# dobrosketchkun/dither_pie

Hardware: AMD Instinct MI355X
Metric: Mpixel/s dither+quantize @4K 256-color (Bayer 8x8 + nearest-palette, uint8 RGB in/out) (higher is better)
Workload: dtype u8; 1 GPU; C2: Bayer 8x8 + 256-colour nearest palette palr(256,7), 3840x2160 RGB, 24 distinct frames rnd(2160,3840,1234+i) per GPU resident in HBM, frames sharded per rank; frames_per_gpu=24, h=2160, w=3840, colors=256, matrix=8x8, parallelism=frames x1

## Files before the change

dither_pie_amd/csrc/accel.hip:

```cpp
#include <algorithm>
#include <cstdio>
#include <cstdlib>
#include <string>
#include <vector>

#include "dp_internal.h"
#include "ordered_fine.h"
#include "tree_query.hip.h"

namespace dp {
namespace {

__device__ __forceinline__ int med3i(const int a, const int b, const int c)
{
    return max(min(a, b), min(max(a, b), c));
}

constexpr int kExcCap = 1 << 16;

template <int MW, int CAP>
__global__ __launch_bounds__(256) void accel_scan_kernel(const PalDev pal, uint32_t *__restrict__ masks,
                                                         uint32_t *__restrict__ nmasks, uint32_t *__restrict__ nsub, uint32_t *__restrict__ code1,
                                                         uint32_t *__restrict__ code2, uint4 *__restrict__ exc,
                                                         uint32_t *__restrict__ exc_count)
// ... 196 lines not shown
{
    const int cell = blockIdx.x;
    const int rc = cell >> 8, gc = (cell >> 4) & 15, bc = cell & 15;
    const int K = pal.K;
    constexpr int kBig = 0x7fffffff;
    constexpr int IM = (1 << kIdxBits) - 1;
    for (int t = 0; t < 16; ++t) {
        const int id = threadIdx.x + 256 * t;
        const uint32_t r = rc * 16 + (id >> 8), g = gc * 16 + ((id >> 4) & 15), b = bc * 16 + (id & 15);
        const uint32_t x4 = r | (g << 8) | (b << 16);
        int m0 = kBig, m1 = kBig, m2 = kBig, m3 = kBig;
        for (int j = 0; j < K; ++j) {
            const int dot = (int)__builtin_amdgcn_udot4(x4, pal.p4[j], 0u, false);
            const int key = pal.nkey[j] - (dot << (kIdxBits + 1));
            const int n3 = med3i(m2, m3, key);
            const int n2 = med3i(m1, m2, key);
            const int n1 = med3i(m0, m1, key);
            m0 = min(m0, key);
            m1 = n1;
            m2 = n2;
            m3 = n3;
        }
        const int d1 = m1 >> kIdxBits, d2 = m2 >> kIdxBits, d3 = m3 >> kIdxBits;
        const uint32_t ur = lut[r], ug = lut[256 + g], ub = lut[512 + b];
        const uint32_t wcell = ((ur >> 4) << 8) | ((ug >> 4) << 4) | (ub >> 4);
        const uint32_t sub = 1u + ((((ur >> 3) & 1u) << 2) | (((ug >> 3) & 1u) << 1) | ((ub >> 3) & 1u));
        uint32_t *whole = masks + (size_t)wcell * 9 * MW, *part = whole + (size_t)sub * MW;
        auto mark = [&](int j) {
            const uint32_t bit = 1u << (j & 31);
            if (!(whole[j >> 5] & bit)) atomicOr(&whole[j >> 5], bit);
            if (!(part[j >> 5] & bit)) atomicOr(&part[j >> 5], bit);
        };
        mark(m0 & IM);
        if (K > 1) mark(m1 & IM);
        if (K > 2 && d2 == d1) mark(m2 & IM);
        if (K > 3 && d3 == d1)
            for (int j = 0; j < K; ++j) {
                const int dot = (int)__builtin_amdgcn_udot4(x4, pal.p4[j], 0u, false);
                const int dj = (pal.nkey[j] - (dot << (kIdxBits + 1))) >> kIdxBits;
                if (dj <= d1) mark(j);
            }
    }
}


constexpr double kFloatListMargin = 1.0 + 6.103515625e-5;

__device__ __forceinline__ void float_members(const double *s_pts, const int K, const double r, const double g,
                                              const double b, uint32_t *mask_a, uint32_t *mask_b)
{
    const double inf = __longlong_as_double(0x7ff0000000000000LL);
    double b0 = inf, b1 = inf;
    for (int j = 0; j < K; ++j) {
        const double d = sq_dist3(s_pts + 3 * j, r, g, b);
        if (d < b1) {
            if (d < b0) {
                b1 = b0;
                b0 = d;
            } else {
                b1 = d;
            }
        }
    }
    const double bound = __dmul_rn(b1, kFloatListMargin);
    for (int j = 0; j < K; ++j) {
        const double d = sq_dist3(s_pts + 3 * j, r, g, b);
        if (d <= bound) {
            atomicOr(&mask_a[j >> 5], 1u << (j & 31));
            if (mask_b) atomicOr(&mask_b[j >> 5], 1u << (j & 31));
        }
    }
}

__global__ __launch_bounds__(256) void accel_scan_float_kernel(const PalDev pal, const uint8_t *__restrict__ reach,
                                                               uint32_t *__restrict__ masks)
{
    __shared__ uint32_t s_mask[9][8];
    __shared__ double s_pts[256 * 3];
    if (threadIdx.x < 72) (&s_mask[0][0])[threadIdx.x] = 0;
    for (int i = threadIdx.x; i < pal.K * 3; i += 256) s_pts[i] = pal.pts[i];
    __syncthreads();
    const int cell = blockIdx.x;
    const int rc = cell >> 8, gc = (cell >> 4) & 15, bc = cell & 15;
    for (int t = 0; t < 16; ++t) {
        const int id = threadIdx.x + 256 * t;
        const int r = rc * 16 + (id >> 8), g = gc * 16 + ((id >> 4) & 15), b = bc * 16 + (id & 15);
        if (!(reach[r] && reach[g] && reach[b])) continue;
        const int sub = 1 + (((((id >> 8) >> 3) & 1) << 2) | (((((id >> 4) & 15) >> 3) & 1) << 1) | (((id & 15) >> 3) & 1));
        float_members(s_pts, pal.K, (double)r, (double)g, (double)b, s_mask[0], s_mask[sub]);
    }
    __syncthreads();
    if (threadIdx.x < 72) masks[cell * 72 + threadIdx.x] = (&s_mask[0][0])[threadIdx.x];
}

__global__ __launch_bounds__(64) void accel_box_float_kernel(const PalDev pal, const uint8_t *__restrict__ reach,
                                                             const Box *__restrict__ boxes, uint32_t *__restrict__ masks)
{
    __shared__ uint32_t s_mask[8];
    __shared__ double s_pts[256 * 3];
    if (threadIdx.x < 8) s_mask[threadIdx.x] = 0;
    for (int i = threadIdx.x; i < pal.K * 3; i += 64) s_pts[i] = pal.pts[i];
    __syncthreads();
    const Box bx = boxes[blockIdx.x];
    const int n = bx.size * bx.size * bx.size;
    for (int id = threadIdx.x; id < n; id += 64) {
        const int r = bx.r0 + id / (bx.size * bx.size), g = bx.g0 + (id / bx.size) % bx.size, b = bx.b0 + id % bx.size;
        if (!(reach[r] && reach[g] && reach[b])) continue;
        float_members(s_pts, pal.K, (double)r, (double)g, (double)b, s_mask, nullptr);
    }
    __syncthreads();
    if (threadIdx.x < 8) masks[blockIdx.x * 8 + threadIdx.x] = s_mask[threadIdx.x];
}

}

namespace {


template <class B, class Launch>
int run_box_kernel(const std::vector<B> &boxes, std::vector<uint32_t> &bm, Launch launch)
{
    B *d_boxes = nullptr;
    uint32_t *d_bm = nullptr;
    hipError_t e = hipMalloc((void **)&d_boxes, sizeof(B) * boxes.size());
    if (e == hipSuccess) e = hipMalloc((void **)&d_bm, sizeof(uint32_t) * bm.size());
    if (e == hipSuccess) e = hipMemcpy(d_boxes, boxes.data(), sizeof(B) * boxes.size(), hipMemcpyHostToDevice);
    if (e == hipSuccess) {
        launch(d_boxes, d_bm, (unsigned)boxes.size());
        e = hipGetLastError();
    }
    if (e == hipSuccess) e = hipMemcpy(bm.data(), d_bm, sizeof(uint32_t) * bm.size(), hipMemcpyDeviceToHost);
    if (d_boxes) (void)hipFree(d_boxes);
    if (d_bm) (void)hipFree(d_bm);
    if (e != hipSuccess) return hip_fail(e, "accelerator refinement");
    return DP_OK;
}

}

int build_accel(PalDev &dev, const std::vector<uint32_t> &p4_host, void **blob_out, size_t *blob_bytes, std::vector<uint32_t> *fine_masks,
                uint32_t **fine_dev)
{
    *blob_out = nullptr;
    *blob_bytes = 0;
    fine_masks->clear();
    *fine_dev = nullptr;
    const int K = dev.K;
    constexpr size_t kCodeWords = (size_t)1 << 20;
    uint32_t *d_masks = nullptr;
    uint8_t *blob = nullptr;
    const int mw = K <= 256 ? 8 : 32;
    const bool big_q = dev.n_inner > kQueueSmall;
    const size_t bytes = sizeof(uint32_t) * (3 * kCodeWords + 2 * kTabMaxWords + kTabCapWords) + sizeof(uint4) * kExcCap + 16 + 768 +
                         sizeof(uint32_t) * (2 * kCells + 2 * kWideCap * kWideList + kCompactMaxWords) + kLeanTabBytes;
    DP_HIP(hipMalloc((void **)&blob, bytes));
    struct DevFree {
        void *p = nullptr;
        ~DevFree()
        {
            if (p) (void)hipFree(p);
        }
    } masks_guard;
    hipError_t e = hipMalloc((void **)&d_masks, sizeof(uint32_t) * kCells * 18 * mw);
    masks_guard.p = d_masks;
    uint32_t *d_nmasks = d_masks + (size_t)kCells * 9 * mw, *d_nsub = d_nmasks + (size_t)kCells * mw;
    if (e == hipSuccess) e = hipMemset(blob, 0, sizeof(uint32_t) * 3 * kCodeWords);
    if (e != hipSuccess) {
        (void)hipFree(blob);
        return hip_fail(e, "accelerator allocation");
    }
    uint32_t *code1 = reinterpret_cast<uint32_t *>(blob);
    uint32_t *code2 = code1 + kCodeWords;
    uint32_t *d_tab = code2 + 2 * kCodeWords;
    uint4 *d_exc = reinterpret_cast<uint4 *>(d_tab + kTabMaxWords);
    uint32_t *d_exc_count = reinterpret_cast<uint32_t *>(d_exc + kExcCap);
    e = hipMemset(d_exc_count, 0, sizeof(uint32_t));
    if (e != hipSuccess) {
        (void)hipFree(blob);
        return hip_fail(e, "accelerator allocation");
    }
#define DP_SCAN(MW, C) hipLaunchKernelGGL((accel_scan_kernel<MW, C>), dim3(kCells), dim3(256), 0, 0, dev, d_masks, d_nmasks, d_nsub, code1, code2, d_exc, d_exc_count)
    if (mw == 8) {
        if (big_q) DP_SCAN(8, kQueueLarge); else DP_SCAN(8, kQueueSmall);
    } else {
        if (big_q) DP_SCAN(32, kQueueLarge); else DP_SCAN(32, kQueueSmall);
    }
#undef DP_SCAN
    std::vector<uint32_t> masks((size_t)kCells * 9 * mw), nmasks((size_t)kCells * 9 * mw);
    e = hipGetLastError();
    if (e == hipSuccess) e = hipMemcpy(masks.data(), d_masks, sizeof(uint32_t) * masks.size(), hipMemcpyDeviceToHost);
    if (e == hipSuccess) e = hipMemcpy(nmasks.data(), d_nmasks, sizeof(uint32_t) * nmasks.size(), hipMemcpyDeviceToHost);
    if (e != hipSuccess) {
        (void)hipFree(blob);
        return hip_fail(e, "accelerator scan");
    }

    std::vector<uint32_t> tab;
    TableStats st;
    auto box_masks = [&](const std::vector<Box> &boxes, std::vector<uint32_t> &bm) {
        return run_box_kernel(boxes, bm, [&](const Box *db, uint32_t *dm, unsigned n) {
            if (mw == 8) hipLaunchKernelGGL(accel_box_kernel<8>, dim3(n), dim3(64), 0, 0, dev, db, dm);
            else hipLaunchKernelGGL(accel_box_kernel<32>, dim3(n), dim3(64), 0, 0, dev, db, dm);
        });
    };
    std::vector<uint32_t> tab4, perm4, perm8, wide4, wide8;
    TableStats st4;
    bool use4 = false;
    if (K <= 64) {
        const int rc4 = assemble_table(masks, mw, 4, kTabCapWords, K, p4_host, p4_host, box_masks, tab4, st4, nmasks.data(), 4, &perm4, &wide4);
        if (rc4 != DP_OK) {
            (void)hipFree(blob);
            return rc4;
        }
        use4 = !st4.too_big && st4.n_split_cells <= kCells * 4 / 100;
        if (exp_env("DP_DEBUG_ACCEL"))
            fprintf(stderr, "accel K=%d: 4-entry table: %d split cells, %d split nodes, %d slow, %zu words, too_big=%d -> use=%d\n", K,
                    st4.n_split_cells, st4.n_split, st4.n_slow, tab4.size(), (int)st4.too_big, (int)use4);
    }
    const bool have8 = K >= 8;
    if (have8) {
        const int rc = assemble_table(masks, mw, 8, kTabMaxWords, K, p4_host, p4_host, box_masks, tab, st, nmasks.data(), kNearSlots, &perm8, &wide8);
        if (rc != DP_OK) {
            (void)hipFree(blob);
            return rc;
        }
        if (exp_env("DP_DEBUG_ACCEL"))
            fprintf(stderr, "accel K=%d: 8-entry table: %d split cells, %d split nodes, %d slow, %zu words (%s), longest list %d, too_big=%d\n",
                    K, st.n_split_cells, st.n_split, st.n_slow, tab.size(), tab.size() <= (size_t)kTabCapWords ? "all in LDS" : "deep nodes in global memory",
                    st.max_cnt, (int)st.too_big);
    }
    if ((!have8 || st.too_big) && !use4) {
        (void)hipFree(blob);
        return DP_OK;
    }
    const std::vector<uint32_t> mass = mass_points(p4_host);
    const int n_mass = (int)mass.size();
    const bool ok8 = have8 && !st.too_big;
    const bool u8_spilled = ok8 && tab.size() > (size_t)kTabCapWords;
    const int m4 = use4 ? entries_in_split_cells(tab4, 4, mass) : n_mass;
    const int m8 = ok8 ? entries_in_split_cells(tab, 8, mass) : n_mass;
    if (use4 && ok8 && m4 * 20 > n_mass && m8 * 2 <= m4) use4 = false;
    const char *force_env = exp_env("DP_FORCE_TABLE");
    const std::string force = force_env ? force_env : "";
    if (force == "u4") use4 = K <= 64 && !st4.too_big;
    else if (!force.empty() && ok8) use4 = false;
    const int u_mass = use4 ? m4 : m8;
    const int u_cells = use4 ? st4.n_split_cells : st.n_split_cells;
    const bool u_spilled = !use4 && u8_spilled;
    const bool u_crowded = u_spilled || u_cells > kCells * 3 / 100 || u_mass * 4 >= n_mass;
    const bool try_warp = (u_crowded && !(use4 && m4 * 50 <= n_mass)) || u_mass * 50 > n_mass;
    std::vector<uint32_t> wtab;
    TableStats wst;
    WarpMaps wm;
    int wbw = 0, w_mass = 0;
    bool w_spilled = false;
    uint32_t *d_wtab = d_exc_count + 4 + kTabCapWords;
    uint8_t *d_lut = reinterpret_cast<uint8_t *>(d_wtab + kTabMaxWords);
    if (K >= 8 && (try_warp || force[0] == 'w') && force[0] != 'u' && !exp_env("DP_NO_WARP")) {
        make_warp(p4_host, wm);
        auto warped = [&](const uint32_t c) {
            return (uint32_t)wm.lut[0][c & 255] | ((uint32_t)wm.lut[1][(c >> 8) & 255] << 8) | ((uint32_t)wm.lut[2][(c >> 16) & 255] << 16);
        };
        std::vector<uint32_t> coordw(K), massw(mass.size());
        for (int j = 0; j < K; ++j) coordw[j] = warped(p4_host[j]);
        for (size_t j = 0; j < mass.size(); ++j) massw[j] = warped(mass[j]);
        e = hipMemcpy(d_lut, &wm.lut[0][0], 768, hipMemcpyHostToDevice);
        if (e == hipSuccess) e = hipMemset(d_masks, 0, sizeof(uint32_t) * kCells * 9 * mw);
        if (e == hipSuccess) {
            if (mw == 8) hipLaunchKernelGGL(accel_scan_warp_kernel<8>, dim3(kCells), dim3(256), 0, 0, dev, d_lut, d_masks);
            else hipLaunchKernelGGL(accel_scan_warp_kernel<32>, dim3(kCells), dim3(256), 0, 0, dev, d_lut, d_masks);
            e = hipGetLastError();
        }
        std::vector<uint32_t> wmasks((size_t)kCells * 9 * mw);
        if (e == hipSuccess) e = hipMemcpy(wmasks.data(), d_masks, sizeof(uint32_t) * wmasks.size(), hipMemcpyDeviceToHost);
        if (e != hipSuccess) {
            (void)hipFree(blob);
            return hip_fail(e, "accelerator scan (warped cells)");
        }
        auto box_masks_w = [&](const std::vector<Box> &boxes, std::vector<uint32_t> &bm) {
            std::vector<Range> ranges(boxes.size());
            for (size_t q = 0; q < boxes.size(); ++q) {
                const Box &b = boxes[q];
                ranges[q] = Range{wm.lo[0][b.r0], wm.lo[0][b.r0 + b.size], wm.lo[1][b.g0], wm.lo[1][b.g0 + b.size],
                                  wm.lo[2][b.b0], wm.lo[2][b.b0 + b.size]};
            }
            return run_box_kernel(ranges, bm, [&](const Range *db, uint32_t *dm, unsigned n) {
                if (mw == 8) hipLaunchKernelGGL(accel_range_kernel<8>, dim3(n), dim3(256), 0, 0, dev, db, dm);
                else hipLaunchKernelGGL(accel_range_kernel<32>, dim3(n), dim3(256), 0, 0, dev, db, dm);
            });
        };
        int w4_mass = -1;
        if (K <= 64 && force != "w8") {
            TableStats s4;
            std::vector<uint32_t> t4;
            const int rc4 = assemble_table(wmasks, mw, 4, kTabCapWords - 192, K, coordw, p4_host, box_masks_w, t4, s4);
            if (rc4 != DP_OK) {
                (void)hipFree(blob);
                return rc4;
            }
            w4_mass = s4.too_big ? n_mass : entries_in_split_cells(t4, 4, massw);
            if (!s4.too_big && ((s4.n_split_cells <= kCells / 100 && s4.n_slow == 0 && w4_mass * 50 <= n_mass) || force == "w4")) {
                wtab.swap(t4);
                wst = s4;
                wbw = 4;
                w_mass = w4_mass;
            }
        }
        if (wbw == 0) {
            const int rc8 = assemble_table(wmasks, mw, 8, kTabMaxWords, K, coordw, p4_host, box_masks_w, wtab, wst);
            if (rc8 != DP_OK) {
                (void)hipFree(blob);
                return rc8;
            }
            if (!wst.too_big) {
                wbw = 8;
                w_spilled = wtab.size() > (size_t)(kTabCapWords - 192);
                w_mass = entries_in_split_cells(wtab, 8, massw);
                if (w_spilled) crowded_nodes_first(wtab, wst, 8, coordw);
            }
        }
        if (exp_env("DP_DEBUG_ACCEL"))
            fprintf(stderr, "accel K=%d: mass in split cells: plain 4-entry %d, plain 8-entry %d of %d (in use: %d-entry, %d cells%s); warped 4-entry %d, "
                    "warped %d-entry table: %d, %d split cells, %d nodes, %d slow, %zu words%s\n",
                    K, m4, m8, n_mass, use4 ? 4 : 8, u_cells, u_spilled ? ", spilled" : "", w4_mass, wbw, w_mass, wst.n_split_cells, wst.n_split,
                    wst.n_slow, wtab.size(), w_spilled ? " (deep nodes in global memory)" : "");
        if (wbw != 0 && (w_mass * 2 > u_mass || (u_mass - w_mass) * 50 < n_mass) && !(u_spilled && !w_spilled) && force.empty()) wbw = 0;
    } else if (exp_env("DP_DEBUG_ACCEL")) {
        fprintf(stderr, "accel K=%d: mass in split cells: plain 4-entry %d, plain 8-entry %d of %d (in use: %d-entry, %d cells)\n", K, m4, m8, n_mass,
                use4 ? 4 : 8, u_cells);
    }
    dev.warp_tab = nullptr;
    dev.warp_lut = nullptr;
    dev.warp_words = dev.warp_total = dev.warp_bw = dev.warp_adapt = 0;
    dev.adapt = (!use4 && u_crowded) ? 1 : 0;
    if (wbw != 0) {
        e = hipMemcpy(d_wtab, wtab.data(), sizeof(uint32_t) * wtab.size(), hipMemcpyHostToDevice);
        if (e != hipSuccess) {
            (void)hipFree(blob);
            return hip_fail(e, "accelerator upload (warped cells)");
        }
        dev.warp_tab = d_wtab;
        dev.warp_lut = d_lut;
        dev.warp_bw = wbw;
        dev.warp_total = (int)wtab.size();
        dev.warp_words = w_spilled ? std::min((int)wtab.size(), kTabStageWords - 3 * 64) : (int)wtab.size();
        dev.warp_adapt = (wbw == 8 && (w_spilled || wst.n_split_cells > kCells * 3 / 100 || w_mass * 4 >= n_mass)) ? 1 : 0;
    }
    dev.cell_perm = dev.cell_perm4 = nullptr;
    dev.near_slots = 0;
    const bool fast8 = have8 && !st.too_big && !st.wide_overflow && !use4 && wbw == 0 && !dev.adapt && tab.size() <= (size_t)kTabCapWords &&
                       wide8.size() <= (size_t)kWideCap * kWideList && !exp_env("DP_NO_FAST");
    if (exp_env("DP_DEBUG_ACCEL") && have8)
        fprintf(stderr, "accel K=%d: fast kernel on the 8-entry table: %s (%d cells with a nearest set above %d entries, %zu flat lists)\n", K,
                fast8 ? "yes" : "no", st.n_near_overflow, kNearSlots, wide8.size() / kWideList);
    if (!fast8) perm8.clear();
    uint32_t *d_perm8 = reinterpret_cast<uint32_t *>(d_lut + 768), *d_perm4 = d_perm8 + kCells;
    uint32_t *d_wide8 = d_perm4 + kCells, *d_wide4 = d_wide8 + kWideCap * kWideList;
    dev.cell_wide = dev.cell_wide4 = nullptr;
    dev.n_wide = dev.n_wide4 = 0;
    if (!perm8.empty()) {
        e = hipMemcpy(d_perm8, perm8.data(), sizeof(uint32_t) * kCells, hipMemcpyHostToDevice);
        if (e == hipSuccess && !wide8.empty()) e = hipMemcpy(d_wide8, wide8.data(), sizeof(uint32_t) * wide8.size(), hipMemcpyHostToDevice);
        dev.cell_wide = d_wide8;
        dev.n_wide = (int)(wide8.size() / kWideList);
        if (e != hipSuccess) {
            (void)hipFree(blob);
            return hip_fail(e, "accelerator upload (staging order)");
        }
        dev.cell_perm = d_perm8;
        dev.near_slots = kNearSlots;
    }
    if (use4 && wbw == 0 && !perm4.empty() && !st4.wide_overflow && wide4.size() <= (size_t)kWideCap * kWideList && !exp_env("DP_NO_FAST")) {
        e = hipMemcpy(d_perm4, perm4.data(), sizeof(uint32_t) * kCells, hipMemcpyHostToDevice);
        if (e == hipSuccess && !wide4.empty()) e = hipMemcpy(d_wide4, wide4.data(), sizeof(uint32_t) * wide4.size(), hipMemcpyHostToDevice);
        dev.cell_wide4 = d_wide4;
        dev.n_wide4 = (int)(wide4.size() / kWideList);
        if (e != hipSuccess) {
            (void)hipFree(blob);
            return hip_fail(e, "accelerator upload (staging order)");
        }
        dev.cell_perm4 = d_perm4;
    }
    dev.cell_tab = nullptr;
    dev.tab_words = 0;
    dev.tab_total = 0;
    if (have8 && !st.too_big && tab.size() > (size_t)kTabCapWords) crowded_nodes_first(tab, st, 8, p4_host);
    dev.comp_tab = nullptr;
    dev.comp_words = dev.comp_warp = 0;
    {
        const bool from_warp = wbw == 8 && (dev.warp_adapt != 0 || exp_env("DP_FORCE_COMPACT"));
        const bool from_plain = wbw == 0 && (dev.adapt != 0 || exp_env("DP_FORCE_COMPACT")) && have8 && !st.too_big;
        const std::vector<uint32_t> &src = from_warp ? wtab : tab;
        if (K <= 256 && (from_warp || from_plain) && src.size() / 4 <= (size_t)kCompactMaxWords && !exp_env("DP_NO_COMPACT")) {
            const std::vector<uint32_t> ct = compact_table(src, p4_host);
            uint32_t *d_comp = d_wide4 + kWideCap * kWideList;
            e = hipMemcpy(d_comp, ct.data(), sizeof(uint32_t) * ct.size(), hipMemcpyHostToDevice);
            if (e != hipSuccess) {
                (void)hipFree(blob);
                return hip_fail(e, "accelerator upload (compact table)");
            }
            dev.comp_tab = d_comp;
            dev.comp_words = (int)ct.size();
            dev.comp_warp = from_warp ? 1 : 0;
            if (exp_env("DP_DEBUG_ACCEL"))
                fprintf(stderr, "accel K=%d: compact table over %s cells: %zu bytes\n", K, from_warp ? "warped" : "plain", ct.size() * 4);
        }
    }
    dev.fine_tab = nullptr;
    dev.fine_words = dev.fine_win = dev.fine_wide = 0;
    if (have8 && !st.too_big && !use4 && wbw == 0 && !dev.adapt && mw == 8 && K >= kWideList && !exp_env("DP_NO_FINE")) {
        fine_masks->resize((size_t)2 * kFineCells * mw);
        uint32_t *ftm = fine_masks->data(), *fnm = ftm + (size_t)kFineCells * mw;
        for (int cell = 0; cell < kCells; ++cell)
            for (int sub = 0; sub < 8; ++sub) {
                const int rc = cell >> 8, gc = (cell >> 4) & 15, bc = cell & 15;
                const size_t fc = (size_t)fine_cell(rc * 16 + ((sub >> 2) & 1) * 8, gc * 16 + ((sub >> 1) & 1) * 8, bc * 16 + (sub & 1) * 8);
                std::copy_n(&masks[((size_t)cell * 9 + 1 + sub) * mw], mw, &ftm[fc * mw]);
                std::copy_n(&nmasks[((size_t)kCells + (size_t)cell * 8 + sub) * mw], mw, &fnm[fc * mw]);
            }
        *fine_dev = d_wide4 + kWideCap * kWideList + kCompactMaxWords;
    }
    if (have8 && !st.too_big) {
        e = hipMemcpy(d_tab, tab.data(), sizeof(uint32_t) * tab.size(), hipMemcpyHostToDevice);
        if (e != hipSuccess) {
            (void)hipFree(blob);
            return hip_fail(e, "accelerator upload");
        }
        dev.cell_tab = d_tab;
        dev.tab_total = (int)tab.size();
        dev.tab_words = tab.size() <= (size_t)kTabCapWords ? (int)tab.size() : std::min((int)tab.size(), kTabStageWords);
    } else {
        st = st4;
    }
    dev.cell_tab4 = nullptr;
    dev.tab4_words = 0;
    if (use4) {
        uint32_t *d_tab4 = d_exc_count + 4;
        e = hipMemcpy(d_tab4, tab4.data(), sizeof(uint32_t) * tab4.size(), hipMemcpyHostToDevice);
        if (e != hipSuccess) {
            dev.cell_tab = nullptr;
            (void)hipFree(blob);
            return hip_fail(e, "accelerator upload");
        }
        dev.cell_tab4 = d_tab4;
        dev.tab4_words = (int)tab4.size();
    }
    dev.n_split = st.n_split;
    dev.n_slow_blocks = st.n_slow;
    dev.n_split_cells = st.n_split_cells;
    dev.max_cell = st.max_cnt;
    dev.code1 = code1;
    dev.code2 = code2;
    {
        uint32_t n_exc = 0;
        e = hipMemcpy(&n_exc, d_exc_count, sizeof(uint32_t), hipMemcpyDeviceToHost);
        if (e == hipSuccess && n_exc > 0 && n_exc <= (uint32_t)kExcCap) {
            std::vector<uint4> ex(n_exc);
            e = hipMemcpy(ex.data(), d_exc, sizeof(uint4) * n_exc, hipMemcpyDeviceToHost);
            std::sort(ex.begin(), ex.end(), [](const uint4 &a, const uint4 &b) { return a.x < b.x; });
            if (e == hipSuccess) e = hipMemcpy(d_exc, ex.data(), sizeof(uint4) * n_exc, hipMemcpyHostToDevice);
        }
        if (e != hipSuccess) {
            dev.cell_tab = nullptr;
            (void)hipFree(blob);
            return hip_fail(e, "accelerator exception list");
        }
        dev.exc = d_exc;
        dev.n_exc = n_exc <= (uint32_t)kExcCap ? (int)n_exc : -1;
    }
    *blob_out = blob;
    *blob_bytes = bytes;
    return DP_OK;
}

int build_fine(PalDev &dev, const std::vector<uint32_t> &p4_host, const std::vector<uint32_t> &fine_masks, uint32_t *fine_dev)
{
    constexpr int mw = 8;
    FineTable ft;
    fine_pack(fine_masks.data(), fine_masks.data() + (size_t)kFineCells * mw, mw, dev.K, p4_host, fine_table_fits, ft);
    if (exp_env("DP_DEBUG_ACCEL"))
        fprintf(stderr, "accel K=%d: fine table: %s, %d windows, %d wide cells, %lld bytes\n", dev.K, ft.ok ? "yes" : "no", ft.n_win, ft.n_wide,
                (long long)fine_table_bytes(ft.n_win, ft.n_wide));
    if (!ft.ok) return DP_OK;
    const std::vector<uint32_t> im = ft.lds_image();
    const hipError_t e = hipMemcpy(fine_dev, im.data(), sizeof(uint32_t) * im.size(), hipMemcpyHostToDevice);
    if (e != hipSuccess) return hip_fail(e, "accelerator upload (fine table)");
    dev.fine_tab = fine_dev;
    dev.fine_words = (int)im.size();
    dev.fine_win = ft.n_win;
    dev.fine_wide = ft.n_wide;
    return DP_OK;
}

int build_accel_float(PalDev &dev, const float *pal_f32, const uint8_t *lut_host, void **blob_out, size_t *blob_bytes)
{
    *blob_out = nullptr;
    *blob_bytes = 0;
    const int K = dev.K;
    std::vector<uint8_t> reach(256, lut_host ? 0 : 1);
    if (lut_host)
        for (int v = 0; v < 256; ++v) reach[lut_host[v]] = 1;
    std::vector<uint32_t> coord4(K), word(K);
    for (int j = 0; j < K; ++j) {
        uint32_t c[3];
        for (int k = 0; k < 3; ++k) {
            const float v = pal_f32[3 * j + k];
            c[k] = (uint32_t)std::min(255.0f, std::max(0.0f, std::nearbyint(v)));
        }
        coord4[j] = c[0] | (c[1] << 8) | (c[2] << 16);
        word[j] = (uint32_t)j * 16u;
    }
    const size_t bytes = sizeof(uint32_t) * kTabMaxWords + 256 + sizeof(uint32_t) * kCompactMaxWords;
    uint8_t *blob = nullptr;
    uint32_t *d_masks = nullptr;
    DP_HIP(hipMalloc((void **)&blob, bytes));
    uint32_t *d_tab = reinterpret_cast<uint32_t *>(blob);
    uint8_t *d_reach = blob + sizeof(uint32_t) * kTabMaxWords;
    hipError_t e = hipMalloc((void **)&d_masks, sizeof(uint32_t) * kCells * 72);
    if (e == hipSuccess) e = hipMemcpy(d_reach, reach.data(), 256, hipMemcpyHostToDevice);
    if (e != hipSuccess) {
        (void)hipFree(blob);
        if (d_masks) (void)hipFree(d_masks);
        return hip_fail(e, "float accelerator allocation");
    }
    hipLaunchKernelGGL(accel_scan_float_kernel, dim3(kCells), dim3(256), 0, 0, dev, d_reach, d_masks);
    std::vector<uint32_t> masks((size_t)kCells * 72);
    e = hipGetLastError();
    if (e == hipSuccess) e = hipMemcpy(masks.data(), d_masks, sizeof(uint32_t) * masks.size(), hipMemcpyDeviceToHost);
    (void)hipFree(d_masks);
    if (e != hipSuccess) {
        (void)hipFree(blob);
        return hip_fail(e, "float accelerator scan");
    }
    std::vector<uint32_t> tab;
    TableStats st;
    const int rc = assemble_table(
        masks, 8, 8, kTabMaxWords, K, coord4, word,
        [&](const std::vector<Box> &boxes, std::vector<uint32_t> &bm) {
            return run_box_kernel(boxes, bm, [&](const Box *db, uint32_t *dm, unsigned n) {
                hipLaunchKernelGGL(accel_box_float_kernel, dim3(n), dim3(64), 0, 0, dev, d_reach, db, dm);
            });
        },
        tab, st);
    if (rc != DP_OK || st.too_big) {
        (void)hipFree(blob);
        return rc;
    }
    if ((int)tab.size() > (160 * 1024 - K * 16 - 256) / 4) crowded_nodes_first(tab, st, 8, coord4);
    e = hipMemcpy(d_tab, tab.data(), sizeof(uint32_t) * tab.size(), hipMemcpyHostToDevice);
    if (e != hipSuccess) {
        (void)hipFree(blob);
        return hip_fail(e, "float accelerator upload");
    }
    dev.ftab = d_tab;
    dev.ftab_total = (int)tab.size();
    const int stage_cap = (160 * 1024 - K * 16 - 256) / 4;
    dev.ftab_words = (int)tab.size() <= stage_cap ? (int)tab.size() : 4096 * 8 + ((stage_cap - 4096 * 8) / 64) * 64;
    dev.n_split = st.n_split;
    dev.n_slow_blocks = st.n_slow;
    dev.max_cell = st.max_cnt;
    dev.comp_tab = nullptr;
    dev.comp_words = dev.comp_warp = 0;
    if (K <= 256 && tab.size() / 4 <= (size_t)kCompactMaxWords && !exp_env("DP_NO_COMPACT")) {
        const std::vector<uint32_t> ct = compact_table(tab, word);
        uint32_t *d_comp = reinterpret_cast<uint32_t *>(d_reach + 256);
        e = hipMemcpy(d_comp, ct.data(), sizeof(uint32_t) * ct.size(), hipMemcpyHostToDevice);
        if (e != hipSuccess) {
            (void)hipFree(blob);
            dev.ftab = nullptr;
            return hip_fail(e, "float accelerator upload (compact table)");
        }
        dev.comp_tab = d_comp;
        dev.comp_words = (int)ct.size();
    }
    *blob_out = blob;
    *blob_bytes = bytes;
    return DP_OK;
}

}
```

dither_pie_amd/csrc/dp_internal.h:

```cpp
#pragma once
#include <hip/hip_runtime.h>

#include <atomic>
#include <cstdarg>
#include <cstdint>
#include <cstdio>
#include <cstdlib>
#include <mutex>
#include <vector>

#include "../../include/ditherpie_hip.h"
#include "host_logic.h"

namespace dp {

constexpr int kQueueTiles = 65536;
constexpr int kIdxBits = 10;
constexpr int kLocalBits = 8;

void set_error(const char *fmt, ...);

inline const char *exp_env(const char *name)
{
#ifdef DP_EXPERIMENTS
    return std::getenv(name);
#else
    (void)name;
    return nullptr;
#endif
}
int hip_fail(hipError_t e, const char *what);

inline void trace_diffusion(const char *kernel, const char *schedule, int G, long long grid, int waves, size_t lds, int K, int n_inner,
                            int model, int numba, int serpentine)
{
#ifdef DP_EXPERIMENTS
    if (std::getenv("DP_ED_TRACE"))
        fprintf(stderr, "dp_diffusion: kernel=%s schedule=%s G=%d grid=%lld waves=%d lds=%zu K=%d n_inner=%d model=%d numba=%d serpentine=%d repair=%d\n",
                kernel, schedule, G, grid, waves, lds, K, n_inner, model, numba, serpentine ? 1 : 0, G > 1 ? 1 : 0);
#else
    (void)kernel; (void)schedule; (void)G; (void)grid; (void)waves; (void)lds; (void)K; (void)n_inner; (void)model; (void)numba; (void)serpentine;
#endif
}

#define DP_HIP(call)                                   \
    do {                                               \
        hipError_t e__ = (call);                       \
        if (e__ != hipSuccess) return dp::hip_fail(e__, #call); \
    } while (0)

struct PalDev {
    int K;
    int n_nodes;
    int n_inner;
    int is_integer;
    const uint32_t *p4;
    const int32_t *nkey;
    const double *pts;
    const float *pts_f32;
    const uint32_t *out_rgb;
    const uint8_t *lut_in;
    const int32_t *indices;
    const int32_t *split_dim;
    const double *split;
    const int32_t *start, *end, *less, *greater;
    double mins[3], maxes[3];
    const uint32_t *cell_tab;
    int tab_words;
    int tab_total;
    const uint32_t *cell_tab4;
    int tab4_words;
    const uint32_t *cell_perm;
    const uint32_t *cell_perm4;
    int near_slots;
    const uint32_t *cell_wide, *cell_wide4;
    int n_wide, n_wide4;
    int adapt;
    const uint32_t *warp_tab;
    const uint8_t *warp_lut;
    int warp_words, warp_total;
    int warp_bw;
    int warp_adapt;
    const uint32_t *comp_tab;
    int comp_words;
    int comp_warp;
    const uint32_t *fine_tab;
    int fine_words;
    int fine_win, fine_wide;
    int n_split;
    int n_slow_blocks;
    int n_split_cells;
    int max_cell;
    const uint32_t *code1;
    const uint32_t *code2;
    const uint32_t *ftab;
    int ftab_words;
    int ftab_total;
    const float4 *fcand;
    const uint4 *ed_cells;
    const uint4 *ed_nodes;
    const uint32_t *ed_coarse;
    const uint32_t *ed_coarse_ext;
    const uint4 *ed_ext16;
    const uint4 *ed_ext_nodes;
    const uint4 *ed_lists16;
    const uint32_t *ed_h4;
    int ed_h4_words;
    int ed_h4_shallow;
    int ed_h4_global;
    int ed_h4_lds_words;
    const uint4 *exc;
    int n_exc;
};

struct ThrDev {
    int th_h, th_w;
    const float *f32;
    const uint32_t *m;
    int sh;
    const float *fpad;
    const uint32_t *mpad;
    uint32_t cls_nib[32];
    int has_cls;
    int tw_pad;
    int pow2;
    double inv_h, inv_w;
};

inline ThrDev no_thresholds()
{
    ThrDev t{};
    t.th_h = t.th_w = 1;
    t.pow2 = 1;
    t.inv_h = t.inv_w = 1.0;
    return t;
}

struct PatDev {
    const uint8_t *tab;
    const uint32_t *c_rank;
    const uint32_t *out_rank;
    int K;
    int brick;
};

struct MetDev {
    const uint16_t *tab;
    const int4 *lab;
    const uint32_t *out_rgb;
    const uint16_t *cbrt;
    int K;
};

}

struct dp_palette {
    dp::PalDev dev;
    void *blob;
    size_t blob_bytes;
    void *accel_blob;
    void *ed_blob;
    void *ext_blob;
    size_t accel_bytes;
    bool accel_tried, same_out;
    std::vector<uint32_t> p4_host;
    std::vector<float> pal_host;
    std::vector<uint8_t> lut_host;
    bool float_accel;
    int device;
    std::vector<double> pts_host;
    bool ed_tried;
    bool ext_tried;
    std::mutex build_mu, dev_mu;
    dp::PatDev pat;
    void *pat_blob;
    std::vector<uint32_t> fine_masks;
    uint32_t *fine_dev;
    std::atomic<bool> fine_pending;
    int metric;
    dp::MetDev met;
    void *met_blob;
};

struct dp_thresholds {
    dp::ThrDev dev;
    void *blob;
    void *blob_pad;
    int device;
};

namespace dp {
struct ProfMark {
    hipEvent_t ev[3];
    int n;
};
bool prof_on();
ProfMark *prof_begin(hipStream_t s);
void prof_mid(ProfMark *m, hipStream_t s);
void prof_end(ProfMark *m, hipStream_t s);
}

namespace dp {
int build_accel(PalDev &dev, const std::vector<uint32_t> &p4_host, void **blob_out, size_t *blob_bytes, std::vector<uint32_t> *fine_masks,
                uint32_t **fine_dev);
int build_fine(PalDev &dev, const std::vector<uint32_t> &p4_host, const std::vector<uint32_t> &fine_masks, uint32_t *fine_dev);
int build_accel_float(PalDev &dev, const float *pal_f32, const uint8_t *lut_host, void **blob_out, size_t *blob_bytes);
int build_ed_cells(PalDev &dev, const double *pts_host, void **blob_out);
int build_ed_ext(PalDev &dev, const double *pts_host, void **blob_out);
int launch_ordered(const uint8_t *in, uint8_t *out, int64_t n_frames, int h, int w, int y0, int x0,
                   const PalDev &pal, int mode, const ThrDev *thr, float ign_scale, int ign_seed, void *ws,
                   size_t ws_bytes, hipStream_t s);
int launch_ign_thresholds(float *out, int h, int w, int y0, int x0, float scale, int seed, hipStream_t s);
int launch_blue_noise(int size, uint32_t seed, float *out_dev, void *scratch_dev, hipStream_t s);
size_t blue_noise_scratch_bytes(int size);
int launch_error_diffusion(const uint8_t *in, uint8_t *out, int64_t n_frames, int h, int w, const PalDev &pal,
                           const int32_t *dx, const int32_t *dy, const float *wq, int ntaps, int serpentine,
                           void *ws, size_t ws_bytes, hipStream_t s, const double *wq64 = nullptr, const double *hybrid = nullptr);
size_t error_diffusion_ws_bytes(int64_t n_frames, int h, int w);
int launch_kmeans_step(const uint8_t *px, int64_t n, const double *centers, const double *mean, int K, int64_t *sums, int64_t *counts,
                       int64_t *sumsq, hipStream_t s);
size_t distinct_first_ws_bytes(int64_t n);
int launch_distinct_first(const uint8_t *px, int64_t n, uint8_t *out, long long *n_distinct, void *ws, hipStream_t s);
size_t distinct_stream_state_bytes();
size_t distinct_stream_ws_bytes(int64_t n);
int launch_distinct_stream_reset(void *state, long long *n_distinct, hipStream_t s);
int launch_distinct_stream_add(const uint8_t *px, int64_t n, void *state, uint8_t *list, long long *n_distinct, void *ws, hipStream_t s);
size_t hist_sample_ws_bytes();
int launch_hist_sample(const void *hist, const long long *ranks, int n_ranks, uint8_t *out, unsigned long long *n_bad, void *ws, hipStream_t s);
size_t kmeans_hist_bytes();
size_t kmeans_hist_ws_bytes(int64_t n);
int launch_kmeans_hist_build(const uint8_t *px, int64_t n, void *hist, int accumulate, void *ws, hipStream_t s);
int launch_kmeans_hist_step(const void *hist, const double *centers, const double *mean, int K, int64_t *sums, int64_t *counts,
                            int64_t *sumsq, hipStream_t s);
int launch_kmeans_hist_iterate(const void *hist, double *centers, const double *mean, int K, int64_t *totals, int64_t *prev,
                               double *status, uint32_t *ticket, double tol, int max_iter, int first, hipStream_t s);
int launch_kmeans_pp(const uint8_t *sample, int n, int K, int first, const double *uniforms, int n_trials, int *out_ids,
                     double *out_centers, hipStream_t s);
int launch_kmeans_update(const int64_t *totals, double *centers, int64_t *prev, double *status, int K, double tol, int max_iter,
                         hipStream_t s);
int launch_variance_gate(const uint8_t *in, uint8_t *gate, int64_t n_frames, int h, int w, const PalDev &pal, float thr,
                         int radius, void *ws, hipStream_t s);
size_t variance_gate_ws_bytes(int64_t n_frames, int h, int w);
int launch_variable_diffusion(const uint8_t *in, uint8_t *out, int64_t n_frames, int h, int w, const PalDev &pal, int model,
                              float p0, float p1, int serpentine, const uint8_t *gate, const float *coef, void *ws,
                              hipStream_t s);
int launch_riemersma(const uint8_t *in, uint8_t *out, int64_t n_frames, int h, int w, const PalDev &pal, hipStream_t s);
size_t halftone_ws_bytes(int64_t n_frames, int h, int w, const dp_halftone_params &P);
int launch_halftone(const uint8_t *in, uint8_t *out, int64_t n_frames, int h, int w, const PalDev &pal,
                    const dp_halftone_params &P, void *ws, size_t ws_bytes, hipStream_t s);
int launch_halftone_pow_flags(int h, int w, const dp_halftone_params &P, int32_t *idx, int64_t cap,
                              unsigned long long *count, hipStream_t s);
int wavelet_filter_len(int wid);
int64_t wavelet_uniforms_needed(int h, int w, int wid);
size_t wavelet_ws_bytes(int64_t n_frames, int h, int w, int wid);
int launch_wavelet(const uint8_t *in, uint8_t *out, int64_t n_frames, int h, int w, const PalDev &pal,
                   const dp_wavelet_params &P, void *ws, size_t ws_bytes, hipStream_t s);
int pattern_check_palette(const char *fn, const dp_palette *p);
int pattern_ensure_table(const dp_palette *pal, hipStream_t s);
PatDev pattern_snapshot(const dp_palette *pal);
bool metric_refused(const char *fn, const dp_palette *pal);
int palette_create_impl(const char *fn, const float *pal_f32, const uint8_t *out_colors, int K, const uint8_t *lut_in, int metric,
                        dp_palette **out);
int metric_ensure_table_locked(dp_palette *p, hipStream_t s);
int launch_metric_rank_table(const MetDev &md, const uint32_t *rank_of, uint8_t *tab, hipStream_t s);
int launch_void_cluster(uint16_t *ranks_dev, int n_matrices, const uint32_t *seeds_host, int h, int w, int sigma256, hipStream_t s);
int launch_resize_nearest(const uint8_t *in, uint8_t *out, int64_t n_frames, int h, int w, int oh, int ow,
                          hipStream_t s);
}
```

dither_pie_amd/csrc/host.cpp:

```cpp
#include <algorithm>
#include <cmath>
#include <cstring>
#include <limits>
#include <numeric>

#include "dp_internal.h"
#include "../../include/ditherpie_hip_dotdiff.h"
#include "../../include/ditherpie_hip_cells.h"
#include "../../include/ditherpie_hip_voidcluster.h"

namespace dp {

static thread_local char g_err[512] = "";

void set_error(const char *fmt, ...)
{
    va_list ap;
    va_start(ap, fmt);
    vsnprintf(g_err, sizeof(g_err), fmt, ap);
    va_end(ap);
}

int hip_fail(hipError_t e, const char *what)
{
    set_error("HIP error %d (%s) in %s", (int)e, hipGetErrorString(e), what);
    return e == hipErrorOutOfMemory ? DP_ENOMEM : DP_EHIP;
}


static thread_local bool g_prof = false;
static thread_local std::vector<ProfMark> *g_marks = nullptr;

bool prof_on() { return g_prof; }

ProfMark *prof_begin(hipStream_t s)
{
    if (!g_prof) return nullptr;
    if (!g_marks) g_marks = new std::vector<ProfMark>();
    if (g_marks->capacity() < 65536) g_marks->reserve(65536);
    if (g_marks->size() >= 65536) return nullptr;
    ProfMark m;
    m.n = 0;
    for (auto &e : m.ev) {
        if (hipEventCreate(&e) != hipSuccess) return nullptr;
    }
    g_marks->push_back(m);
    ProfMark *p = &g_marks->back();
    (void)hipEventRecord(p->ev[0], s);
    p->n = 1;
    return p;
}

void prof_mid(ProfMark *m, hipStream_t s)
{
    if (!m) return;
    (void)hipEventRecord(m->ev[1], s);
    m->n = 2;
}

void prof_end(ProfMark *m, hipStream_t s)
{
    if (!m) return;
    if (m->n == 1) prof_mid(m, s);
    (void)hipEventRecord(m->ev[2], s);
    m->n = 3;
}

}

using namespace dp;

extern "C" {

int dp_version(void) { return DP_ABI_VERSION; }

const char *dp_last_error(void) { return g_err; }

int dp_device_info(int *n_devices, char *arch_buf, size_t arch_buf_len)
{
    int n = 0;
    hipError_t e = hipGetDeviceCount(&n);
    if (e != hipSuccess) {
        n = 0;
        (void)hipGetLastError();
    }
    if (n_devices) *n_devices = n;
    if (arch_buf && arch_buf_len) {
        arch_buf[0] = 0;
        if (n > 0) {
            int dev = 0;
            DP_HIP(hipGetDevice(&dev));
            hipDeviceProp_t prop;
            DP_HIP(hipGetDeviceProperties(&prop, dev));
            snprintf(arch_buf, arch_buf_len, "%s", prop.gcnArchName);
        }
    }
    return DP_OK;
}

int dp_kdtree_build_host(const double *pts, int K, int32_t *indices, int32_t *split_dim, double *split,
                         int32_t *start, int32_t *end, int32_t *less, int32_t *greater, int *n_nodes)
{
    if (!pts || K < 1 || !indices || !split_dim || !split || !start || !end || !less || !greater || !n_nodes) {
        set_error("dp_kdtree_build_host: bad argument");
        return DP_EINVAL;
    }
    HostTree t;
    build_tree(pts, K, t);
    const size_t n = t.split_dim.size();
    std::memcpy(indices, t.indices.data(), sizeof(int32_t) * (size_t)K);
    std::memcpy(split_dim, t.split_dim.data(), sizeof(int32_t) * n);
    std::memcpy(split, t.split.data(), sizeof(double) * n);
    std::memcpy(start, t.start.data(), sizeof(int32_t) * n);
    std::memcpy(end, t.end.data(), sizeof(int32_t) * n);
    std::memcpy(less, t.less.data(), sizeof(int32_t) * n);
    std::memcpy(greater, t.greater.data(), sizeof(int32_t) * n);
    *n_nodes = (int)n;
    return DP_OK;
}

int dp_palette_create(const float *pal_f32, const uint8_t *out_colors, int K, const uint8_t *lut_in,
                      dp_palette **out)
{
    return dp::palette_create_impl("dp_palette_create", pal_f32, out_colors, K, lut_in, 0, out);
}

}

int dp::palette_create_impl(const char *fn, const float *pal_f32, const uint8_t *out_colors, int K, const uint8_t *lut_in, int metric,
                            dp_palette **out)
{
    if (!pal_f32 || !out_colors || !out || K < 1) {
        set_error("%s: bad argument", fn);
        return DP_EINVAL;
    }
    if (K > DP_MAX_COLORS) {
        set_error("%s: %d colours requested, this backend supports at most %d", fn, K,
                  DP_MAX_COLORS);
        return DP_EUNSUPPORTED;
    }
    std::vector<double> pts((size_t)K * 3);
    bool integer = (lut_in == nullptr);
    for (int i = 0; i < K * 3; ++i) {
        const float v = pal_f32[i];
        if (!std::isfinite(v)) {
            set_error("%s: non-finite palette value", fn);
            return DP_EINVAL;
        }
        pts[i] = (double)v;
        if (!(v >= 0.0f && v <= 255.0f && v == std::floor(v))) integer = false;
    }
    HostTree t;
    build_tree(pts.data(), K, t);
    const int nn = (int)t.split_dim.size();
    int inner = 0;
    for (int i = 0; i < nn; ++i) inner += t.split_dim[i] >= 0;
    if (inner > kQueueLarge) {
        set_error("%s: KD-tree with %d inner nodes exceeds the device traversal queue (%d)", fn, inner,
                  kQueueLarge);
        return DP_EUNSUPPORTED;
    }

    std::vector<uint8_t> blob;
    auto put = [&](const void *src, size_t bytes) {
        size_t off = (blob.size() + 15) & ~size_t(15);
        blob.resize(off + bytes);
        if (bytes) std::memcpy(blob.data() + off, src, bytes);
        return off;
    };
    std::vector<uint32_t> p4(K), orgb(K);
    std::vector<int32_t> nkey(K);
    for (int j = 0; j < K; ++j) {
        orgb[j] = (uint32_t)out_colors[3 * j] | ((uint32_t)out_colors[3 * j + 1] << 8) |
                  ((uint32_t)out_colors[3 * j + 2] << 16);
        if (integer) {
            const uint32_t r = (uint32_t)pal_f32[3 * j], g = (uint32_t)pal_f32[3 * j + 1],
                           b = (uint32_t)pal_f32[3 * j + 2];
            p4[j] = r | (g << 8) | (b << 16);
            nkey[j] = (int32_t)(((r * r + g * g + b * b) << kIdxBits) | (uint32_t)j);
        } else {
            p4[j] = 0;
            nkey[j] = 0;
        }
    }
    const size_t o_p4 = put(p4.data(), sizeof(uint32_t) * K);
    const size_t o_nk = put(nkey.data(), sizeof(int32_t) * K);
    const size_t o_pts = put(pts.data(), sizeof(double) * 3 * K);
    const size_t o_pf = put(pal_f32, sizeof(float) * 3 * K);
    const size_t o_org = put(orgb.data(), sizeof(uint32_t) * K);
    const size_t o_lut = lut_in ? put(lut_in, 256) : 0;
    std::vector<float> fcand((size_t)K * 4);
    for (int j = 0; j < K; ++j) {
        fcand[4 * j] = pal_f32[3 * j];
        fcand[4 * j + 1] = pal_f32[3 * j + 1];
        fcand[4 * j + 2] = pal_f32[3 * j + 2];
        std::memcpy(&fcand[4 * j + 3], &orgb[j], sizeof(float));
    }
    const size_t o_fc = put(fcand.data(), sizeof(float) * 4 * K);
    const size_t o_idx = put(t.indices.data(), sizeof(int32_t) * K);
    const size_t o_sd = put(t.split_dim.data(), sizeof(int32_t) * nn);
    const size_t o_sp = put(t.split.data(), sizeof(double) * nn);
    const size_t o_st = put(t.start.data(), sizeof(int32_t) * nn);
    const size_t o_en = put(t.end.data(), sizeof(int32_t) * nn);
    const size_t o_le = put(t.less.data(), sizeof(int32_t) * nn);
    const size_t o_gr = put(t.greater.data(), sizeof(int32_t) * nn);

    dp_palette *p = new (std::nothrow) dp_palette();
    if (!p) return DP_ENOMEM;
    p->blob = nullptr;
    p->blob_bytes = blob.size();
    hipError_t e = hipGetDevice(&p->device);
    if (e == hipSuccess) e = hipMalloc(&p->blob, blob.size());
    if (e == hipSuccess) e = hipMemcpy(p->blob, blob.data(), blob.size(), hipMemcpyHostToDevice);
    if (e != hipSuccess) {
        if (p->blob) (void)hipFree(p->blob);
        delete p;
        return hip_fail(e, "dp_palette_create upload");
    }
    const uint8_t *base = (const uint8_t *)p->blob;
    PalDev &d = p->dev;
    d = PalDev{};
    d.K = K;
    d.n_nodes = nn;
    d.n_inner = inner;
    d.is_integer = integer ? 1 : 0;
    d.p4 = (const uint32_t *)(base + o_p4);
    d.nkey = (const int32_t *)(base + o_nk);
    d.pts = (const double *)(base + o_pts);
    d.pts_f32 = (const float *)(base + o_pf);
    d.out_rgb = (const uint32_t *)(base + o_org);
    d.lut_in = lut_in ? (base + o_lut) : nullptr;
    d.fcand = (const float4 *)(base + o_fc);
    d.indices = (const int32_t *)(base + o_idx);
    d.split_dim = (const int32_t *)(base + o_sd);
    d.split = (const double *)(base + o_sp);
    d.start = (const int32_t *)(base + o_st);
    d.end = (const int32_t *)(base + o_en);
    d.less = (const int32_t *)(base + o_le);
    d.greater = (const int32_t *)(base + o_gr);
    for (int c = 0; c < 3; ++c) {
        d.mins[c] = t.mins[c];
        d.maxes[c] = t.maxes[c];
    }
    p->ed_blob = nullptr;
    p->ext_blob = nullptr;
    p->accel_blob = nullptr;
    p->accel_bytes = 0;
    p->accel_tried = false;
    p->p4_host = p4;
    p->same_out = integer && K >= 4 && K <= DP_MAX_COLORS;
    for (int j = 0; j < K && p->same_out; ++j) p->same_out = (orgb[j] == p4[j]);
    p->float_accel = !integer && K >= 8 && K <= 256;
    for (int i = 0; i < 3 * K && p->float_accel; ++i) p->float_accel = pal_f32[i] >= 0.0f && pal_f32[i] <= 255.0f;
    if (p->float_accel) {
        p->pal_host.assign(pal_f32, pal_f32 + 3 * K);
        if (lut_in) p->lut_host.assign(lut_in, lut_in + 256);
    }
    p->pts_host = pts;
    p->ed_tried = false;
    p->ext_tried = false;
    p->pat = dp::PatDev{nullptr, nullptr, nullptr, 0, 0};
    p->pat_blob = nullptr;
    p->fine_dev = nullptr;
    p->fine_pending = false;
    p->metric = metric;
    p->met = dp::MetDev{nullptr, nullptr, nullptr, nullptr, 0};
    p->met_blob = nullptr;
    *out = p;
    return DP_OK;
}

extern "C" {

static dp::PalDev snapshot(const dp_palette *pal_c)
{
    dp_palette *p = const_cast<dp_palette *>(pal_c);
    std::lock_guard<std::mutex> lock(p->dev_mu);
    return p->dev;
}

static void publish(dp_palette *p, const dp::PalDev &d)
{
    std::lock_guard<std::mutex> lock(p->dev_mu);
    p->dev = d;
}

static int ensure_ed_tables(const dp_palette *pal_c)
{
    dp_palette *p = const_cast<dp_palette *>(pal_c);
    std::lock_guard<std::mutex> lock(p->build_mu);
    if (p->ed_tried) return DP_OK;
    p->ed_tried = true;
    if (p->dev.K > 8 && p->dev.K <= DP_MAX_COLORS) {
        dp::PalDev d = snapshot(p);
        const int rc = build_ed_cells(d, p->pts_host.data(), &p->ed_blob);
        if (rc != DP_OK) return rc;
        publish(p, d);
    }
    return DP_OK;
}

static int ensure_ed_ext(const dp_palette *pal_c)
{
    dp_palette *p = const_cast<dp_palette *>(pal_c);
    std::lock_guard<std::mutex> lock(p->build_mu);
    if (p->ext_tried) return DP_OK;
    p->ext_tried = true;
    if (p->dev.K > 16) {
        dp::PalDev d = snapshot(p);
        const int rc = build_ed_ext(d, p->pts_host.data(), &p->ext_blob);
        if (rc != DP_OK) return rc;
        publish(p, d);
    }
    return DP_OK;
}

static int ensure_fine_table(const dp_palette *pal_c, hipStream_t s)
{
    dp_palette *p = const_cast<dp_palette *>(pal_c);
    std::lock_guard<std::mutex> lock(p->build_mu);
    if (!p->fine_pending.load()) return DP_OK;
    hipStreamCaptureStatus capturing = hipStreamCaptureStatusNone;
    if (hipStreamIsCapturing(s, &capturing) != hipSuccess || capturing != hipStreamCaptureStatusNone) return DP_OK;
    p->fine_pending = false;
    dp::PalDev d = snapshot(p);
    const int rc = build_fine(d, p->p4_host, p->fine_masks, p->fine_dev);
    std::vector<uint32_t>().swap(p->fine_masks);
    if (rc != DP_OK) return rc;
    publish(p, d);
    return DP_OK;
}

void dp_palette_destroy(dp_palette *p)
{
    if (!p) return;
    if (p->ed_blob) (void)hipFree(p->ed_blob);
    if (p->ext_blob) (void)hipFree(p->ext_blob);
    if (p->blob) (void)hipFree(p->blob);
    if (p->accel_blob) (void)hipFree(p->accel_blob);
    if (p->pat_blob) (void)hipFree(p->pat_blob);
    if (p->met_blob) (void)hipFree(p->met_blob);
    delete p;
}

int dp_palette_info(const dp_palette *p, int *K, int *is_integer, int *n_nodes)
{
    if (!p) {
        set_error("dp_palette_info: NULL palette");
        return DP_EINVAL;
    }
    if (K) *K = p->dev.K;
    if (is_integer) *is_integer = p->dev.is_integer;
    if (n_nodes) *n_nodes = p->dev.n_nodes;
    return DP_OK;
}

int dp_palette_build_accel(dp_palette *p)
{
    if (!p) {
        set_error("dp_palette_build_accel: NULL palette");
        return DP_EINVAL;
    }
    if (p->metric != 0) return DP_OK;
    std::lock_guard<std::mutex> lock(p->build_mu);
    if (p->accel_tried || !(p->same_out || p->float_accel)) return DP_OK;
    p->accel_tried = true;
    dp::PalDev d = snapshot(p);
    int rc;
    if (p->float_accel)
        rc = build_accel_float(d, p->pal_host.data(), p->lut_host.empty() ? nullptr : p->lut_host.data(), &p->accel_blob,
                               &p->accel_bytes);
    else
        rc = build_accel(d, p->p4_host, &p->accel_blob, &p->accel_bytes, &p->fine_masks, &p->fine_dev);
    if (rc == DP_OK) publish(p, d);
    if (rc == DP_OK && !p->fine_masks.empty()) p->fine_pending = true;
    return rc;
}

int dp_palette_accel_info(const dp_palette *p, int *pool_entries, int *max_cell)
{
    if (!p) {
        set_error("dp_palette_accel_info: NULL palette");
        return DP_EINVAL;
    }
    const dp::PalDev d = snapshot(p);
    if (pool_entries) *pool_entries = d.cell_tab ? d.tab_words : (d.cell_tab4 ? d.tab4_words : (d.ftab ? d.ftab_words : 0));
    if (max_cell) *max_cell = (d.cell_tab || d.cell_tab4 || d.ftab) ? d.max_cell : 0;
    return DP_OK;
}

static hipError_t thresholds_upload(void *dst, const void *src, size_t bytes, bool on_stream, hipStream_t s)
{
    if (!on_stream) return hipMemcpy(dst, src, bytes, hipMemcpyHostToDevice);
    const hipError_t e = hipMemcpyAsync(dst, src, bytes, hipMemcpyHostToDevice, s);
    return e == hipSuccess ? hipStreamSynchronize(s) : e;
}

static int thresholds_from_device_f32(float *dev_f32, int th_h, int th_w, const float *host_copy,
                                      dp_thresholds **out, bool on_stream = false, hipStream_t stream = nullptr)
{
    const int n = th_h * th_w;
    int sh = -1;
    std::vector<uint32_t> m;
    for (int s = 0; s <= 13 && sh < 0; ++s) {
        bool ok = true;
        for (int i = 0; i < n && ok; ++i) {
            const double v = (double)host_copy[i] * (double)(1u << s);
            ok = host_copy[i] >= 0.0f && host_copy[i] <= 1.0f && v == std::floor(v);
        }
        if (ok) sh = s;
    }
    dp_thresholds *t = new (std::nothrow) dp_thresholds();
    if (!t) return DP_ENOMEM;
    t->blob = dev_f32;
    (void)hipGetDevice(&t->device);
    t->dev = dp::no_thresholds();
    t->dev.th_h = th_h;
    t->dev.th_w = th_w;
    t->dev.f32 = dev_f32;
    t->blob_pad = nullptr;
    if (sh >= 0) {
        m.resize(n);
        for (int i = 0; i < n; ++i) m[i] = (uint32_t)((double)host_copy[i] * (double)(1u << sh));
        uint32_t *dm = (uint32_t *)(dev_f32 + n);
        hipError_t e = thresholds_upload(dm, m.data(), sizeof(uint32_t) * n, on_stream, stream);
        if (e != hipSuccess) {
            delete t;
            return hip_fail(e, "thresholds integer upload");
        }
        t->dev.m = dm;
        t->dev.sh = sh;
    }
    t->dev.pow2 = ((th_h & (th_h - 1)) == 0 && (th_w & (th_w - 1)) == 0) ? 1 : 0;
    t->dev.inv_h = 1.0 / (double)th_h;
    t->dev.inv_w = 1.0 / (double)th_w;
    if ((int64_t)th_h * (th_w + 3) <= (1 << 18)) {
        const int twp = th_w + 3;
        const size_t np = (size_t)th_h * twp;
        std::vector<uint32_t> pad(2 * np);
        for (int y = 0; y < th_h; ++y)
            for (int x = 0; x < twp; ++x) {
                const size_t src = (size_t)y * th_w + (x % th_w);
                std::memcpy(&pad[(size_t)y * twp + x], &host_copy[src], sizeof(float));
                pad[np + (size_t)y * twp + x] = sh >= 0 ? m[src] : 0u;
            }
        if (n <= 256 && t->dev.pow2) {
            bool any = false;
            for (int r = 0; r < th_h; ++r)
                for (int p0 = 0; p0 < th_w; ++p0) {
                    uint32_t bits = 0;
                    for (int q = 0; q < 4; ++q) {
                        bool all = true;
                        for (int l = 0; l < 64 && all; ++l) all = host_copy[(size_t)r * th_w + (size_t)((p0 + 4 * l + q) % th_w)] >= 0.5f;
                        bits |= all ? (1u << q) : 0u;
                    }
                    const int idx = r * th_w + p0;
                    t->dev.cls_nib[idx >> 3] |= bits << ((idx & 7) * 4);
                    any |= bits != 0;
                }
            t->dev.has_cls = any ? 1 : 0;
        }
        void *dp = nullptr;
        hipError_t e = hipMalloc(&dp, sizeof(uint32_t) * pad.size());
        if (e == hipSuccess) e = thresholds_upload(dp, pad.data(), sizeof(uint32_t) * pad.size(), on_stream, stream);
        if (e != hipSuccess) {
            if (dp) (void)hipFree(dp);
            delete t;
            return hip_fail(e, "thresholds padded upload");
        }
        t->blob_pad = dp;
        t->dev.fpad = (const float *)dp;
        t->dev.mpad = sh >= 0 ? (const uint32_t *)dp + np : nullptr;
        t->dev.tw_pad = twp;
    }
    *out = t;
    return DP_OK;
}

int dp_thresholds_create(const float *thr_host, int th_h, int th_w, dp_thresholds **out)
{
    if (!thr_host || !out || th_h < 1 || th_w < 1 || (int64_t)th_h * th_w > (1 << 20)) {
        set_error("dp_thresholds_create: bad argument");
        return DP_EINVAL;
    }
    const int n = th_h * th_w;
    for (int i = 0; i < n; ++i)
        if (std::isnan(thr_host[i])) {
            set_error("dp_thresholds_create: NaN threshold");
            return DP_EINVAL;
        }
    float *d = nullptr;
    DP_HIP(hipMalloc((void **)&d, sizeof(float) * 2 * (size_t)n));
    hipError_t e = hipMemcpy(d, thr_host, sizeof(float) * n, hipMemcpyHostToDevice);
    if (e != hipSuccess) {
        (void)hipFree(d);
        return hip_fail(e, "dp_thresholds_create upload");
    }
    int rc = thresholds_from_device_f32(d, th_h, th_w, thr_host, out);
    if (rc != DP_OK) (void)hipFree(d);
    return rc;
}

int dp_thresholds_blue_noise(int size, uint32_t seed, void *stream, dp_thresholds **out)
{
    if (!out || size < 2 || size > 256) {
        set_error("dp_thresholds_blue_noise: size must be in [2,256]");
        return DP_EINVAL;
    }
    const int n = size * size;
    float *d = nullptr;
    void *scratch = nullptr;
    DP_HIP(hipMalloc((void **)&d, sizeof(float) * 2 * (size_t)n));
    hipStream_t s = (hipStream_t)stream;
    hipError_t e = hipMallocAsync(&scratch, blue_noise_scratch_bytes(size), s);
    if (e != hipSuccess) {
        (void)hipFree(d);
        return hip_fail(e, "blue-noise scratch");
    }
    int rc = launch_blue_noise(size, seed, d, scratch, s);
    std::vector<float> host(n);
    if (rc == DP_OK) {
        e = hipMemcpyAsync(host.data(), d, sizeof(float) * n, hipMemcpyDeviceToHost, s);
        if (e == hipSuccess) e = hipStreamSynchronize(s);
        if (e != hipSuccess) rc = hip_fail(e, "blue-noise download");
    }
    (void)hipFreeAsync(scratch, s);
    if (rc == DP_OK) rc = thresholds_from_device_f32(d, size, size, host.data(), out, true, s);
    if (rc != DP_OK) (void)hipFree(d);
    return rc;
}

int dp_thresholds_shape(const dp_thresholds *t, int *th_h, int *th_w, int *is_integer_form)
{
    if (!t) {
        set_error("dp_thresholds_shape: NULL");
        return DP_EINVAL;
    }
    if (th_h) *th_h = t->dev.th_h;
    if (th_w) *th_w = t->dev.th_w;
    if (is_integer_form) *is_integer_form = t->dev.m != nullptr;
    return DP_OK;
}

int dp_thresholds_download(const dp_thresholds *t, float *thr_host)
{
    if (!t || !thr_host) {
        set_error("dp_thresholds_download: NULL");
        return DP_EINVAL;
    }
    DP_HIP(hipMemcpy(thr_host, t->dev.f32, sizeof(float) * (size_t)t->dev.th_h * t->dev.th_w,
                     hipMemcpyDeviceToHost));
    return DP_OK;
}

void dp_thresholds_destroy(dp_thresholds *t)
{
    if (!t) return;
    if (t->blob) (void)hipFree(t->blob);
    if (t->blob_pad) (void)hipFree(t->blob_pad);
    delete t;
}

int dp_ign_thresholds(float *out_dev, int h, int w, int y0, int x0, float scale, int seed, void *stream)
{
    if (!out_dev || h < 1 || w < 1) {
        set_error("dp_ign_thresholds: bad argument");
        return DP_EINVAL;
    }
    return launch_ign_thresholds(out_dev, h, w, y0, x0, scale, seed, (hipStream_t)stream);
}

size_t dp_ordered_workspace_bytes(int64_t n_frames, int h, int w)
{
    if (n_frames < 0 || h < 0 || w < 0) return 0;
    const int64_t npx = n_frames * (int64_t)h * w;
    const int64_t tiles = (npx + 255) / 256;
    return (size_t)(tiles * 32 + 1024 + 4 * ((size_t)dp::kQueueTiles + 8));
}

int dp_ordered_u8(const uint8_t *in_dev, uint8_t *out_dev, int64_t n_frames, int h, int w, int y0, int x0,
                  const dp_palette *pal, int mode, const dp_thresholds *thr, float ign_scale, int ign_seed,
                  void *workspace_dev, size_t workspace_bytes, void *stream)
{
    if (metric_refused("dp_ordered_u8", pal)) return DP_EUNSUPPORTED;
    if (n_frames == 0 && pal && h >= 1 && w >= 1) return DP_OK;
    if (!in_dev || !out_dev || !pal || n_frames < 0 || h < 1 || w < 1 || y0 < 0 || x0 < 0) {
        set_error("dp_ordered_u8: bad argument");
        return DP_EINVAL;
    }
    if (mode != DP_MODE_NEAREST && mode != DP_MODE_MATRIX && mode != DP_MODE_IGN) {
        set_error("dp_ordered_u8: unknown mode %d", mode);
        return DP_EINVAL;
    }
    if (mode == DP_MODE_MATRIX && !thr) {
        set_error("dp_ordered_u8: DP_MODE_MATRIX needs a threshold matrix");
        return DP_EINVAL;
    }
    if ((int64_t)h * w > (int64_t)1 << 30 || (int64_t)y0 + h > (int64_t)1 << 30 || (int64_t)x0 + w > (int64_t)1 << 30) {
        set_error("dp_ordered_u8: frame too large");
        return DP_EINVAL;
    }
    if (n_frames == 0) return DP_OK;
    if (!workspace_dev || workspace_bytes < dp_ordered_workspace_bytes(n_frames, h, w) ||
        ((uintptr_t)workspace_dev & 15)) {
        set_error("dp_ordered_u8: workspace too small or misaligned (need %zu bytes, 16-byte aligned)",
                  dp_ordered_workspace_bytes(n_frames, h, w));
        return DP_EWORKSPACE;
    }
    if (mode == DP_MODE_MATRIX && thr->dev.mpad && pal->fine_pending.load(std::memory_order_relaxed)) {
        const int rc = ensure_fine_table(pal, (hipStream_t)stream);
        if (rc != DP_OK) return rc;
    }
    return launch_ordered(in_dev, out_dev, n_frames, h, w, y0, x0, snapshot(pal), mode, thr ? &thr->dev : nullptr,
                          ign_scale, ign_seed, workspace_dev, workspace_bytes, (hipStream_t)stream);
}

size_t dp_error_diffusion_workspace_bytes(int64_t n_frames, int h, int w)
{
    if (n_frames < 0 || h < 0 || w < 0) return 0;
    return error_diffusion_ws_bytes(n_frames, h, w);
}

static int error_diffusion_common(const uint8_t *in_dev, uint8_t *out_dev, int64_t n_frames, int h, int w,
                                  const dp_palette *pal, const int32_t *dx, const int32_t *dy, const float *wq,
                                  const double *wq64, int ntaps, int serpentine, void *workspace_dev, size_t workspace_bytes,
                                  void *stream, const char *fn, const double *hybrid = nullptr);

int dp_error_diffusion_u8(const uint8_t *in_dev, uint8_t *out_dev, int64_t n_frames, int h, int w,
                          const dp_palette *pal, const int32_t *dx, const int32_t *dy, const float *wq,
                          int ntaps, int serpentine, void *workspace_dev, size_t workspace_bytes,
                          void *stream)
{
    return error_diffusion_common(in_dev, out_dev, n_frames, h, w, pal, dx, dy, wq, nullptr, ntaps, serpentine, workspace_dev,
                                  workspace_bytes, stream, "dp_error_diffusion_u8");
}

int dp_error_diffusion_numba_u8(const uint8_t *in_dev, uint8_t *out_dev, int64_t n_frames, int h, int w,
                                const dp_palette *pal, const int32_t *dx, const int32_t *dy, const float *weights,
                                double divisor, int ntaps, int serpentine, void *workspace_dev, size_t workspace_bytes,
                                void *stream)
{
    if (ntaps < 0 || ntaps > 16 || (ntaps && !weights) || !(divisor > 0.0)) {
        set_error("dp_error_diffusion_numba_u8: bad argument");
        return DP_EINVAL;
    }
    float wq[16];
    double wq64[16];
    for (int k = 0; k < ntaps; ++k) {
        wq64[k] = (double)weights[k] / divisor;
        wq[k] = (float)wq64[k];
    }
    return error_diffusion_common(in_dev, out_dev, n_frames, h, w, pal, dx, dy, wq, wq64, ntaps, serpentine, workspace_dev,
                                  workspace_bytes, stream, "dp_error_diffusion_numba_u8");
}

int dp_hybrid_numba_u8(const uint8_t *in_dev, uint8_t *out_dev, int64_t n_frames, int h, int w, const dp_palette *pal,
                       double lum_factor, double col_factor, void *workspace_dev, size_t workspace_bytes, void *stream)
{
    static const int32_t dx[4] = {1, -1, 0, 1}, dy[4] = {0, 1, 1, 1};
    static const double wq64[4] = {7.0 / 16.0, 3.0 / 16.0, 5.0 / 16.0, 1.0 / 16.0};
    static const float wq[4] = {7.0f / 16.0f, 3.0f / 16.0f, 5.0f / 16.0f, 1.0f / 16.0f};
    const double hybrid[2] = {lum_factor, col_factor};
    return error_diffusion_common(in_dev, out_dev, n_frames, h, w, pal, dx, dy, wq, wq64, 4, 0, workspace_dev, workspace_bytes, stream,
                                  "dp_hybrid_numba_u8", hybrid);
}

static int error_diffusion_common(const uint8_t *in_dev, uint8_t *out_dev, int64_t n_frames, int h, int w,
                                  const dp_palette *pal, const int32_t *dx, const int32_t *dy, const float *wq,
                                  const double *wq64, int ntaps, int serpentine, void *workspace_dev, size_t workspace_bytes,
                                  void *stream, const char *fn, const double *hybrid)
{
    if (metric_refused(fn, pal)) return DP_EUNSUPPORTED;
    if (n_frames == 0 && pal && h >= 1 && w >= 1) return DP_OK;
    if (!in_dev || !out_dev || !pal || n_frames < 0 || h < 1 || w < 1 || ntaps < 0 || ntaps > 16 ||
        (ntaps && (!dx || !dy || !wq))) {
        set_error("%s: bad argument", fn);
        return DP_EINVAL;
    }
    for (int k = 0; k < ntaps; ++k) {
        const bool forward = dy[k] > 0 || (dy[k] == 0 && dx[k] > 0);
        if (!forward || dy[k] > 2 || dx[k] < -2 || dx[k] > 2) {
            set_error("%s: tap %d (dx=%d, dy=%d) is outside the supported causal window", fn, k, dx[k], dy[k]);
            return DP_EUNSUPPORTED;
        }
    }
    if (n_frames == 0) return DP_OK;
    if (!workspace_dev || workspace_bytes < dp_error_diffusion_workspace_bytes(n_frames, h, w)) {
        set_error("%s: workspace too small (need %zu bytes)", fn, dp_error_diffusion_workspace_bytes(n_frames, h, w));
        return DP_EWORKSPACE;
    }
    const int rc_tab = ensure_ed_tables(pal);
    if (rc_tab != DP_OK) return rc_tab;
    return launch_error_diffusion(in_dev, out_dev, n_frames, h, w, snapshot(pal), dx, dy, wq, ntaps, serpentine,
                                  workspace_dev, workspace_bytes, (hipStream_t)stream, wq64, hybrid);
}

int dp_variable_diffusion_u8(const uint8_t *in_dev, uint8_t *out_dev, int64_t n_frames, int h, int w,
                             const dp_palette *pal, int model, float p0, float p1, int serpentine,
                             const uint8_t *gate_dev, const float *coef_dev, void *workspace_dev,
                             size_t workspace_bytes, void *stream)
{
    if (metric_refused("dp_variable_diffusion_u8", pal)) return DP_EUNSUPPORTED;
    if (n_frames == 0 && pal && h >= 1 && w >= 1) return DP_OK;
    if (!in_dev || !out_dev || !pal || n_frames < 0 || h < 1 || w < 1 || model < 1 || model > 4 ||
        (model == DP_DIFFUSER_ADAPTIVE_VARIANCE && !gate_dev) || (model == DP_DIFFUSER_OSTROMOUKHOV && !coef_dev)) {
        set_error("dp_variable_diffusion_u8: bad argument");
        return DP_EINVAL;
    }
    if (!workspace_dev || workspace_bytes < dp_error_diffusion_workspace_bytes(n_frames, h, w)) {
        set_error("dp_variable_diffusion_u8: workspace too small (need %zu bytes)",
                  dp_error_diffusion_workspace_bytes(n_frames, h, w));
        return DP_EWORKSPACE;
    }
    const int rc_tab = ensure_ed_tables(pal);
    if (rc_tab != DP_OK) return rc_tab;
    if (model != DP_DIFFUSER_OSTROMOUKHOV) {
        const int rc_ext = ensure_ed_ext(pal);
        if (rc_ext != DP_OK) return rc_ext;
    }
    return launch_variable_diffusion(in_dev, out_dev, n_frames, h, w, snapshot(pal), model, p0, p1, serpentine ? 1 : 0,
                                     gate_dev, coef_dev, workspace_dev, (hipStream_t)stream);
}

int dp_riemersma_u8(const uint8_t *in_dev, uint8_t *out_dev, int64_t n_frames, int h, int w, const dp_palette *pal, void *stream)
{
    if (metric_refused("dp_riemersma_u8", pal)) return DP_EUNSUPPORTED;
    if (!pal || n_frames < 0 || h < 0 || w < 0) {
        set_error("dp_riemersma_u8: bad argument (NULL palette or negative size)");
        return DP_EINVAL;
    }
    if (n_frames == 0 || h == 0 || w == 0) return DP_OK;
    if (!in_dev || !out_dev) {
        set_error("dp_riemersma_u8: bad argument (NULL frame buffer)");
        return DP_EINVAL;
    }
    try {
        return launch_riemersma(in_dev, out_dev, n_frames, h, w, snapshot(pal), (hipStream_t)stream);
    } catch (const std::exception &e) {
        set_error("dp_riemersma_u8: %s", e.what());
        return DP_ENOMEM;
    }
}

static bool halftone_params_ok(const char *fn, const dp_halftone_params *P, int K)
{
    if (!P) {
        set_error("%s: bad argument (NULL params)", fn);
        return false;
    }
    if (!(std::isfinite(P->cell_size) && P->cell_size > 0.0)) {
        set_error("%s: bad argument (cell_size must be finite and > 0)", fn);
        return false;
    }
    if (!(std::isfinite(P->cos_a) && std::isfinite(P->sin_a) && std::isfinite(P->exponent) && std::isfinite(P->min_dot) &&
          std::isfinite(P->max_dot) && std::isfinite(P->sharpness))) {
        set_error("%s: bad argument (non-finite parameter)", fn);
        return false;
    }
    if (P->exp_class < DP_HT_EXP_IDENTITY || P->exp_class > DP_HT_EXP_POW || P->shape < DP_HT_SHAPE_CIRCLE ||
        P->shape > DP_HT_SHAPE_DIAMOND) {
        set_error("%s: bad argument (unknown exponent class or shape)", fn);
        return false;
    }
// ... 391 lines not shown
```

dither_pie_amd/csrc/host_logic.h:

```cpp
#pragma once
#include <algorithm>
#include <cmath>
#include <cstdint>
#include <cstring>
#include <initializer_list>
#include <limits>
#include <numeric>
#include <thread>
#include <utility>
#include <exception>
#include <vector>

#include "../../include/ditherpie_hip.h"

namespace dp {

constexpr int kLeafSize = 10;
constexpr int kWideList = 16;
constexpr int kQueueSmall = 64;
constexpr int kQueueLarge = 256;

struct HostTree {
    int K = 0;
    std::vector<double> pts;
// ... 260 lines not shown
        }
        if (st.too_big || kids.empty()) break;
        std::vector<Box> boxes(kids.size());
        for (size_t q = 0; q < kids.size(); ++q) boxes[q] = kids[q].box;
        std::vector<uint32_t> bm(kids.size() * (size_t)mw);
        const int rc = box_masks(boxes, bm);
        if (rc != DP_OK) return rc;
        for (size_t q = 0; q < kids.size(); ++q) {
            const Box &c = kids[q].box;
            uint32_t blk[8];
            if (make_block(&bm[q * (size_t)mw], c.r0 + c.size / 2, c.g0 + c.size / 2, c.b0 + c.size / 2, blk))
                std::copy(blk, blk + bw, tab.begin() + kids[q].pos);
            else
                pending.push_back(kids[q]);
        }
    }
    return DP_OK;
}

inline void crowded_nodes_first(std::vector<uint32_t> &tab, const TableStats &st, const int bw, const std::vector<uint32_t> &coord4)
{
    const size_t n = st.node_box.size();
    if (n < 2) return;
    std::vector<int> score(n, 0);
    for (size_t k = 0; k < n; ++k) {
        const Box &b = st.node_box[k];
        for (const uint32_t c : coord4) {
            const int r = c & 255, g = (c >> 8) & 255, bl = (c >> 16) & 255;
            score[k] += (r >= b.r0 && r < b.r0 + b.size && g >= b.g0 && g < b.g0 + b.size && bl >= b.b0 && bl < b.b0 + b.size);
        }
    }
    std::vector<uint32_t> order(n), where(n);
    for (size_t k = 0; k < n; ++k) order[k] = (uint32_t)k;
    std::stable_sort(order.begin(), order.end(), [&](uint32_t a, uint32_t b) { return score[a] > score[b]; });
    for (size_t k = 0; k < n; ++k) where[order[k]] = (uint32_t)k;
    const size_t base = (size_t)kCells * bw, node_words = 8 * (size_t)bw;
    std::vector<uint32_t> moved(tab.size());
    std::copy(tab.begin(), tab.begin() + base, moved.begin());
    for (size_t k = 0; k < n; ++k)
        std::copy(tab.begin() + base + k * node_words, tab.begin() + base + (k + 1) * node_words,
                  moved.begin() + base + where[k] * node_words);
    for (uint32_t &w : moved)
        if ((w >> 30) == 2u) w = 0x80000000u | where[w & 0xffffffu];
    tab.swap(moved);
}

struct WarpMaps {
    uint8_t lut[3][256];
    int lo[3][257];
};

inline void make_warp(const std::vector<uint32_t> &coord4, WarpMaps &wm)
{
    const size_t K = coord4.size();
    for (int c = 0; c < 3; ++c) {
        std::vector<int> v(K);
        for (size_t j = 0; j < K; ++j) v[j] = (coord4[j] >> (8 * c)) & 255;
        std::sort(v.begin(), v.end());
        int a[17];
        a[0] = 0;
        a[16] = 256;
        for (int i = 1; i < 16; ++i) {
            int q = v[K * (size_t)i / 16];
            q = std::max(q, a[i - 1] + 1);
            q = std::min(q, 256 - (16 - i));
            a[i] = q;
        }
        for (int i = 0; i < 16; ++i) {
            const int w = a[i + 1] - a[i];
            for (int x = a[i]; x < a[i + 1]; ++x) wm.lut[c][x] = (uint8_t)(16 * i + ((x - a[i]) * 16) / w);
        }
        int x = 0;
        for (int u = 0; u <= 256; ++u) {
            while (x < 256 && (int)wm.lut[c][x] < u) ++x;
            wm.lo[c][u] = x;
        }
    }
}

inline std::vector<uint32_t> mass_points(const std::vector<uint32_t> &coord4)
{
    std::vector<uint32_t> out(coord4);
    const size_t K = coord4.size();
    constexpr int kNear = 4;
    for (size_t j = 0; j < K && K > (size_t)kNear; ++j) {
        const int r = coord4[j] & 255, g = (coord4[j] >> 8) & 255, b = (coord4[j] >> 16) & 255;
        uint64_t best[kNear];
        for (uint64_t &v : best) v = ~0ull;
        for (size_t k = 0; k < K; ++k) {
            if (k == j) continue;
            const int dr = (int)(coord4[k] & 255) - r, dg = (int)((coord4[k] >> 8) & 255) - g, db = (int)((coord4[k] >> 16) & 255) - b;
            uint64_t key = ((uint64_t)(dr * dr + dg * dg + db * db) << 32) | k;
            for (uint64_t &v : best)
                if (key < v) std::swap(key, v);
        }
        for (const uint64_t key : best) {
            const uint32_t c = coord4[key & 0xffffffffu];
            const int cr = c & 255, cg = (c >> 8) & 255, cb = (c >> 16) & 255;
            for (const int q : {1, 2})
                out.push_back((uint32_t)(r + (cr - r) * q / 4) | ((uint32_t)(g + (cg - g) * q / 4) << 8) | ((uint32_t)(b + (cb - b) * q / 4) << 16));
        }
    }
    return out;
}

constexpr int kCompactMaxWords = 36 * 1024;
inline std::vector<uint32_t> compact_table(const std::vector<uint32_t> &tab, const std::vector<uint32_t> &coord4)
{
    std::vector<std::pair<uint32_t, uint32_t>> by_colour(coord4.size());
    for (size_t j = 0; j < coord4.size(); ++j) by_colour[j] = {coord4[j], (uint32_t)j};
    std::sort(by_colour.begin(), by_colour.end());
    std::vector<uint32_t> out(tab.size() / 4);
    for (size_t b = 0; b + 8 <= tab.size(); b += 8) {
        if (tab[b] >> 31) {
            const bool split = (tab[b] >> 30) == 2u;
            out[b / 4] = split ? (0x80000000u | (uint32_t)((4096u + (tab[b] & 0xffffffu) * 8u) * 8u)) : 0xC0000000u;
            out[b / 4 + 1] = 0xffffffffu;
            continue;
        }
        uint32_t w[2] = {0u, 0u};
        for (int i = 0; i < 8; ++i) {
            int nth = 0;
            for (int k = 0; k < i; ++k) nth += tab[b + k] == tab[b + i];
            auto it = std::lower_bound(by_colour.begin(), by_colour.end(), std::make_pair(tab[b + i], 0u));
            uint32_t idx = 0u;
            if (it != by_colour.end() && it->first == tab[b + i]) {
                if ((size_t)(it - by_colour.begin()) + nth < by_colour.size() && (it + nth)->first == tab[b + i]) it += nth;
                idx = it->second;
            }
            w[i >> 2] |= idx << (8 * (i & 3));
        }
        out[b / 4] = w[0];
        out[b / 4 + 1] = w[1];
    }
    return out;
}

inline int entries_in_split_cells(const std::vector<uint32_t> &tab, const int bw, const std::vector<uint32_t> &coord4)
{
    int n = 0;
    for (const uint32_t c : coord4) {
        const size_t slot = (size_t)cell_slot((c & 255) >> 4, ((c >> 8) & 255) >> 4, ((c >> 16) & 255) >> 4);
        n += (int)(tab[slot * bw] >> 31);
    }
    return n;
}


constexpr int kFineCells = 32 * 32 * 32;
constexpr int kFineQuad = 4, kFineWindow = 6;
constexpr int kFineIds = kWideCap;

inline int fine_cell(const int r, const int g, const int b) { return (r >> 3) | ((g >> 3) << 5) | ((b >> 3) << 10); }

struct FineTable {
    bool ok = false;
    int n_win = 0, n_wide = 0;
    std::vector<uint16_t> off;
    std::vector<uint32_t> quad;
    std::vector<uint32_t> pair;
    std::vector<uint16_t> win_idx;
    std::vector<uint16_t> wide_cell;
    std::vector<uint32_t> wide;
    std::vector<uint16_t> wide_idx;
    std::vector<uint32_t> lds_image() const
    {
        std::vector<uint32_t> im;
        im.reserve(quad.size() + wide.size() + pair.size() + kFineCells / 2 + kFineIds / 2);
        im.insert(im.end(), quad.begin(), quad.end());
        im.insert(im.end(), wide.begin(), wide.end());
        im.insert(im.end(), pair.begin(), pair.end());
        for (int c = 0; c < kFineCells; c += 2) im.push_back((uint32_t)off[c] | ((uint32_t)off[c + 1] << 16));
        for (int i = 0; i < kFineIds; i += 2) {
            const uint32_t lo = i < n_wide ? wide_cell[i] : 0xffffu, hi = i + 1 < n_wide ? wide_cell[i + 1] : 0xffffu;
            im.push_back(lo | (hi << 16));
        }
        return im;
    }
};

template <class Fits>
void fine_pack(const uint32_t *tmask, const uint32_t *nmask, const int mw, const int K, const std::vector<uint32_t> &coord4, Fits fits,
               FineTable &ft)
{
    ft = FineTable{};
    if (K < kWideList || K > 256 || K > 32 * mw) return;
    struct Mask {
        uint64_t w[4];
        int count() const
        {
            int n = 0;
            for (int i = 0; i < 4; ++i)
                for (uint64_t bits = w[i]; bits; bits &= bits - 1ull) ++n;
            return n;
        }
        bool any() const { return (w[0] | w[1] | w[2] | w[3]) != 0; }
        bool operator==(const Mask &o) const { return w[0] == o.w[0] && w[1] == o.w[1] && w[2] == o.w[2] && w[3] == o.w[3]; }
        Mask without(const Mask &o) const { return Mask{{w[0] & ~o.w[0], w[1] & ~o.w[1], w[2] & ~o.w[2], w[3] & ~o.w[3]}}; }
        Mask with(const Mask &o) const { return Mask{{w[0] | o.w[0], w[1] | o.w[1], w[2] | o.w[2], w[3] | o.w[3]}}; }
        void set(const int j) { w[j >> 6] |= 1ull << (j & 63); }
    };
    auto load = [&](const uint32_t *m) {
        Mask r{{0, 0, 0, 0}};
        for (int wi = 0; wi < mw && wi < 8; ++wi) r.w[wi >> 1] |= (uint64_t)m[wi] << (32 * (wi & 1));
        for (int j = K; j < 256; ++j) r.w[j >> 6] &= ~(1ull << (j & 63));
        return r;
    };
    auto each = [](const Mask &m, auto f) {
        for (int wi = 0; wi < 4; ++wi)
            for (uint64_t bits = m.w[wi]; bits; bits &= bits - 1ull) f(64 * wi + __builtin_ctzll(bits));
    };
    ft.off.assign(kFineCells, 0);
    std::vector<Mask> tms(kFineCells), nms(kFineCells);
    constexpr int kClasses = (kFineWindow + 1) * (kFineQuad + 1);
    int class_count[kClasses + 1] = {0};
    std::vector<uint8_t> cls(kFineCells, 0xff);
    for (int cell = 0; cell < kFineCells; ++cell) {
        const Mask tm = tms[cell] = load(tmask + (size_t)cell * mw), nm = nms[cell] = load(nmask + (size_t)cell * mw);
        const int nt = tm.count(), nn = nm.count();
        if (nt > kWideList) return;
        if (nn > kFineQuad || nt > kFineWindow) {
            if (ft.n_wide == kFineIds || !fits(1, ft.n_wide + 1)) return;
            ++ft.n_wide;
            ft.wide_cell.push_back((uint16_t)cell);
            Mask list = tm;
            for (int j = 0, n = nt; n < kWideList; ++j)
                if (!(tm.w[j >> 6] >> (j & 63) & 1ull)) {
                    list.set(j);
                    ++n;
                }
            each(list, [&](const int j) {
                ft.wide_idx.push_back((uint16_t)j);
                ft.wide.push_back(coord4[j]);
            });
            continue;
        }
        cls[cell] = (uint8_t)((kFineWindow - nt) * (kFineQuad + 1) + (kFineQuad - nn));
        ++class_count[cls[cell] + 1];
    }
    for (int c = 0; c < kClasses; ++c) class_count[c + 1] += class_count[c];
    std::vector<int> order(class_count[kClasses]);
    for (int cell = 0; cell < kFineCells; ++cell)
        if (cls[cell] != 0xff) order[class_count[cls[cell]]++] = cell;
    struct Win {
        Mask a, ab;
        int na, nb;
    };
    std::vector<Win> wins(1, Win{Mask{{0, 0, 0, 0}}, Mask{{0, 0, 0, 0}}, kFineQuad, kFineWindow - kFineQuad});
    std::vector<std::vector<int>> holds(K);
    constexpr int kSlots = 1 << 16;
    std::vector<int> seen(kSlots, 0);
    for (const int cell : order) {
        const Mask &nm = nms[cell], &tm = tms[cell];
        uint64_t h = 0x9e3779b97f4a7c15ull;
        for (int wi = 0; wi < 4; ++wi) h = (h ^ nm.w[wi]) * 0xff51afd7ed558ccdull, h = (h ^ (h >> 29) ^ tm.w[wi]) * 0xc4ceb9fe1a85ec53ull;
        int slot = (int)((h >> 40) & (kSlots - 1));
        bool met = false;
        for (; seen[slot] != 0; slot = (slot + 1) & (kSlots - 1))
            if (nms[seen[slot] - 1] == nm && tms[seen[slot] - 1] == tm) {
                ft.off[cell] = ft.off[seen[slot] - 1];
                met = true;
                break;
            }
        if (met) continue;
        seen[slot] = cell + 1;
        const Mask rest = tm.without(nm);
        int best = -1, best_cost = kFineWindow + 1;
        int rarest = -1;
        each(nm, [&](const int j) {
            if (rarest < 0 || holds[j].size() < holds[rarest].size()) rarest = j;
        });
        {
            for (const int wi : holds[rarest]) {
                const Win &w = wins[wi];
                const Mask need_a = nm.without(w.a), need_r = rest.without(w.ab);
                int c = 0;
                if (need_a.any() || need_r.any()) {
                    if (w.na + w.nb == kFineWindow || need_a.without(w.ab).w[0] != need_a.w[0] || need_a.without(w.ab).w[1] != need_a.w[1] ||
                        need_a.without(w.ab).w[2] != need_a.w[2] || need_a.without(w.ab).w[3] != need_a.w[3])
                        continue;
                    const int add_a = need_a.count();
                    if (w.na + add_a > kFineQuad) continue;
                    const int add_r = need_r.count();
                    if (add_r > (kFineQuad - w.na - add_a) + (kFineWindow - kFineQuad - w.nb)) continue;
                    c = add_a + add_r;
                }
                if (c < best_cost || (c == best_cost && wi < best)) {
                    best = wi;
                    best_cost = c;
                }
            }
        }
        if (best < 0) {
            if (wins.size() == 0xffffu || !fits((int)wins.size() + 1, ft.n_wide)) return;
            best = (int)wins.size();
            wins.push_back(Win{Mask{{0, 0, 0, 0}}, Mask{{0, 0, 0, 0}}, 0, 0});
        }
        Win &w = wins[best];
        each(nm.without(w.a), [&](const int j) {
            w.a.set(j);
            w.ab.set(j);
            ++w.na;
            holds[j].push_back(best);
        });
        each(rest.without(w.ab), [&](const int j) {
            w.ab.set(j);
            if (w.nb < kFineWindow - kFineQuad) {
                ++w.nb;
            } else {
                w.a.set(j);
                ++w.na;
                holds[j].push_back(best);
            }
        });
        ft.off[cell] = (uint16_t)best;
    }
    ft.n_win = (int)wins.size();
    ft.win_idx.assign((size_t)ft.n_win * kFineWindow, 0);
    for (int wi = 1; wi < ft.n_win; ++wi) {
        Win &w = wins[wi];
        for (int j = 0; w.na + w.nb < kFineWindow; ++j)
            if (!(w.ab.w[j >> 6] >> (j & 63) & 1ull)) {
                w.ab.set(j);
                if (w.na < kFineQuad) w.a.set(j), ++w.na;
                else ++w.nb;
            }
        uint16_t *e = &ft.win_idx[(size_t)wi * kFineWindow];
        int pa = 0, pb = kFineQuad;
        each(w.a, [&](const int j) { e[pa++] = (uint16_t)j; });
        each(w.ab.without(w.a), [&](const int j) { e[pb++] = (uint16_t)j; });
    }
    ft.quad.resize((size_t)ft.n_win * kFineQuad);
    ft.pair.resize((size_t)ft.n_win * (kFineWindow - kFineQuad));
    for (int wi = 0; wi < ft.n_win; ++wi)
        for (int p = 0; p < kFineWindow; ++p) {
            const uint32_t c = coord4[ft.win_idx[(size_t)wi * kFineWindow + p]];
            if (p < kFineQuad) ft.quad[(size_t)wi * kFineQuad + p] = c;
            else ft.pair[(size_t)wi * (kFineWindow - kFineQuad) + p - kFineQuad] = c;
        }
    ft.ok = true;
}


struct U4 {
    uint32_t x, y, z, w;
};
inline U4 make_u4(uint32_t x, uint32_t y, uint32_t z, uint32_t w) { return U4{x, y, z, w}; }

constexpr int kEdCells = 32 * 32 * 32;

template <class F>
inline void parallel_cells(const int n, F &&body, const int serial_below = 1024)
{
    unsigned nt = std::thread::hardware_concurrency();
    nt = nt < 1 ? 1 : (nt > 8 ? 8 : nt);
    if (n < serial_below || nt == 1) {
        body(0, n);
        return;
    }
    std::vector<std::thread> th;
    const int chunk = (n + (int)nt - 1) / (int)nt;
    for (unsigned t = 1; t < nt; ++t) {
        const int lo = (int)t * chunk, hi = std::min(n, lo + chunk);
        if (lo < hi) th.emplace_back([&body, lo, hi]() { body(lo, hi); });
    }
    body(0, std::min(n, chunk));
    for (auto &t : th) t.join();
}

struct EdTables {
    std::vector<U4> nodes;
    bool give_up = false;
    std::vector<U4> l16;
    std::vector<uint32_t> coarse;
    std::vector<uint32_t> ext;
    std::vector<U4> ext16;
    std::vector<U4> ext_nodes;
    std::vector<uint32_t> h4;
    size_t h4_wanted = 0;
    double h4_none = 0.0;
    double h4_depth = 0.0;
};
constexpr size_t kEdH4LdsWords = 27648;
constexpr size_t kEdH4MaxWords = 65536;
constexpr uint32_t kEdH4NoAnswer = 0xffff00ffu;

constexpr size_t kEdExtMaxNodes = 2048;
inline int ed_list_cap(const int K) { return K > 256 ? 12 : 15; }
inline int ed_list_get(const uint32_t (&w)[4], const int pos , const bool wide)
{
    if (!wide) return (int)((w[(pos + 1) >> 2] >> (8 * ((pos + 1) & 3))) & 255u);
    const int off = 8 + 10 * pos, wi = off >> 5, sh = off & 31;
    uint32_t v = w[wi] >> sh;
    if (sh > 22 && wi < 3) v |= w[wi + 1] << (32 - sh);
    return (int)(v & 1023u);
}
inline void ed_list_put(uint32_t (&w)[4], const int pos , const int j, const bool wide)
{
    if (!wide) {
        w[(pos + 1) >> 2] |= (uint32_t)j << (8 * ((pos + 1) & 3));
        return;
    }
    const int off = 8 + 10 * pos, wi = off >> 5, sh = off & 31;
    w[wi] |= (uint32_t)j << sh;
    if (sh > 22 && wi < 3) w[wi + 1] |= (uint32_t)j >> (32 - sh);
}

inline void ed_tables_refine(const double *pts, const int K, std::vector<U4> &host, EdTables &out, const int what = 1)
{
    const bool wide = K > 256;
    const int cap = ed_list_cap(K);
    std::vector<U4> &nodes = out.nodes;
    nodes.clear();
    auto box_list = [&](const std::vector<int> &from, const double lo[3], const double size, std::vector<int> &list) {
        double bound = std::numeric_limits<double>::infinity();
        for (int j : from) {
            double far2 = 0.0;
            for (int k = 0; k < 3; ++k) {
                const double c = pts[3 * j + k];
                const double m = std::max(std::fabs(c - lo[k]), std::fabs(c - (lo[k] + size)));
                far2 += m * m;
            }
            bound = std::min(bound, far2);
        }
        bound = bound * (1.0 + 1e-12) + 1e-9;
        list.clear();
        for (int j : from) {
            double near2 = 0.0;
            for (int k = 0; k < 3; ++k) {
                const double c = pts[3 * j + k];
                const double m = std::max(std::max(lo[k] - c, c - (lo[k] + size)), 0.0);
                near2 += m * m;
            }
            if (near2 <= bound) list.push_back(j);
        }
    };
    auto prune_list = [&](const double lo[3], const double size, std::vector<int> &list) {
        std::vector<int> keep;
        for (int j : list) {
            bool dominated = false;
            for (int k : list) {
                if (k == j) continue;
                double mx = 0.0;
                for (int d = 0; d < 3; ++d) {
                    const double a = 2.0 * (pts[3 * j + d] - pts[3 * k + d]);
                    mx += std::max(a * lo[d], a * (lo[d] + size));
                    mx += pts[3 * k + d] * pts[3 * k + d] - pts[3 * j + d] * pts[3 * j + d];
                }
                if (mx < -1e-9 * (1.0 + std::fabs(mx))) {
                    dominated = true;
                    break;
                }
            }
            if (!dominated) keep.push_back(j);
        }
        list.swap(keep);
    };
    int corner_entry[8];
    for (int c = 0; c < 8; ++c) {
        double best = std::numeric_limits<double>::infinity();
        corner_entry[c] = 0;
        for (int j = 0; j < K; ++j) {
            double d2 = 0.0;
            for (int d = 0; d < 3; ++d) {
                const double m = pts[3 * j + d] - ((c >> d) & 1 ? 255.0 : 0.0);
                d2 += m * m;
            }
            if (d2 < best) {
                best = d2;
                corner_entry[c] = j;
            }
        }
    }
    auto pack = [&](const std::vector<int> &list, const double *lo = nullptr, const double size = 0.0) {
        uint32_t w[4] = {(uint32_t)list.size(), 0u, 0u, 0u};
        for (size_t n = 1; n <= list.size(); ++n) ed_list_put(w, (int)n - 1, list[n - 1], wide);
        if (lo && !list.empty() && list.size() <= 12 && (int)list.size() < K) {
            const int oct = (lo[0] + 0.5 * size < 128.0 ? 1 : 0) | (lo[1] + 0.5 * size < 128.0 ? 2 : 0) | (lo[2] + 0.5 * size < 128.0 ? 4 : 0);
            int filler = corner_entry[oct];
            if (std::find(list.begin(), list.end(), filler) != list.end()) {
                filler = -1;
                double far_d = -1.0;
                for (int j = 0; j < K; ++j) {
                    if (std::find(list.begin(), list.end(), j) != list.end()) continue;
                    double d2 = 0.0;
                    for (int d = 0; d < 3; ++d) {
                        const double m = pts[3 * j + d] - (lo[d] + 0.5 * size);
                        d2 += m * m;
                    }
                    if (d2 > far_d) {
                        far_d = d2;
                        filler = j;
                    }
// ... 2130 lines not shown
```

dither_pie_amd/csrc/host_sanitize.cpp:

```cpp
#include <cstdio>
#include <cstdlib>
#include <cstring>
#include <string>

#include "host_logic.h"
#include "ordered_plan.h"
#include "ordered_fine.h"

using namespace dp;

static std::vector<double> read_pts(const char *path, int K)
{
    std::vector<double> p((size_t)K * 3);
    FILE *f = fopen(path, "rb");
    if (!f || fread(p.data(), sizeof(double), p.size(), f) != p.size()) {
        fprintf(stderr, "cannot read %d points from %s\n", K, path);
        exit(2);
    }
    fclose(f);
    return p;
}

static uint32_t lcg(uint32_t &s)
{
// ... 500 lines not shown
            return 2;
        }
        const size_t n = (size_t)head[0], stride = (size_t)head[1], pre_rows = head[6] ? n : 1;
        std::vector<int64_t> sizes(n), offsets(n + 1, -1);
        std::vector<uint8_t> streams(n * stride), pre(pre_rows * (size_t)head[5]), post((size_t)head[7]);
        std::vector<uint8_t> out(n * (size_t)png_file_bound(head[1], head[5], head[7]));
        if (fread(sizes.data(), sizeof(int64_t), n, f) != n || fread(streams.data(), 1, streams.size(), f) != streams.size() ||
            fread(pre.data(), 1, pre.size(), f) != pre.size() || fread(post.data(), 1, post.size(), f) != post.size()) {
            fprintf(stderr, "short record %d in %s\n", c, path);
            return 2;
        }
        const int64_t total = png_file_assemble(streams.data(), head[1], sizes.data(), head[0], head[2], (uint32_t)head[3], (uint32_t)head[4], pre.data(),
                                                head[6] ? head[5] : 0, head[5], post.data(), head[7], out.data(), offsets.data());
        if (total < 0 || (size_t)total > out.size() || offsets[n] != total) {
            printf("case %d: %lld bytes against a bound of %zu\n", c, (long long)total, out.size());
            return 1;
        }
        printf("file %d %lld ", c, (long long)total);
        for (int64_t i = 0; i < total; ++i) printf("%02x", out[(size_t)i]);
        printf("\n");
        uint32_t joined = crc32_bytes(nullptr, 0);
        for (size_t r = 0; r < n; ++r) {
            const size_t len = (size_t)png_file_clamp(sizes[r], head[1]);
            const uint32_t one = crc32_bytes(streams.data() + r * stride, len);
            joined = crc32_combine(joined, one, len);
            printf("crc %d %zu %08x %08x\n", c, r, one, joined);
        }
    }
    fclose(f);
    return 0;
}

static int run_orderedplan(const char *path, const int n_cases)
{
    FILE *f = fopen(path, "rb");
    if (!f) {
        fprintf(stderr, "cannot open %s\n", path);
        return 2;
    }
    for (int c = 0; c < n_cases; ++c) {
        OrderedFacts facts;
        OrderedSwitches sw;
        if (fread(&facts, sizeof(facts), 1, f) != 1 || fread(&sw, sizeof(sw), 1, f) != 1 || facts.hw < 1 || facts.w < 1 || facts.n_cus < 1) {
            fprintf(stderr, "bad record %d in %s\n", c, path);
            return 2;
        }
        const OrderedPlan p = plan_ordered(facts, sw);
        static const char *const tables[] = {"plain8", "plain4", "warped"};
        printf("plan %d %s %d %d %d %d %d %s %u %u %u %u %u %u %u %d %d %u\n", c, family_name(p.family), p.mode, p.bw, (int)p.adapt, (int)p.warp,
               (int)p.half, tables[p.table], p.grid, p.block, p.n_tiles, p.n_words, p.adv_y, p.adv_x, p.lds_bytes, p.fix_mode,
               (int)p.fix_big_queue, p.fix_grid);
    }
    fclose(f);
    return 0;
}

static void fine_masks(const std::vector<uint8_t> &pal, const int K, const int mw, std::vector<uint32_t> &tm, std::vector<uint32_t> &nm)
{
    tm.assign((size_t)kFineCells * mw, 0u);
    nm.assign((size_t)kFineCells * mw, 0u);
    parallel_cells(kFineCells, [&](const int lo, const int hi) {
        std::vector<int> cand, d;
        for (int cell = lo; cell < hi; ++cell) {
            const int c0[3] = {(cell & 31) * 8, ((cell >> 5) & 31) * 8, (cell >> 10) * 8};
            int u0 = 1 << 30, u1 = 1 << 30;
            std::vector<int> dmin(K);
            for (int j = 0; j < K; ++j) {
                int lo2 = 0, hi2 = 0;
                for (int k = 0; k < 3; ++k) {
                    const int p = pal[3 * j + k], a = c0[k], b = c0[k] + 7;
                    const int near = p < a ? a - p : (p > b ? p - b : 0), far = std::max(std::abs(p - a), std::abs(p - b));
                    lo2 += near * near;
                    hi2 += far * far;
                }
                dmin[j] = lo2;
                if (hi2 < u0) {
                    u1 = u0;
                    u0 = hi2;
                } else if (hi2 < u1) {
                    u1 = hi2;
                }
            }
            cand.clear();
            for (int j = 0; j < K; ++j)
                if (dmin[j] <= u1) cand.push_back(j);
            d.resize(cand.size());
            uint32_t *t = &tm[(size_t)cell * mw], *n = &nm[(size_t)cell * mw];
            for (int i = 0; i < 512; ++i) {
                const int r = c0[0] + (i & 7), g = c0[1] + ((i >> 3) & 7), b = c0[2] + (i >> 6);
                int d0 = 1 << 30, d1 = 1 << 30;
                for (size_t q = 0; q < cand.size(); ++q) {
                    const uint8_t *p = &pal[3 * (size_t)cand[q]];
                    d[q] = (r - p[0]) * (r - p[0]) + (g - p[1]) * (g - p[1]) + (b - p[2]) * (b - p[2]);
                    if (d[q] < d0) {
                        d1 = d0;
                        d0 = d[q];
                    } else if (d[q] < d1) {
                        d1 = d[q];
                    }
                }
                for (size_t q = 0; q < cand.size(); ++q) {
                    const int j = cand[q];
                    if (d[q] <= d1) t[j >> 5] |= 1u << (j & 31);
                    if (d[q] == d0) n[j >> 5] |= 1u << (j & 31);
                }
            }
        }
    });
}

static int run_finepack(const char *path, const int K, const char *out_path)
{
    if (K < 2 || K > 256) {
        fprintf(stderr, "finepack: 2 <= K <= 256\n");
        return 2;
    }
    std::vector<uint8_t> pal((size_t)K * 3);
    FILE *f = fopen(path, "rb");
    if (!f || fread(pal.data(), 1, pal.size(), f) != pal.size()) {
        fprintf(stderr, "cannot read %d colours from %s\n", K, path);
        return 2;
    }
    fclose(f);
    const int mw = 8;
    std::vector<uint32_t> coord4(K), tm, nm;
    for (int j = 0; j < K; ++j) coord4[j] = (uint32_t)pal[3 * j] | ((uint32_t)pal[3 * j + 1] << 8) | ((uint32_t)pal[3 * j + 2] << 16);
    fine_masks(pal, K, mw, tm, nm);
    FineTable ft, again;
    fine_pack(tm.data(), nm.data(), mw, K, coord4, fine_table_fits, ft);
    fine_pack(tm.data(), nm.data(), mw, K, coord4, fine_table_fits, again);
    const std::vector<uint32_t> im = ft.ok ? ft.lds_image() : std::vector<uint32_t>();
    int bad = ft.ok != again.ok || ft.off != again.off || ft.win_idx != again.win_idx || ft.wide_idx != again.wide_idx;
    if (ft.ok) bad += (int64_t)im.size() * 4 != fine_table_bytes(ft.n_win, ft.n_wide) || !fine_table_fits(ft.n_win, ft.n_wide);
    f = fopen(out_path, "wb");
    if (!f) return 2;
    const int32_t head[4] = {ft.ok ? 1 : 0, ft.n_win, ft.n_wide, (int32_t)im.size()};
    fwrite(head, sizeof(int32_t), 4, f);
    if (ft.ok) {
        fwrite(ft.off.data(), 2, ft.off.size(), f);
        fwrite(ft.win_idx.data(), 2, ft.win_idx.size(), f);
        fwrite(ft.wide_cell.data(), 2, ft.wide_cell.size(), f);
        fwrite(ft.wide_idx.data(), 2, ft.wide_idx.size(), f);
        fwrite(ft.quad.data(), 4, ft.quad.size(), f);
        fwrite(ft.pair.data(), 4, ft.pair.size(), f);
        fwrite(ft.wide.data(), 4, ft.wide.size(), f);
        fwrite(im.data(), 4, im.size(), f);
    }
    fclose(f);
    printf("finepack K=%d ok=%d windows=%d wide=%d bytes=%lld bad=%d\n", K, (int)ft.ok, ft.n_win, ft.n_wide,
           (long long)(ft.ok ? fine_table_bytes(ft.n_win, ft.n_wide) : 0), bad);
    return bad ? 1 : 0;
}

static int run_fineplan(const char *path, const int n_cases)
{
    FILE *f = fopen(path, "rb");
    if (!f) {
        fprintf(stderr, "cannot open %s\n", path);
        return 2;
    }
    for (int c = 0; c < n_cases; ++c) {
        OrderedFacts facts;
        OrderedSwitches sw;
        FineFacts ff;
        if (fread(&facts, sizeof(facts), 1, f) != 1 || fread(&sw, sizeof(sw), 1, f) != 1 || fread(&ff, sizeof(ff), 1, f) != 1 || facts.hw < 1 ||
            facts.w < 1 || facts.n_cus < 1) {
            fprintf(stderr, "bad record %d in %s\n", c, path);
            return 2;
        }
        const OrderedPlan p = plan_ordered(facts, sw);
        printf("fine %d %s %d\n", c, family_name(p.family), (int)fine_replaces(p, ff));
    }
    fclose(f);
    return 0;
}

static int run_finekeys(const char *path, const int n_cases)
{
    FILE *f = fopen(path, "rb");
    if (!f) {
        fprintf(stderr, "cannot open %s\n", path);
        return 2;
    }
    for (int c = 0; c < n_cases; ++c) {
        FineFacts ff;
        if (fread(&ff, sizeof(ff), 1, f) != 1 || ff.n_win < 0 || ff.thr_bytes < 0) {
            fprintf(stderr, "bad record %d in %s\n", c, path);
            fclose(f);
            return 2;
        }
        printf("keys %d %d\n", c, fine_keys_level(ff));
    }
    fclose(f);
    return 0;
}

static int run_voidcluster(const char *path, const int n_cases)
{
    FILE *f = fopen(path, "rb");
    if (!f) {
        fprintf(stderr, "cannot open %s\n", path);
        return 2;
    }
    for (int c = 0; c < n_cases; ++c) {
        int32_t head[4];
        if (fread(head, sizeof(int32_t), 4, f) != 4 || !vac_args_ok(head[0], head[1], head[3])) {
            fprintf(stderr, "bad record %d in %s\n", c, path);
            return 2;
        }
        const int n = head[0] * head[1];
        std::vector<uint16_t> ranks((size_t)n);
        std::vector<float> thr((size_t)n);
        int rounds = 0;
        vac_generate(head[0], head[1], (uint32_t)head[2], head[3], ranks.data(), &rounds);
        vac_thresholds(ranks.data(), n, thr.data());
        printf("ranks %d %d", c, rounds);
        for (int i = 0; i < n; ++i) printf(" %u", (unsigned)ranks[(size_t)i]);
        printf("\nthr %d", c);
        for (int i = 0; i < n; ++i) {
            uint32_t bits;
            std::memcpy(&bits, &thr[(size_t)i], sizeof(bits));
            printf(" %08x", bits);
        }
        printf("\n");
    }
    fclose(f);
    return 0;
}

static int run_metric(const char *path, const int n_cases)
{
    FILE *f = fopen(path, "rb");
    if (!f) {
        fprintf(stderr, "cannot open %s\n", path);
        return 2;
    }
    for (int c = 0; c < n_cases; ++c) {
        int32_t head[2];
        if (fread(head, sizeof(int32_t), 2, f) != 2 || head[0] < 1 || head[0] > 256 || head[1] < 0 || head[1] > (1 << 20)) {
            fprintf(stderr, "bad record %d in %s\n", c, path);
            return 2;
        }
        const int K = head[0], n = head[1];
        std::vector<float> pal((size_t)3 * K), thr((size_t)n);
        std::vector<uint8_t> rgb((size_t)3 * n);
        if (fread(pal.data(), sizeof(float), pal.size(), f) != pal.size() || fread(thr.data(), sizeof(float), thr.size(), f) != thr.size() ||
            fread(rgb.data(), 1, rgb.size(), f) != rgb.size() || !metric_palette_ok(pal.data(), K)) {
            fprintf(stderr, "bad record %d in %s\n", c, path);
            return 2;
        }
        std::vector<int32_t> lab((size_t)3 * n), coords((size_t)3 * K), d0((size_t)n), d1((size_t)n);
        std::vector<uint8_t> i0((size_t)n), i1((size_t)n);
        for (int i = 0; i < n; ++i) metric_lab(rgb[3 * (size_t)i], rgb[3 * (size_t)i + 1], rgb[3 * (size_t)i + 2], i & 1 ? metric_cbrt_table() : nullptr, &lab[3 * (size_t)i]);
        metric_palette_coords(pal.data(), K, 1, coords.data());
        metric_top2(rgb.data(), n, coords.data(), K, 1, i0.data(), i1.data(), d0.data(), d1.data());
        printf("lab %d", c);
        for (int i = 0; i < 3 * n; ++i) printf(" %d", lab[(size_t)i]);
        printf("\ntop %d", c);
        for (int i = 0; i < n; ++i) printf(" %u %u %d", (unsigned)i0[(size_t)i], (unsigned)i1[(size_t)i], (int)metric_takes_nearest(d0[(size_t)i], d1[(size_t)i], thr[(size_t)i]));
        printf("\n");
    }
    fclose(f);
    return 0;
}

static int run_idiffplan(const char *path, const int n_cases)
{
    FILE *f = fopen(path, "rb");
    if (!f) {
        fprintf(stderr, "cannot open %s\n", path);
        return 2;
    }
    for (int c = 0; c < n_cases; ++c) {
        int32_t head[3];
        if (fread(head, sizeof(int32_t), 3, f) != 3 || head[0] > 64) {
            fprintf(stderr, "bad record %d in %s\n", c, path);
            return 2;
        }
        const size_t n = head[0] > 0 ? (size_t)head[0] : 0;
        std::vector<int32_t> dx(n), dy(n), wt(n);
        if (fread(dx.data(), sizeof(int32_t), n, f) != n || fread(dy.data(), sizeof(int32_t), n, f) != n || fread(wt.data(), sizeof(int32_t), n, f) != n) {
            fprintf(stderr, "bad record %d in %s\n", c, path);
            return 2;
        }
        IdiffPlan p;
        const int rc = idiff_plan(dx.data(), dy.data(), wt.data(), head[0], head[1], head[2], p);
        printf("idiff %d %d %d %d", c, rc, p.n, p.skew);
        for (int k = 0; k < p.n; ++k) printf(" %u", (unsigned)p.q[k]);
        printf("\n");
    }
    fclose(f);
    return 0;
}

static int run_okfit(const char *path, const int n_cases)
{
    FILE *f = fopen(path, "rb");
    if (!f) {
        fprintf(stderr, "cannot open %s\n", path);
        return 2;
    }
    for (int c = 0; c < n_cases; ++c) {
        int32_t head[3];
        if (fread(head, sizeof(int32_t), 3, f) != 3 || head[0] < 0 || head[0] > (1 << 24)) {
            fprintf(stderr, "bad record %d in %s\n", c, path);
            return 2;
        }
        const size_t n = (size_t)head[0];
        std::vector<uint32_t> codes(n), counts(n);
        if (fread(codes.data(), sizeof(uint32_t), n, f) != n || fread(counts.data(), sizeof(uint32_t), n, f) != n) {
            fprintf(stderr, "bad record %d in %s\n", c, path);
            return 2;
        }
        const int K = head[1], rule = okfit_check(codes.data(), counts.data(), (int64_t)n, K, head[2]);
        printf("okfit %d %d", c, rule);
        if (!rule) {
            std::vector<uint8_t> pal((size_t)3 * K);
            std::vector<int32_t> centres((size_t)3 * K);
            int n_iter = 0;
            uint64_t distortion = 0;
            okfit_host(codes.data(), counts.data(), (int64_t)n, K, head[2], pal.data(), centres.data(), &n_iter, &distortion);
            printf(" %d %llu", n_iter, (unsigned long long)distortion);
            for (int i = 0; i < 3 * K; ++i) printf(" %u", (unsigned)pal[(size_t)i]);
            for (int i = 0; i < 3 * K; ++i) printf(" %d", centres[(size_t)i]);
        }
        printf("\n");
    }
    fclose(f);
    return 0;
}

static int run_resamplecoeffs(const char *path, const int n_cases)
{
    FILE *f = fopen(path, "rb");
    if (!f) {
        fprintf(stderr, "cannot open %s\n", path);
        return 2;
    }
    for (int c = 0; c < n_cases; ++c) {
        int32_t head[3];
        if (fread(head, sizeof(int32_t), 3, f) != 3 || head[0] < 1 || head[1] < 1 || head[0] > kResampleMaxSize || head[1] > kResampleMaxSize ||
            head[2] < 0 || head[2] >= kResampleFilters) {
            fprintf(stderr, "bad record %d in %s\n", c, path);
            return 2;
        }
        std::vector<int32_t> bounds, kk;
        const int ksize = resample_coeffs(head[0], head[1], head[2], bounds, kk);
        printf("coeffs %d %d", c, ksize);
        for (const int32_t v : bounds) printf(" %d", v);
        for (const int32_t v : kk) printf(" %d", v);
        printf("\n");
    }
    fclose(f);
    return 0;
}

static int run_resample(const char *path, const int n_cases, const char *out_path)
{
    FILE *f = fopen(path, "rb");
    FILE *g = fopen(out_path, "wb");
    if (!f || !g) {
        fprintf(stderr, "cannot open %s or %s\n", path, out_path);
        return 2;
    }
    for (int c = 0; c < n_cases; ++c) {
        int32_t head[6];
        if (fread(head, sizeof(int32_t), 6, f) != 6 || head[1] < 0 || head[1] > 64) {
            fprintf(stderr, "bad record %d in %s\n", c, path);
            return 2;
        }
        ResamplePlanHost p;
        const int rule = resample_plan(head[0], head[2], head[3], head[4], head[5], p);
        printf("resample %d %d", c, rule);
        if (!rule) {
            const size_t nin = (size_t)head[1] * 3u * (size_t)p.h * (size_t)p.w, nout = (size_t)head[1] * 3u * (size_t)p.oh * (size_t)p.ow;
            std::vector<uint8_t> in(nin), out(nout);
            if (fread(in.data(), 1, nin, f) != nin) {
                fprintf(stderr, "bad record %d in %s\n", c, path);
                return 2;
            }
            resample_host(p, in.data(), out.data(), head[1]);
            if (fwrite(out.data(), 1, nout, g) != nout) return 2;
            printf(" %d %d %d %d %d %d %lld %lld", p.y0, p.y1, p.need_h ? 1 : 0, p.need_v ? 1 : 0, p.mul32 ? 1 : 0, p.h_kernel,
                   (long long)std::max(p.ver.max_abs, p.hor.max_abs), (long long)std::max(p.need_v ? p.ver.max_sum : 0, p.hor.max_sum));
        }
        printf("\n");
    }
    fclose(f);
    fclose(g);
    return 0;
}

int main(int argc, char **argv)
{
    if (argc < 4) {
        fprintf(stderr, "usage: %s kdtree|edtables|accel <pts.f64> <K> [bw]  |  mediancut <rgb.u8> <n> <depth>  |  indexmap <lists.bin> <n>  |  giflzw <cases.bin> <n>  |  pngdeflate|pngdyn|pngfile <cases.bin> <n>  |  orderedplan <cases.bin> <n>  |  voidcluster <cases.bin> <n>  |  metric <cases.bin> <n>  |  finepack <pal.u8> <K> <out.bin>  |  fineplan <cases.bin> <n>  |  finekeys <cases.bin> <n>  |  idiffplan <cases.bin> <n>  |  okfit <cases.bin> <n>  |  resamplecoeffs <cases.bin> <n>  |  resample <cases.bin> <n> <out.bin>\n", argv[0]);
        return 2;
    }
    if (std::string(argv[1]) == "mediancut") return run_mediancut(argv[2], atol(argv[3]), argc > 4 ? atoi(argv[4]) : 4);
    if (std::string(argv[1]) == "indexmap") return run_indexmap(argv[2], atoi(argv[3]));
    if (std::string(argv[1]) == "giflzw") return run_giflzw(argv[2], atoi(argv[3]));
    if (std::string(argv[1]) == "pngdeflate") return run_pngdeflate(argv[2], atoi(argv[3]), false);
    if (std::string(argv[1]) == "pngdyn") return run_pngdeflate(argv[2], atoi(argv[3]), true);
    if (std::string(argv[1]) == "pngfile") return run_pngfile(argv[2], atoi(argv[3]));
    if (std::string(argv[1]) == "orderedplan") return run_orderedplan(argv[2], atoi(argv[3]));
    if (std::string(argv[1]) == "voidcluster") return run_voidcluster(argv[2], atoi(argv[3]));
    if (std::string(argv[1]) == "metric") return run_metric(argv[2], atoi(argv[3]));
    if (std::string(argv[1]) == "finepack") return argc > 4 ? run_finepack(argv[2], atoi(argv[3]), argv[4]) : 2;
    if (std::string(argv[1]) == "fineplan") return run_fineplan(argv[2], atoi(argv[3]));
    if (std::string(argv[1]) == "finekeys") return run_finekeys(argv[2], atoi(argv[3]));
    if (std::string(argv[1]) == "idiffplan") return run_idiffplan(argv[2], atoi(argv[3]));
    if (std::string(argv[1]) == "okfit") return run_okfit(argv[2], atoi(argv[3]));
    if (std::string(argv[1]) == "resamplecoeffs") return run_resamplecoeffs(argv[2], atoi(argv[3]));
    if (std::string(argv[1]) == "resample") return argc > 4 ? run_resample(argv[2], atoi(argv[3]), argv[4]) : 2;
    const int K = atoi(argv[3]);
    if (K < 1 || K > 1024) return 2;
    const std::vector<double> pts = read_pts(argv[2], K);
    const std::string cmd = argv[1];
    if (cmd == "kdtree") return run_kdtree(pts, K);
    if (cmd == "edtables") return run_edtables(pts, K);
    if (cmd == "accel") return run_accel(pts, K, argc > 4 ? atoi(argv[4]) : 8);
    return 2;
}
```

dither_pie_amd/csrc/ordered.hip:

```cpp
#include <type_traits>

#include "dp_internal.h"
#include "ordered_plan.h"
#include "ordered_fine.h"
#include "tree_query.hip.h"

namespace dp {

namespace {

constexpr int kListCap = 16384;
constexpr int kLdsTreeK = 256;
constexpr int kLdsTreeNodes = 512;
constexpr int kDrainAt = kListCap - kBlock * 64;

struct Geo {
    uint32_t n_px;
    uint32_t hw, w, h;
    double inv_hw, inv_w;
    int y0, x0;
    int ty0, tx0;
    int aligned;
    int neg2;
    uint32_t adv_y, adv_x;
// ... 1769 lines not shown
                                      int &m1, int &m2)
{
    int n0, n1, n2, n3, n4, n5, p0, p1, p2, p3, p4, p5;
    asm volatile(
        "v_dot4_u32_u8 %[n0], %[c0], %[c0], 0\n\t"
        "v_dot4_u32_u8 %[p0], %[x], %[c0], 0\n\t"
        "v_dot4_u32_u8 %[n1], %[c1], %[c1], 0\n\t"
        "v_dot4_u32_u8 %[p1], %[x], %[c1], 0\n\t"
        "v_dot4_u32_u8 %[n2], %[c2], %[c2], 0\n\t"
        "v_dot4_u32_u8 %[p2], %[x], %[c2], 0\n\t"
        "v_dot4_u32_u8 %[n3], %[c3], %[c3], 0\n\t"
        "v_dot4_u32_u8 %[p3], %[x], %[c3], 0\n\t"
        "v_dot4_u32_u8 %[n4], %[c4], %[c4], 0\n\t"
        "v_dot4_u32_u8 %[p4], %[x], %[c4], 0\n\t"
        "v_dot4_u32_u8 %[n5], %[c5], %[c5], 0\n\t"
        "v_dot4_u32_u8 %[p5], %[x], %[c5], 0\n\t"
        "v_lshl_add_u32 %[n0], %[n0], 8, 0\n\t"
        "v_lshl_add_u32 %[n1], %[n1], 8, 4\n\t"
        "v_lshl_add_u32 %[n2], %[n2], 8, 8\n\t"
        "v_lshl_add_u32 %[n3], %[n3], 8, 12\n\t"
        "v_lshl_add_u32 %[n4], %[n4], 8, 16\n\t"
        "v_lshl_add_u32 %[n5], %[n5], 8, 20\n\t"
        "v_mad_i32_i24 %[n0], %[p0], %[ng], %[n0]\n\t"
        "v_mad_i32_i24 %[n1], %[p1], %[ng], %[n1]\n\t"
        "v_mad_i32_i24 %[n2], %[p2], %[ng], %[n2]\n\t"
        "v_mad_i32_i24 %[n3], %[p3], %[ng], %[n3]\n\t"
        "v_mad_i32_i24 %[n4], %[p4], %[ng], %[n4]\n\t"
        "v_mad_i32_i24 %[n5], %[p5], %[ng], %[n5]\n\t"
        "v_min3_i32 %[m0], %[n0], %[n1], %[n2]\n\t"
        "v_med3_i32 %[m1], %[n0], %[n1], %[n2]\n\t"
        "v_max3_i32 %[m2], %[n0], %[n1], %[n2]\n\t"
        "v_med3_i32 %[m2], %[m1], %[m2], %[n3]\n\t"
        "v_med3_i32 %[m1], %[m0], %[m1], %[n3]\n\t"
        "v_min_i32 %[m0], %[m0], %[n3]\n\t"
        "v_med3_i32 %[m2], %[m1], %[m2], %[n4]\n\t"
        "v_med3_i32 %[m1], %[m0], %[m1], %[n4]\n\t"
        "v_min_i32 %[m0], %[m0], %[n4]\n\t"
        "v_med3_i32 %[m2], %[m1], %[m2], %[n5]\n\t"
        "v_med3_i32 %[m1], %[m0], %[m1], %[n5]\n\t"
        "v_min_i32 %[m0], %[m0], %[n5]\n\t"
        : [n0] "=&v"(n0), [n1] "=&v"(n1), [n2] "=&v"(n2), [n3] "=&v"(n3), [n4] "=&v"(n4), [n5] "=&v"(n5), [p0] "=&v"(p0),
          [p1] "=&v"(p1), [p2] "=&v"(p2), [p3] "=&v"(p3), [p4] "=&v"(p4), [p5] "=&v"(p5), [m0] "=&v"(m0), [m1] "=&v"(m1),
          [m2] "=&v"(m2)
        : [x] "v"(x), [c0] "v"(ca.x), [c1] "v"(ca.y), [c2] "v"(ca.z), [c3] "v"(ca.w), [c4] "v"(c4), [c5] "v"(c5),
          [ng] "s"(neg2));
}

__device__ __forceinline__ void cand4k(const uint32_t x, const uint4 ca, const uint4 na, const int neg2, int &m0, int &m1)
{
    int n0, n1, n2, n3, p0, p1, p2, p3;
    asm volatile(
        "v_dot4_u32_u8 %[p0], %[x], %[c0], 0\n\t"
        "v_dot4_u32_u8 %[p1], %[x], %[c1], 0\n\t"
        "v_dot4_u32_u8 %[p2], %[x], %[c2], 0\n\t"
        "v_dot4_u32_u8 %[p3], %[x], %[c3], 0\n\t"
        "v_mad_i32_i24 %[n0], %[p0], %[ng], %[k0]\n\t"
        "v_mad_i32_i24 %[n1], %[p1], %[ng], %[k1]\n\t"
        "v_mad_i32_i24 %[n2], %[p2], %[ng], %[k2]\n\t"
        "v_mad_i32_i24 %[n3], %[p3], %[ng], %[k3]\n\t"
        "v_min3_i32 %[m0], %[n0], %[n1], %[n2]\n\t"
        "v_med3_i32 %[m1], %[n0], %[n1], %[n2]\n\t"
        "v_med3_i32 %[m1], %[m0], %[m1], %[n3]\n\t"
        "v_min_i32 %[m0], %[m0], %[n3]\n\t"
        : [n0] "=&v"(n0), [n1] "=&v"(n1), [n2] "=&v"(n2), [n3] "=&v"(n3), [p0] "=&v"(p0), [p1] "=&v"(p1), [p2] "=&v"(p2),
          [p3] "=&v"(p3), [m0] "=&v"(m0), [m1] "=&v"(m1)
        : [x] "v"(x), [c0] "v"(ca.x), [c1] "v"(ca.y), [c2] "v"(ca.z), [c3] "v"(ca.w), [k0] "v"(na.x), [k1] "v"(na.y), [k2] "v"(na.z),
          [k3] "v"(na.w), [ng] "s"(neg2));
}

template <int KEYS>
__device__ __forceinline__ void cand6k(const uint32_t x, const uint4 ca, const uint4 na, const uint32_t c4, const uint32_t c5,
                                       const uint32_t k4, const uint32_t k5, const int neg2, int &m0, int &m1, int &m2)
{
    int n0, n1, n2, n3, n4, n5, p0, p1, p2, p3, p4, p5;
    if constexpr (KEYS == 1) {
        (void)k4, (void)k5;
        asm volatile(
            "v_dot4_u32_u8 %[p0], %[x], %[c0], 0\n\t"
            "v_dot4_u32_u8 %[p1], %[x], %[c1], 0\n\t"
            "v_dot4_u32_u8 %[p2], %[x], %[c2], 0\n\t"
            "v_dot4_u32_u8 %[p3], %[x], %[c3], 0\n\t"
            "v_dot4_u32_u8 %[n4], %[c4], %[c4], 0\n\t"
            "v_dot4_u32_u8 %[p4], %[x], %[c4], 0\n\t"
            "v_dot4_u32_u8 %[n5], %[c5], %[c5], 0\n\t"
            "v_dot4_u32_u8 %[p5], %[x], %[c5], 0\n\t"
            "v_mad_i32_i24 %[n0], %[p0], %[ng], %[k0]\n\t"
            "v_mad_i32_i24 %[n1], %[p1], %[ng], %[k1]\n\t"
            "v_mad_i32_i24 %[n2], %[p2], %[ng], %[k2]\n\t"
            "v_mad_i32_i24 %[n3], %[p3], %[ng], %[k3]\n\t"
            "v_lshl_add_u32 %[n4], %[n4], 8, 16\n\t"
            "v_lshl_add_u32 %[n5], %[n5], 8, 20\n\t"
            "v_mad_i32_i24 %[n4], %[p4], %[ng], %[n4]\n\t"
            "v_mad_i32_i24 %[n5], %[p5], %[ng], %[n5]\n\t"
            "v_min3_i32 %[m0], %[n0], %[n1], %[n2]\n\t"
            "v_med3_i32 %[m1], %[n0], %[n1], %[n2]\n\t"
            "v_max3_i32 %[m2], %[n0], %[n1], %[n2]\n\t"
            "v_med3_i32 %[m2], %[m1], %[m2], %[n3]\n\t"
            "v_med3_i32 %[m1], %[m0], %[m1], %[n3]\n\t"
            "v_min_i32 %[m0], %[m0], %[n3]\n\t"
            "v_med3_i32 %[m2], %[m1], %[m2], %[n4]\n\t"
            "v_med3_i32 %[m1], %[m0], %[m1], %[n4]\n\t"
            "v_min_i32 %[m0], %[m0], %[n4]\n\t"
            "v_med3_i32 %[m2], %[m1], %[m2], %[n5]\n\t"
            "v_med3_i32 %[m1], %[m0], %[m1], %[n5]\n\t"
            "v_min_i32 %[m0], %[m0], %[n5]\n\t"
            : [n0] "=&v"(n0), [n1] "=&v"(n1), [n2] "=&v"(n2), [n3] "=&v"(n3), [n4] "=&v"(n4), [n5] "=&v"(n5), [p0] "=&v"(p0),
              [p1] "=&v"(p1), [p2] "=&v"(p2), [p3] "=&v"(p3), [p4] "=&v"(p4), [p5] "=&v"(p5), [m0] "=&v"(m0), [m1] "=&v"(m1),
              [m2] "=&v"(m2)
            : [x] "v"(x), [c0] "v"(ca.x), [c1] "v"(ca.y), [c2] "v"(ca.z), [c3] "v"(ca.w), [c4] "v"(c4), [c5] "v"(c5), [k0] "v"(na.x),
              [k1] "v"(na.y), [k2] "v"(na.z), [k3] "v"(na.w), [ng] "s"(neg2));
    } else {
        asm volatile(
            "v_dot4_u32_u8 %[p0], %[x], %[c0], 0\n\t"
            "v_dot4_u32_u8 %[p1], %[x], %[c1], 0\n\t"
            "v_dot4_u32_u8 %[p2], %[x], %[c2], 0\n\t"
            "v_dot4_u32_u8 %[p3], %[x], %[c3], 0\n\t"
            "v_dot4_u32_u8 %[p4], %[x], %[c4], 0\n\t"
            "v_dot4_u32_u8 %[p5], %[x], %[c5], 0\n\t"
            "v_mad_i32_i24 %[n0], %[p0], %[ng], %[k0]\n\t"
            "v_mad_i32_i24 %[n1], %[p1], %[ng], %[k1]\n\t"
            "v_mad_i32_i24 %[n2], %[p2], %[ng], %[k2]\n\t"
            "v_mad_i32_i24 %[n3], %[p3], %[ng], %[k3]\n\t"
            "v_mad_i32_i24 %[n4], %[p4], %[ng], %[k4]\n\t"
            "v_mad_i32_i24 %[n5], %[p5], %[ng], %[k5]\n\t"
            "v_min3_i32 %[m0], %[n0], %[n1], %[n2]\n\t"
            "v_med3_i32 %[m1], %[n0], %[n1], %[n2]\n\t"
            "v_max3_i32 %[m2], %[n0], %[n1], %[n2]\n\t"
            "v_med3_i32 %[m2], %[m1], %[m2], %[n3]\n\t"
            "v_med3_i32 %[m1], %[m0], %[m1], %[n3]\n\t"
            "v_min_i32 %[m0], %[m0], %[n3]\n\t"
            "v_med3_i32 %[m2], %[m1], %[m2], %[n4]\n\t"
            "v_med3_i32 %[m1], %[m0], %[m1], %[n4]\n\t"
            "v_min_i32 %[m0], %[m0], %[n4]\n\t"
            "v_med3_i32 %[m2], %[m1], %[m2], %[n5]\n\t"
            "v_med3_i32 %[m1], %[m0], %[m1], %[n5]\n\t"
            "v_min_i32 %[m0], %[m0], %[n5]\n\t"
            : [n0] "=&v"(n0), [n1] "=&v"(n1), [n2] "=&v"(n2), [n3] "=&v"(n3), [n4] "=&v"(n4), [n5] "=&v"(n5), [p0] "=&v"(p0),
              [p1] "=&v"(p1), [p2] "=&v"(p2), [p3] "=&v"(p3), [p4] "=&v"(p4), [p5] "=&v"(p5), [m0] "=&v"(m0), [m1] "=&v"(m1),
              [m2] "=&v"(m2)
            : [x] "v"(x), [c0] "v"(ca.x), [c1] "v"(ca.y), [c2] "v"(ca.z), [c3] "v"(ca.w), [c4] "v"(c4), [c5] "v"(c5), [k0] "v"(na.x),
              [k1] "v"(na.y), [k2] "v"(na.z), [k3] "v"(na.w), [k4] "v"(k4), [k5] "v"(k5), [ng] "s"(neg2));
    }
}

__device__ __forceinline__ uint32_t fine_cell_offset(const uint32_t x)
{
    return ((x >> 2) & 0x3eu) | ((x >> 5) & 0x7c0u) | ((x >> 8) & 0xf800u);
}

struct FineLds {
    uint32_t wide_at, norm_at, pair_at, off_at, ids_at, thr_at;
};

template <int MODE, int KEYS>
__device__ __forceinline__ uint32_t fine_pixel_full(const uint32_t entry, const uint8_t *__restrict__ in, uint8_t *__restrict__ out,
                                                    unsigned long long *__restrict__ flags, const Geo &g, const PalDev &pal,
                                                    const ThrDev &thr, const uint32_t *s_words, const FineLds &at)
{
    const uint32_t mask = entry & 15u;
    const uint32_t p = (entry >> 4) * 4u + (uint32_t)__builtin_ctz(mask | 16u);
    const uint8_t *s_bytes = reinterpret_cast<const uint8_t *>(s_words);
    const uint8_t *b = in + (size_t)p * 3;
    const uint32_t x = (uint32_t)b[0] | ((uint32_t)b[1] << 8) | ((uint32_t)b[2] << 16);
    LeanThr th;
    pixel_threshold<MODE>(p, g, thr, s_words + at.thr_at / 4, 0.0f, 0.0f, 0.0f, th);
    const uint32_t cell2 = fine_cell_offset(x);
    uint32_t c = 0;
    bool done = false, slow = false;
    if (*reinterpret_cast<const uint16_t *>(s_bytes + at.off_at + cell2) == 0) {
        const uint16_t *ids = reinterpret_cast<const uint16_t *>(s_bytes + at.ids_at);
        const uint32_t cell = cell2 >> 1;
        uint32_t lo = 0;
#pragma unroll
        for (uint32_t step = kFineIds / 2; step != 0u; step >>= 1)
            if ((uint32_t)ids[lo + step] <= cell) lo += step;
        if constexpr (KEYS == 0) done = resolve_wide<MODE>(x, th, thr.sh, s_words + at.wide_at / 4 + lo * kWideList, kWideList, c);
        else done = resolve_wide<MODE>(x, th, thr.sh, pal.fine_tab + (uint32_t)pal.fine_win * kFineQuad + lo * kWideList, kWideList, c);
    }
    if (!done) {
        bool hard;
        Leaf lf;
        leaf_find_global<8>(x, pal, lf);
        c = resolve_pixel<MODE, 8>(x, th, lf, g, pal, thr, nullptr, slow, hard);
    }
    uint8_t *o = out + (size_t)p * 3;
    o[0] = (uint8_t)c;
    o[1] = (uint8_t)(c >> 8);
    o[2] = (uint8_t)(c >> 16);
    if (slow) flag_slow_pixel(p, flags, g);
    const uint32_t rest = mask & (mask - 1u);
    return rest ? ((entry & ~15u) | rest) : 0u;
}

template <int MODE, int KEYS>
__global__ __launch_bounds__(kCellBlock, 4) void ordered_fine_kernel(const uint8_t *__restrict__ in, uint8_t *__restrict__ out,
                                                                    unsigned long long *__restrict__ flags, const Geo g,
                                                                    const PalDev pal, const ThrDev thr, const float sx, const float sy,
                                                                    const float sc, const uint32_t n_tiles)
{
    static_assert(MODE == 1, "integer thresholds in LDS only");
    (void)sx, (void)sy, (void)sc;
    static_assert(KEYS >= 0 && KEYS <= 2, "key levels: ordered_fine.h");
    __shared__ __align__(16) uint32_t smem[kLeanLdsWords];
    FineLds at;
    if constexpr (KEYS == 0) {
        for (int i = threadIdx.x * 2; i < pal.fine_words; i += kCellBlock * 2)
            *reinterpret_cast<uint2 *>(&smem[i]) = *reinterpret_cast<const uint2 *>(&pal.fine_tab[i]);
        at.wide_at = (uint32_t)pal.fine_win * (kFineQuad * 4);
        at.norm_at = 0;
        at.pair_at = at.wide_at + (uint32_t)pal.fine_wide * (kWideList * 4);
        at.off_at = at.pair_at + (uint32_t)pal.fine_win * ((kFineWindow - kFineQuad) * 4);
    } else {
        constexpr int kPairRec = KEYS == 2 ? 4 : 2;
        const int n_win = pal.fine_win;
        const int pair_src = n_win * kFineQuad + pal.fine_wide * kWideList;
        const int tail_src = pair_src + n_win * (kFineWindow - kFineQuad);
        at.wide_at = 0;
        at.norm_at = (uint32_t)n_win * (kFineQuad * 4);
        at.pair_at = 2 * at.norm_at;
        at.off_at = at.pair_at + (uint32_t)n_win * (kPairRec * 4);
        for (int wi = threadIdx.x; wi < n_win; wi += kCellBlock) {
            const uint4 c = *reinterpret_cast<const uint4 *>(&pal.fine_tab[wi * kFineQuad]);
            *reinterpret_cast<uint4 *>(&smem[wi * 4]) = c;
            *reinterpret_cast<uint4 *>(&smem[n_win * 4 + wi * 4]) =
                make_uint4((__builtin_amdgcn_udot4(c.x, c.x, 0u, false) << kLocalBits), (__builtin_amdgcn_udot4(c.y, c.y, 0u, false) << kLocalBits) + 4u,
                           (__builtin_amdgcn_udot4(c.z, c.z, 0u, false) << kLocalBits) + 8u, (__builtin_amdgcn_udot4(c.w, c.w, 0u, false) << kLocalBits) + 12u);
            const uint2 b = *reinterpret_cast<const uint2 *>(&pal.fine_tab[pair_src + wi * 2]);
            if constexpr (KEYS == 2)
                *reinterpret_cast<uint4 *>(&smem[n_win * 8 + wi * 4]) =
                    make_uint4(b.x, b.y, (__builtin_amdgcn_udot4(b.x, b.x, 0u, false) << kLocalBits) + 16u,
                               (__builtin_amdgcn_udot4(b.y, b.y, 0u, false) << kLocalBits) + 20u);
            else
                *reinterpret_cast<uint2 *>(&smem[n_win * 8 + wi * 2]) = b;
        }
        uint32_t *s_tail = smem + at.off_at / 4;
        for (int i = threadIdx.x * 2; i < (kFineCells + kFineIds) / 2; i += kCellBlock * 2)
            *reinterpret_cast<uint2 *>(&s_tail[i]) = *reinterpret_cast<const uint2 *>(&pal.fine_tab[tail_src + i]);
    }
    at.ids_at = at.off_at + kFineCells * 2;
    at.thr_at = at.ids_at + kFineIds * 2;
    {
        const int n = thr.th_h * thr.tw_pad;
        const int thr_word = KEYS == 0 ? pal.fine_words : (int)(at.thr_at / 4);
        for (int i = threadIdx.x; i < n; i += kCellBlock) smem[thr_word + i] = thr.mpad[i];
    }
    __syncthreads();
    const uint8_t *s_bytes = reinterpret_cast<const uint8_t *>(smem);
    const uint32_t lane = threadIdx.x & 63u;
    uint32_t *s_queue = smem + (kLeanLdsWords - kLeanQueueWords) + (threadIdx.x >> 6) * kLeanQueue;
    uint32_t qcount = 0;
    const uint3 *in3 = reinterpret_cast<const uint3 *>(in);
    uint3 *out3 = reinterpret_cast<uint3 *>(out);
    const uint32_t n_full = g.n_px >> 2;

    auto windows = [&](const uint32_t xq[4], uint32_t win[4]) {
#pragma unroll
        for (int q = 0; q < 4; ++q) win[q] = *reinterpret_cast<const uint16_t *>(s_bytes + at.off_at + fine_cell_offset(xq[q]));
    };
    auto drain = [&](const uint32_t n) {
        qcount -= n;
        __threadfence_block();
        uint32_t rest = 0u;
        if (lane < n) rest = fine_pixel_full<MODE, KEYS>(s_queue[qcount + lane], in, out, flags, g, pal, thr, smem, at);
        queue_push(s_queue, qcount, rest != 0u, rest);
    };

    uint32_t tile = blockIdx.x;
    uint32_t fy = 0, fx = 0;
    uint3 wn = make_uint3(0u, 0u, 0u), wnn = make_uint3(0u, 0u, 0u);
    uint32_t xn[4], winn[4];
    if (tile < n_tiles) {
        const uint32_t gidx0 = tile * kCellBlock + threadIdx.x;
        if (gidx0 < n_full) wn = in3[gidx0];
        if (gidx0 * 4u < g.n_px) locate(g, gidx0 * 4u, fy, fx);
        const uint32_t gidx1 = gidx0 + gridDim.x * kCellBlock;
        if (tile + gridDim.x < n_tiles && gidx1 < n_full) wnn = in3[gidx1];
    }
    unpack4(wn, xn);
    windows(xn, winn);
    const bool use_cls = thr.has_cls != 0;
    uint32_t cls_word = 0, cls_shift = 0;
    auto tile_class = [&](const uint32_t ty, const uint32_t tx, const uint32_t gi) {
        cls_word = 0;
        cls_shift = 0;
        if (!use_cls) return;
        const uint32_t y0l = (uint32_t)__builtin_amdgcn_readfirstlane((int)ty), x0l = (uint32_t)__builtin_amdgcn_readfirstlane((int)tx);
        const uint32_t g0 = (uint32_t)__builtin_amdgcn_readfirstlane((int)gi);
        if (x0l + 256u > g.w || g0 + 64u > n_full) return;
        const uint32_t row = ((uint32_t)g.y0 + y0l) & (uint32_t)(thr.th_h - 1), col = ((uint32_t)g.x0 + x0l) & (uint32_t)(thr.th_w - 1);
        const uint32_t idx = row * (uint32_t)thr.th_w + col;
        cls_word = thr.cls_nib[idx >> 3];
        cls_shift = (idx & 7u) * 4u;
    };
    if (tile < n_tiles) tile_class(fy, fx, tile * kCellBlock + threadIdx.x);
    for (; tile < n_tiles; tile += gridDim.x) {
        const uint32_t gidx = tile * kCellBlock + threadIdx.x;
        uint32_t xq[4], win[4];
#pragma unroll
        for (int q = 0; q < 4; ++q) {
            xq[q] = xn[q];
            win[q] = winn[q];
        }
        const uint32_t cls = (cls_word >> cls_shift) & 15u;
        const uint32_t cy = fy, cx = fx;
        {
            unpack4(wnn, xn);
            windows(xn, winn);
            const uint32_t next = tile + gridDim.x, next2 = next + gridDim.x;
            const uint32_t gn = next * kCellBlock + threadIdx.x, gn2 = next2 * kCellBlock + threadIdx.x;
            wnn = make_uint3(0u, 0u, 0u);
            if (next2 < n_tiles && gn2 < n_full) wnn = in3[gn2];
            tile_advance(g, fy, fx);
            cls_word = 0;
            if (next < n_tiles) tile_class(fy, fx, gn);
        }
        clear_flags(flags, gidx, lane);
        bool rare[4] = {false, false, false, false};
        if (gidx < n_full) {
            constexpr int kPairShift = KEYS == 2 ? 4 : 3;
            uint4 ca[4], na[4];
#pragma unroll
            for (int q = 0; q < 4; ++q) {
                ca[q] = *reinterpret_cast<const uint4 *>(s_bytes + (win[q] << 4));
                if constexpr (KEYS != 0) na[q] = *reinterpret_cast<const uint4 *>(s_bytes + ((win[q] << 4) + at.norm_at));
            }
            auto body = [&](auto cls_c) {
                constexpr uint32_t CLS = (uint32_t)decltype(cls_c)::value;
                uint32_t pb[4];
                uint2 cb[4], nb[4];
#pragma unroll
                for (int q = 0; q < 4; ++q) {
                    if ((CLS >> q) & 1u) continue;
                    pb[q] = (win[q] << kPairShift) + (at.pair_at - 16u);
                    if constexpr (KEYS == 2) {
                        const uint4 v = *reinterpret_cast<const uint4 *>(s_bytes + pb[q] + 16u);
                        cb[q] = make_uint2(v.x, v.y);
                        nb[q] = make_uint2(v.z, v.w);
                    } else {
                        cb[q] = *reinterpret_cast<const uint2 *>(s_bytes + pb[q] + 16u);
                        nb[q] = make_uint2(0u, 0u);
                    }
                }
                LeanThr th[4];
#pragma unroll
                for (int q = 0; q < 4; ++q) {
                    th[q].mt = 0;
                    th[q].t = 0.0f;
                }
                if (CLS != 15u) {
                    uint32_t row, col;
                    thr_pos(thr, (uint32_t)g.y0 + cy, (uint32_t)g.x0 + cx, row, col);
                    const uint32_t ta = row * (uint32_t)thr.tw_pad + col;
#pragma unroll
                    for (int q = 0; q < 4; ++q) {
                        if ((CLS >> q) & 1u) continue;
                        th[q].mt = *reinterpret_cast<const uint32_t *>(s_bytes + at.thr_at + (ta + q) * 4u);
                    }
                }
                const bool straddle = cx + 3u >= g.w;
                uint32_t col[4];
#pragma unroll
                for (int q = 0; q < 4; ++q) {
                    const uint32_t x = xq[q];
                    if ((CLS >> q) & 1u) {
                        int m0, m1;
                        if constexpr (KEYS == 0) cand4n(x, ca[q], g.neg2, m0, m1);
                        else cand4k(x, ca[q], na[q], g.neg2, m0, m1);
                        rare[q] = ((uint32_t)(m0 ^ m1) < (1u << kLocalBits)) | straddle;
                        col[q] = *reinterpret_cast<const uint32_t *>(s_bytes + ((win[q] << 4) | ((uint32_t)m0 & 0xfcu)));
                    } else {
                        int m0, m1, m2;
                        if constexpr (KEYS == 0) cand6(x, ca[q], cb[q].x, cb[q].y, g.neg2, m0, m1, m2);
                        else cand6k<KEYS>(x, ca[q], na[q], cb[q].x, cb[q].y, nb[q].x, nb[q].y, g.neg2, m0, m1, m2);
                        const int a0 = m0 >> kLocalBits, a1 = m1 >> kLocalBits;
                        const bool tie = (a0 == a1) | ((uint32_t)(m1 ^ m2) < (1u << kLocalBits));
                        const int xx = (int)__builtin_amdgcn_udot4(x, x, 0u, false);
                        const uint32_t d0 = (uint32_t)(a0 + xx);
                        const uint32_t S = d0 + (uint32_t)a1 + (uint32_t)xx;
                        bool eq;
                        const bool nearest = lean_decide<MODE>(d0, S, th[q], thr.sh, eq);
                        rare[q] = tie | eq | straddle;
                        const uint32_t pos = (uint32_t)(nearest ? m0 : m1) & 0xfcu;
                        col[q] = *reinterpret_cast<const uint32_t *>(s_bytes + ((pos < 16u ? (win[q] << 4) : pb[q]) + pos));
                    }
                }
                out3[gidx] = pack4(col);
            };
            if (cls == 5u) body(std::integral_constant<int, 5>{});
            else if (cls == 10u) body(std::integral_constant<int, 10>{});
            else if (cls == 15u) body(std::integral_constant<int, 15>{});
            else body(std::integral_constant<int, 0>{});
        } else {
#pragma unroll
            for (int q = 0; q < 4; ++q) rare[q] = gidx * 4u + (uint32_t)q < g.n_px;
        }
        const uint32_t rmask = (rare[0] ? 1u : 0u) | (rare[1] ? 2u : 0u) | (rare[2] ? 4u : 0u) | (rare[3] ? 8u : 0u);
        const unsigned long long rb = __ballot(rmask != 0u);
        if (rb != 0ull) {
            if (rmask != 0u)
                s_queue[__builtin_amdgcn_mbcnt_hi((uint32_t)(rb >> 32), __builtin_amdgcn_mbcnt_lo((uint32_t)rb, qcount))] = (gidx << 4) | rmask;
            qcount += (uint32_t)__popcll(rb);
            while (qcount >= 64u) drain(64u);
        }
    }
    while (qcount != 0u) drain(qcount < 64u ? qcount : 64u);
}

constexpr int kFloatKeyGap = 128;

struct alignas(16) Cand3 {
    float x, y, z;
};

__device__ __forceinline__ int med3_i32(const int a, const int b, const int c)
{
    int r;
    asm("v_med3_i32 %0, %1, %2, %3" : "=v"(r) : "v"(a), "v"(b), "v"(c));
    return r;
}

template <int MODE>
__global__ __launch_bounds__(kCellBlock) void ordered_lean_float_kernel(const uint8_t *__restrict__ in,
                                                                        uint8_t *__restrict__ out,
                                                                        unsigned long long *__restrict__ flags,
                                                                        const Geo g, const PalDev pal, const ThrDev thr,
                                                                        const float sx, const float sy, const float sc,
                                                                        const uint32_t n_tiles)
{
    __shared__ __align__(16) uint32_t smem[kLeanLdsWords];
    const uint32_t cand_base = (uint32_t)pal.ftab_words * 4u;
    for (int i = threadIdx.x * 4; i < pal.ftab_words; i += kCellBlock * 4) {
        uint4 v = *reinterpret_cast<const uint4 *>(&pal.ftab[i]);
        v.x += (v.x >> 31) ? 0u : cand_base;
        v.y += (v.y >> 31) ? 0u : cand_base;
        v.z += (v.z >> 31) ? 0u : cand_base;
        v.w += (v.w >> 31) ? 0u : cand_base;
        *reinterpret_cast<uint4 *>(&smem[i]) = v;
    }
    const uint32_t lut_base = cand_base + (uint32_t)pal.K * 16u;
    for (int i = threadIdx.x; i < pal.K; i += kCellBlock)
        *reinterpret_cast<float4 *>(&smem[pal.ftab_words + 4 * i]) = pal.fcand[i];
    if (threadIdx.x < 256)
        reinterpret_cast<uint8_t *>(smem)[lut_base + threadIdx.x] = pal.lut_in ? pal.lut_in[threadIdx.x] : (uint8_t)threadIdx.x;
    __syncthreads();
    const uint8_t *s_bytes = reinterpret_cast<const uint8_t *>(smem);
    const uint8_t *s_lut = s_bytes + lut_base;
    const uint32_t lane = threadIdx.x & 63u;
    const uint3 *in3 = reinterpret_cast<const uint3 *>(in);
    uint3 *out3 = reinterpret_cast<uint3 *>(out);
    const uint32_t n_full = g.n_px >> 2;

    uint32_t tile = blockIdx.x;
    uint32_t fy = 0, fx = 0;
    uint3 wn = make_uint3(0u, 0u, 0u);
    if (tile < n_tiles) {
        const uint32_t gidx0 = tile * kCellBlock + threadIdx.x;
        if (gidx0 < n_full) wn = in3[gidx0];
        if (gidx0 * 4u < g.n_px) locate(g, gidx0 * 4u, fy, fx);
    }
    for (; tile < n_tiles; tile += gridDim.x) {
        const uint32_t gidx = tile * kCellBlock + threadIdx.x;
        const uint3 wc = wn;
        {
            const uint32_t next = tile + gridDim.x;
            const uint32_t gn = next * kCellBlock + threadIdx.x;
            if (next < n_tiles && gn < n_full) wn = in3[gn];
        }
        bool slow[4] = {false, false, false, false};
        if (gidx < n_full) {
            uint32_t xs[4];
            unpack4(wc, xs);
            float tq[4] = {0.0f, 0.0f, 0.0f, 0.0f};
            if (MODE == 2) {
                uint32_t row, col;
                thr_pos(thr, (uint32_t)g.y0 + fy, (uint32_t)g.x0 + fx, row, col);
                const uint32_t at = row * (uint32_t)thr.tw_pad + col;
#pragma unroll
                for (int q = 0; q < 4; ++q) tq[q] = thr.fpad[at + q];
            } else if (MODE == 3) {
#pragma unroll
                for (int q = 0; q < 4; ++q) tq[q] = ign_threshold(g.x0 + (int)fx + q, g.y0 + (int)fy, sx, sy, sc);
            }
            const bool straddle = (MODE != 0) && (fx + 3u >= g.w);
            uint32_t col[4];
#pragma unroll
            for (int q = 0; q < 4; ++q) {
                const uint32_t r = s_lut[xs[q] & 255u], gg = s_lut[(xs[q] >> 8) & 255u], b = s_lut[xs[q] >> 16];
                const uint32_t x = r | (gg << 8) | (b << 16);
                uint32_t blk = cell_offset(x);
                uint4 ca = *reinterpret_cast<const uint4 *>(s_bytes + blk);
                bool s = straddle;
                bool from_global = false;
                for (int bit = 3; (ca.x >> 31) != 0; --bit) {
                    if ((ca.x & 0x40000000u) || bit < 0) {
                        s = true;
                        ca = make_uint4(cand_base, cand_base, cand_base, cand_base);
                        from_global = false;
                        blk = 0u;
                        break;
                    }
                    const uint32_t sub = (((x >> bit) & 1u) << 2) | (((x >> (8 + bit)) & 1u) << 1) | ((x >> (16 + bit)) & 1u);
                    blk = (4096u * 8u + ((ca.x & 0xffffffu) * 8u + sub) * 8u) * 4u;
                    from_global = blk >= cand_base;
                    ca = from_global ? *reinterpret_cast<const uint4 *>(reinterpret_cast<const uint8_t *>(pal.ftab) + blk)
                                     : *reinterpret_cast<const uint4 *>(s_bytes + blk);
                }
                uint4 cb;
                if (from_global) {
                    cb = *reinterpret_cast<const uint4 *>(reinterpret_cast<const uint8_t *>(pal.ftab) + blk + 16);
                    ca.x += cand_base;
                    ca.y += cand_base;
                    ca.z += cand_base;
                    ca.w += cand_base;
                    cb.x += cand_base;
                    cb.y += cand_base;
                    cb.z += cand_base;
                    cb.w += cand_base;
                } else {
                    cb = *reinterpret_cast<const uint4 *>(s_bytes + blk + 16);
                    if (s && (ca.x == cand_base)) cb = ca;
                }
                const uint32_t off[8] = {ca.x, ca.y, ca.z, ca.w, cb.x, cb.y, cb.z, cb.w};
                const float fr = (float)r, fg = (float)gg, fb = (float)b;
                int key[8];
#pragma unroll
                for (int c = 0; c < 8; ++c) {
                    const float4 cc = *reinterpret_cast<const float4 *>(s_bytes + off[c]);
                    const float dx = cc.x - fr, dy = cc.y - fg, dz = cc.z - fb;
                    const float d = fmaf(dz, dz, fmaf(dy, dy, dx * dx));
                    key[c] = (int)((__float_as_uint(d) & ~7u) | (uint32_t)c);
                }
                int m0 = min(min(key[0], key[1]), key[2]);
                int m1 = med3_i32(key[0], key[1], key[2]);
                int m2 = max(max(key[0], key[1]), key[2]);
#pragma unroll
                for (int c = 3; c < 8; ++c) {
                    m2 = med3_i32(m1, m2, key[c]);
                    m1 = med3_i32(m0, m1, key[c]);
                    m0 = min(m0, key[c]);
                }
                s |= (m1 - m0) <= kFloatKeyGap;
                uint32_t o0 = off[0], o1 = off[0];
#pragma unroll
                for (int c = 1; c < 8; ++c) {
                    o0 = ((uint32_t)m0 & 7u) == (uint32_t)c ? off[c] : o0;
                    o1 = ((uint32_t)m1 & 7u) == (uint32_t)c ? off[c] : o1;
                }
                const uint32_t a0 = s ? cand_base : o0;
// ... 357 lines not shown
    if (threadIdx.x == 0) s_count = 0;
    __syncthreads();

    auto drain = [&]() {
        const uint32_t n = s_count;
        for (uint32_t i = threadIdx.x; i < n; i += kBlock) {
            const uint32_t p = s_list[i];
            const uint8_t *b = in + (size_t)p * 3;
            uint32_t c0 = b[0], c1 = b[1], c2 = b[2];
            if (pal.lut_in) {
                c0 = pal.lut_in[c0];
                c1 = pal.lut_in[c1];
                c2 = pal.lut_in[c2];
            }
            double d2[2];
            int ii[2];
            int pick;
            if (MODE == 0) {
                tree_query<1, CAP>(pal, (double)c0, (double)c1, (double)c2, d2, ii);
                pick = ii[0];
            } else {
                tree_query<2, CAP>(pal, (double)c0, (double)c1, (double)c2, d2, ii);
                uint32_t y, x;
                locate(g, p, y, x);
                float t;
                if (MODE == 3)
                    t = ign_threshold(g.x0 + (int)x, g.y0 + (int)y, sx, sy, sc);
                else
                    t = thr.f32[(((uint32_t)g.y0 + y) % (uint32_t)thr.th_h) * thr.th_w +
                                (((uint32_t)g.x0 + x) % (uint32_t)thr.th_w)];
                pick = ordered_use_nearest(d2[0], d2[1], t) ? ii[0] : ii[1];
                if (pick >= pal.K) pick = ii[0];
            }
            const uint32_t c = pal.out_rgb[pick];
            uint8_t *o = out + (size_t)p * 3;
            o[0] = (uint8_t)c;
            o[1] = (uint8_t)(c >> 8);
            o[2] = (uint8_t)(c >> 16);
        }
        __syncthreads();
        if (threadIdx.x == 0) s_count = 0;
        __syncthreads();
    };

    if (n_dirty <= (uint32_t)kQueueTiles) {
        for (uint32_t base = blockIdx.x * 64u; base < n_dirty; base += gridDim.x * 64u) {
            const uint32_t e = base + (threadIdx.x >> 2), q = threadIdx.x & 3u;
            unsigned long long wd = 0;
            uint32_t tile = 0;
            if (e < n_dirty) {
                tile = g.dirty[1 + e];
                wd = flags[(size_t)tile * 4 + q];
            }
            if (wd) {
                const int n = __popcll(wd);
                uint32_t pos = atomicAdd(&s_count, (uint32_t)n);
                while (wd) {
                    const int lane = __ffsll((long long)wd) - 1;
                    wd &= wd - 1;
                    s_list[pos++] = ((tile * 64u + (uint32_t)lane) << 2) + q;
                }
            }
            __syncthreads();
            if (s_count > (uint32_t)kDrainAt) drain();
        }
        drain();
        return;
    }
    constexpr int kWordsPerIter = 8;
    for (uint32_t base = blockIdx.x * kBlock * kWordsPerIter; base < n_words; base += gridDim.x * kBlock * kWordsPerIter) {
        unsigned long long word[kWordsPerIter];
        unsigned long long any = 0;
#pragma unroll
        for (int k = 0; k < kWordsPerIter; ++k) {
            const uint32_t wi = base + k * kBlock + threadIdx.x;
            word[k] = (wi < n_words) ? flags[wi] : 0ull;
            any |= word[k];
        }
        if (!__syncthreads_or(any != 0ull)) continue;
#pragma unroll
        for (int k = 0; k < kWordsPerIter; ++k) {
            const uint32_t wi = base + k * kBlock + threadIdx.x;
            unsigned long long wd = word[k];
            if (wd) {
                const int n = __popcll(wd);
                uint32_t pos = atomicAdd(&s_count, (uint32_t)n);
                const uint32_t tile = wi >> 2, q = wi & 3u;
                while (wd) {
                    const int lane = __ffsll((long long)wd) - 1;
                    wd &= wd - 1;
                    s_list[pos++] = ((tile * 64u + (uint32_t)lane) << 2) + q;
                }
            }
            __syncthreads();
            if (s_count > (uint32_t)kDrainAt) drain();
        }
    }
    drain();
}

__global__ void ign_field_kernel(float *__restrict__ out, const int h, const int w, const int y0, const int x0,
                                 const float sx, const float sy, const float sc)
{
    const int x = blockIdx.x * blockDim.x + threadIdx.x;
    const int y = blockIdx.y;
    if (x < w && y < h) out[(size_t)y * w + x] = ign_threshold(x0 + x, y0 + y, sx, sy, sc);
}

__global__ void resize_tables_kernel(int *__restrict__ xtab, int *__restrict__ ytab, const int w, const int ow,
                                     const int h, const int oh)
{
    const int which = threadIdx.x;
    if (which > 1) return;
    const int n_in = which ? h : w, n_out = which ? oh : ow;
    int *tab = which ? ytab : xtab;
    const double a = (double)n_in / (double)n_out;
    double xo = __dmul_rn(a, 0.5);
    for (int x = 0; x < n_out; ++x) {
        int v = (int)xo;
        tab[x] = v < n_in ? v : n_in - 1;
        xo = __dadd_rn(xo, a);
    }
}

__global__ void resize_nearest_kernel(const uint8_t *__restrict__ in, uint8_t *__restrict__ out, const int h,
                                      const int w, const int oh, const int ow, const int *__restrict__ xtab,
                                      const int *__restrict__ ytab)
{
    const int x = blockIdx.x * blockDim.x + threadIdx.x;
    const int y = blockIdx.y;
    const size_t f = blockIdx.z;
    if (x >= ow || y >= oh) return;
    const uint8_t *s = in + (f * h * w + (size_t)ytab[y] * w + xtab[x]) * 3;
    uint8_t *d = out + (f * oh * ow + (size_t)y * ow + x) * 3;
    d[0] = s[0];
    d[1] = s[1];
    d[2] = s[2];
}

int num_cus()
{
    static thread_local int cached_dev = -1, cached = 0;
    int dev = 0;
    if (hipGetDevice(&dev) != hipSuccess) return 256;
    if (dev != cached_dev) {
        int n = 0;
        if (hipDeviceGetAttribute(&n, hipDeviceAttributeMultiprocessorCount, dev) != hipSuccess || n <= 0) n = 256;
        cached = n;
        cached_dev = dev;
    }
    return cached;
}

static inline void trace_plan(const OrderedPlan &p, bool aligned, bool fine, int keys)
{
#ifdef DP_EXPERIMENTS
    if (std::getenv("DP_ORDERED_TRACE")) {
        constexpr const char *tables[] = {"plain8", "plain4", "warped"};
        char keys_s[16] = "";
        if (fine) snprintf(keys_s, sizeof(keys_s), " keys=%d", keys);
        fprintf(stderr, "dp_ordered_u8: pass 1 = %s (4-byte aligned frames: %d) mode=%d bw=%d adapt=%d warp=%d half=%d table=%s fix_big_queue=%d kernel=%s%s\n",
                family_name(p.family), aligned ? 1 : 0, p.mode, p.bw, p.adapt ? 1 : 0, p.warp ? 1 : 0, p.half ? 1 : 0, tables[p.table],
                p.fix_big_queue ? 1 : 0, fine ? "fine" : family_name(p.family), keys_s);
    }
#else
    (void)p;
    (void)aligned;
    (void)fine;
    (void)keys;
#endif
}

using TileKernel = void (*)(const uint8_t *, uint8_t *, unsigned long long *, Geo, PalDev, ThrDev, float, float, float, uint32_t);
using BruteKernel = void (*)(const uint8_t *, uint8_t *, unsigned long long *, Geo, PalDev, ThrDev, float, float, float);
using FixKernel = void (*)(const uint8_t *, uint8_t *, const unsigned long long *, uint32_t, Geo, PalDev, ThrDev, float, float, float);

template <int M>
TileKernel tile_kernel_of(const OrderedPlan &p)
{
    switch (p.family) {
    case kFamCell:
        return ordered_cell_kernel<M>;
    case kFamFast:
        if (p.bw == 4) return ordered_fast_kernel<M, 4>;
        return ordered_fast_kernel<M, 8>;
    case kFamLean:
        if (p.warp && p.bw == 4) return ordered_lean_kernel<M, 4, false, true>;
        if (p.warp && p.adapt) return ordered_lean_kernel<M, 8, true, true>;
        if (p.warp) return ordered_lean_kernel<M, 8, false, true>;
        if (p.bw == 4 && p.half) return ordered_lean_kernel<M, 4, false, false, true>;
        if (p.bw == 4) return ordered_lean_kernel<M, 4, false, false>;
        if (p.adapt) return ordered_lean_kernel<M, 8, true, false>;
        return ordered_lean_kernel<M, 8, false, false>;
    case kFamCompact:
        if (p.warp && p.half) return ordered_compact_kernel<M, true, true>;
        if (p.warp) return ordered_compact_kernel<M, true, false>;
        if (p.half) return ordered_compact_kernel<M, false, true>;
        return ordered_compact_kernel<M, false, false>;
    case kFamLeanFloat:
        if constexpr (M != 1) return ordered_lean_float_kernel<M>;
        break;
    case kFamCompactFloat:
        if constexpr (M != 1) return ordered_compact_float_kernel<M>;
        break;
    case kFamBrute:
        break;
    }
    return nullptr;
}

TileKernel tile_kernel(const OrderedPlan &p)
{
    switch (p.mode) {
    case 0: return tile_kernel_of<0>(p);
    case 1: return tile_kernel_of<1>(p);
    case 2: return tile_kernel_of<2>(p);
    case 3: return tile_kernel_of<3>(p);
    }
    return nullptr;
}

TileKernel fine_kernel(const int keys)
{
    switch (keys) {
    case 0: return ordered_fine_kernel<1, 0>;
    case 1: return ordered_fine_kernel<1, 1>;
#ifdef DP_EXPERIMENTS
    case 2: return ordered_fine_kernel<1, 2>;
#endif
    }
    return nullptr;
}

BruteKernel brute_kernel(const OrderedPlan &p, const bool integer)
{
    switch (p.mode) {
    case 0: return integer ? ordered_int_kernel<0> : ordered_f64_kernel<0>;
    case 1: return integer ? ordered_int_kernel<1> : ordered_f64_kernel<1>;
    case 2: return integer ? ordered_int_kernel<2> : ordered_f64_kernel<2>;
    case 3: return integer ? ordered_int_kernel<3> : ordered_f64_kernel<3>;
    }
    return nullptr;
}

FixKernel fix_kernel(const OrderedPlan &p)
{
    const bool big = p.fix_big_queue;
    switch (p.fix_mode) {
    case 0: return big ? fixup_kernel<0, kQueueLarge> : fixup_kernel<0, kQueueSmall>;
    case 2: return big ? fixup_kernel<2, kQueueLarge> : fixup_kernel<2, kQueueSmall>;
    case 3: return big ? fixup_kernel<3, kQueueLarge> : fixup_kernel<3, kQueueSmall>;
    }
    return nullptr;
}

OrderedFacts facts_of(const PalDev &pal, const ThrDev &thr, const Geo &g, const int mode)
{
    return OrderedFacts{mode, pal.K, pal.is_integer, pal.n_inner,
                        g.n_px, g.hw, g.w,
                        g.y0, g.x0, g.aligned,
                        pal.cell_tab != nullptr, pal.tab_words, pal.tab_total,
                        pal.cell_tab4 != nullptr, pal.tab4_words,
                        pal.warp_tab != nullptr, pal.warp_words, pal.warp_total, pal.warp_bw, pal.warp_adapt,
                        pal.adapt, pal.cell_perm != nullptr, pal.cell_perm4 != nullptr, pal.n_wide, pal.n_wide4,
                        pal.comp_tab != nullptr, pal.comp_words, pal.comp_warp,
                        pal.ftab != nullptr, pal.ftab_words,
                        thr.m != nullptr, thr.mpad != nullptr, thr.fpad != nullptr, thr.th_h, thr.th_w, thr.tw_pad,
                        num_cus()};
}

}

int launch_ordered(const uint8_t *in, uint8_t *out, int64_t n_frames, int h, int w, int y0, int x0,
                   const PalDev &pal, int mode, const ThrDev *thr_in, float ign_scale, int ign_seed, void *ws,
                   size_t ws_bytes, hipStream_t s)
{
    (void)ws_bytes;
    const ThrDev thr = mode == DP_MODE_MATRIX ? *thr_in : no_thresholds();
    OrderedSwitches sw;
    sw.lean_no_half = exp_env("DP_LEAN_NO_HALF") != nullptr;
    sw.fast_all = exp_env("DP_FAST_ALL") != nullptr;
    sw.force_compact = exp_env("DP_FORCE_COMPACT") != nullptr;
    sw.no_compact_kernel = exp_env("DP_NO_COMPACT_KERNEL") != nullptr;
    sw.compact_no_half = exp_env("DP_COMPACT_NO_HALF") != nullptr;

    const float sx = (float)((double)ign_seed * 0.37), sy = (float)((double)ign_seed * 0.73);
    const int64_t hw = (int64_t)h * w;
    const int64_t max_frames = std::max<int64_t>(1, ((int64_t)1 << 30) / hw - 1);
    unsigned long long *fl = reinterpret_cast<unsigned long long *>(ws);
    const size_t dirty_off = ((size_t)((std::min(max_frames, n_frames) * hw + 255) / 256) * 32 + 768) & ~size_t(7);

    for (int64_t f0 = 0; f0 < n_frames; f0 += max_frames) {
        const int64_t nf = std::min(max_frames, n_frames - f0);
        const uint8_t *in_c = in + (size_t)f0 * hw * 3;
        uint8_t *out_c = out + (size_t)f0 * hw * 3;
        Geo g;
        g.n_px = (uint32_t)(nf * hw);
        g.hw = (uint32_t)hw;
        g.w = (uint32_t)w;
        g.h = (uint32_t)h;
        g.inv_hw = 1.0 / (double)hw;
        g.inv_w = 1.0 / (double)w;
        g.y0 = y0;
        g.x0 = x0;
        g.ty0 = y0 % thr.th_h;
        g.tx0 = x0 % thr.th_w;
        g.aligned = (((uintptr_t)in_c | (uintptr_t)out_c) & 3) == 0;
        g.neg2 = -(2 << kLocalBits);
        g.dirty = reinterpret_cast<uint32_t *>(reinterpret_cast<uint8_t *>(ws) + dirty_off);
        const OrderedPlan plan = plan_ordered(facts_of(pal, thr, g, mode), sw);
        g.adv_y = plan.adv_y;
        g.adv_x = plan.adv_x;
        const bool brute = plan.family == kFamBrute;
        const FineFacts fine_facts{pal.fine_tab != nullptr, pal.fine_win, pal.fine_wide, thr.th_h * thr.tw_pad * 4};
        const bool fine = fine_replaces(plan, fine_facts) && !exp_env("DP_NO_FINE_KERNEL");
        int keys_cap = kFineKeysShipped;
        if (const char *cap = exp_env("DP_FINE_KEYS_MAX")) keys_cap = std::min(2, std::max(0, std::atoi(cap)));
        const int fine_keys = fine ? std::min(fine_keys_level(fine_facts), keys_cap) : 0;
        const BruteKernel brute_k = brute ? brute_kernel(plan, pal.is_integer != 0) : nullptr;
        const TileKernel tile_k = brute ? nullptr : (fine ? fine_kernel(fine_keys) : tile_kernel(plan));
        const FixKernel fix_k = fix_kernel(plan);
        if ((brute ? brute_k == nullptr : tile_k == nullptr) || fix_k == nullptr) {
            set_error("dp_ordered_u8: no %s kernel for mode %d", family_name(plan.family), plan.mode);
            return DP_EUNSUPPORTED;
        }
        DP_HIP(hipMemsetAsync(g.dirty, 0, sizeof(uint32_t), s));
        ProfMark *pm = prof_begin(s);
        if (brute) {
            hipLaunchKernelGGL(brute_k, dim3(plan.grid), dim3(plan.block), 0, s, in_c, out_c, fl, g, pal, thr, sx, sy, ign_scale);
        } else {
            if (plan.family == kFamCell)
                DP_HIP(hipFuncSetAttribute(reinterpret_cast<const void *>(tile_k), hipFuncAttributeMaxDynamicSharedMemorySize, (int)plan.lds_bytes));
            PalDev pal1 = pal;
            if (plan.table == kTabWarped) {
                pal1.cell_tab = pal.warp_tab;
                pal1.tab_words = pal.warp_words;
                pal1.tab_total = pal.warp_total;
            } else if (plan.table == kTabPlain4) {
                pal1.cell_tab = pal.cell_tab4;
                pal1.tab_words = pal.tab4_words;
                pal1.tab_total = pal.tab4_words;
            }
            hipLaunchKernelGGL(tile_k, dim3(plan.grid), dim3(plan.block), plan.lds_bytes, s, in_c, out_c, fl, g, pal1, thr, sx, sy, ign_scale,
                               plan.n_tiles);
        }
        DP_HIP(hipGetLastError());
        trace_plan(plan, g.aligned, fine, fine_keys);
        prof_mid(pm, s);
        hipLaunchKernelGGL(fix_k, dim3(plan.fix_grid), dim3(kBlock), 0, s, in_c, out_c, fl, plan.n_words, g, pal, thr, sx, sy, ign_scale);
        prof_end(pm, s);
        DP_HIP(hipGetLastError());
    }
    return DP_OK;
}

int launch_ign_thresholds(float *out, int h, int w, int y0, int x0, float scale, int seed, hipStream_t s)
{
    const float sx = (float)((double)seed * 0.37), sy = (float)((double)seed * 0.73);
    if (h > 65535) {
        set_error("dp_ign_thresholds: h > 65535 not supported");
        return DP_EUNSUPPORTED;
    }
    hipLaunchKernelGGL(ign_field_kernel, dim3((w + 255) / 256, h), dim3(256), 0, s, out, h, w, y0, x0, sx, sy, scale);
    DP_HIP(hipGetLastError());
    return DP_OK;
}

int launch_resize_nearest(const uint8_t *in, uint8_t *out, int64_t n_frames, int h, int w, int oh, int ow,
                          hipStream_t s)
{
    if (oh > 65535 || n_frames > 65535) {
        set_error("dp_resize_nearest_u8: oh or n_frames > 65535 not supported");
        return DP_EUNSUPPORTED;
    }
    int *tabs = nullptr;
    DP_HIP(hipMallocAsync((void **)&tabs, sizeof(int) * ((size_t)ow + oh), s));
    hipLaunchKernelGGL(resize_tables_kernel, dim3(1), dim3(64), 0, s, tabs, tabs + ow, w, ow, h, oh);
    hipLaunchKernelGGL(resize_nearest_kernel, dim3((ow + 255) / 256, oh, (unsigned)n_frames), dim3(256), 0, s, in, out,
                       h, w, oh, ow, tabs, tabs + ow);
    hipError_t e = hipGetLastError();
    (void)hipFreeAsync(tabs, s);
    if (e != hipSuccess) return hip_fail(e, "resize launch");
    return DP_OK;
}

}
```

dither_pie_amd/csrc/ordered_fine.h:

```cpp
#pragma once
#include <cstdint>

#include "ordered_plan.h"

namespace dp {

constexpr int64_t fine_table_bytes(const int n_win, const int n_wide)
{
    return (int64_t)n_win * (kFineWindow * 4) + (int64_t)n_wide * kWideList * 4 + kFineCells * 2 + kFineIds * 2;
}
constexpr bool fine_table_fits(const int n_win, const int n_wide)
{
    return fine_table_bytes(n_win, n_wide) + 16 * 19 * 4 <= kLeanTabBytes;
}

struct FineFacts {
    int32_t present;
    int32_t n_win, n_wide;
    int32_t thr_bytes;
};

inline bool fine_replaces(const OrderedPlan &p, const FineFacts &f)
{
    return f.present != 0 && p.family == kFamLean && p.mode == 1 && p.bw == 8 && p.table == kTabPlain8 && !p.adapt && !p.warp && !p.half &&
           fine_table_bytes(f.n_win, f.n_wide) + (int64_t)f.thr_bytes <= kLeanTabBytes;
}

constexpr int64_t fine_keys_bytes(const int level, const int n_win)
{
    return (int64_t)n_win * (level == 2 ? 48 : 40) + kFineCells * 2 + kFineIds * 2;
}
inline int fine_keys_level(const FineFacts &f)
{
    if (f.present == 0) return 0;
    for (int level = 2; level >= 1; --level)
        if (fine_keys_bytes(level, f.n_win) + (int64_t)f.thr_bytes <= kLeanTabBytes) return level;
    return 0;
}

constexpr int kFineKeysShipped = 1;

}
```

Measured before the change: 415,500 Mpixel/s.

## Add two-level fine palette table splitting wide cells into 4-unit sub-cells

Adds a second, two-level fine lookup table. Cells whose candidate lists are too wide are subdivided into eight 4x4x4 sub-cells, each mapped to its own small window, so fewer pixels fall back to the slow wide-list path. The kernel gains a SUB template variant that resolves tagged cell entries through a per-sub-cell row in LDS. The host builds this table first by default and delays the plain fine table until a threshold size no longer fits. The cost is extra host build work, a larger device blob, and one additional dependent LDS lookup for tagged cells.

```diff
diff --git a/dither_pie_amd/csrc/accel.hip b/dither_pie_amd/csrc/accel.hip
--- a/dither_pie_amd/csrc/accel.hip
+++ b/dither_pie_amd/csrc/accel.hip
@@ -372,7 +372,7 @@
     const int mw = K <= 256 ? 8 : 32;
     const bool big_q = dev.n_inner > kQueueSmall;
     const size_t bytes = sizeof(uint32_t) * (3 * kCodeWords + 2 * kTabMaxWords + kTabCapWords) + sizeof(uint4) * kExcCap + 16 + 768 +
-                         sizeof(uint32_t) * (2 * kCells + 2 * kWideCap * kWideList + kCompactMaxWords) + kLeanTabBytes;
+                         sizeof(uint32_t) * (2 * kCells + 2 * kWideCap * kWideList + kCompactMaxWords) + 2 * kLeanTabBytes;
     DP_HIP(hipMalloc((void **)&blob, bytes));
     struct DevFree {
         void *p = nullptr;
@@ -628,6 +628,8 @@
     }
     dev.fine_tab = nullptr;
     dev.fine_words = dev.fine_win = dev.fine_wide = 0;
+    dev.fsub_tab = nullptr;
+    dev.fsub_win = dev.fsub_wide = 0;
     if (have8 && !st.too_big && !use4 && wbw == 0 && !dev.adapt && mw == 8 && K >= kWideList && !exp_env("DP_NO_FINE")) {
         fine_masks->resize((size_t)2 * kFineCells * mw);
         uint32_t *ftm = fine_masks->data(), *fnm = ftm + (size_t)kFineCells * mw;
@@ -693,10 +695,25 @@
     return DP_OK;
 }
 
-int build_fine(PalDev &dev, const std::vector<uint32_t> &p4_host, const std::vector<uint32_t> &fine_masks, uint32_t *fine_dev)
+int build_fine(PalDev &dev, const std::vector<uint32_t> &p4_host, const std::vector<uint32_t> &fine_masks, uint32_t *fine_dev, const bool sub)
 {
     constexpr int mw = 8;
     FineTable ft;
+    if (sub) {
+        fine_pack_sub(fine_masks.data(), fine_masks.data() + (size_t)kFineCells * mw, mw, dev.K, p4_host, fine_sub_fits, ft);
+        if (exp_env("DP_DEBUG_ACCEL"))
+            fprintf(stderr, "accel K=%d: two-level fine table: %s, %d windows, %d wide cells, %zu sub-cells still wide, %lld bytes\n", dev.K,
+                    ft.ok ? "yes" : "no", ft.n_win, ft.n_wide, ft.sub_wide.size(), (long long)fine_sub_bytes(ft.n_win, ft.n_wide));
+        if (!ft.ok) return DP_OK;
+        const std::vector<uint32_t> im = ft.sub_image();
+        uint32_t *at = fine_dev + kLeanTabBytes / 4;
+        const hipError_t e = hipMemcpy(at, im.data(), sizeof(uint32_t) * im.size(), hipMemcpyHostToDevice);
+        if (e != hipSuccess) return hip_fail(e, "accelerator upload (two-level fine table)");
+        dev.fsub_tab = at;
+        dev.fsub_win = ft.n_win;
+        dev.fsub_wide = ft.n_wide;
+        return DP_OK;
+    }
     fine_pack(fine_masks.data(), fine_masks.data() + (size_t)kFineCells * mw, mw, dev.K, p4_host, fine_table_fits, ft);
     if (exp_env("DP_DEBUG_ACCEL"))
         fprintf(stderr, "accel K=%d: fine table: %s, %d windows, %d wide cells, %lld bytes\n", dev.K, ft.ok ? "yes" : "no", ft.n_win, ft.n_wide,
diff --git a/dither_pie_amd/csrc/dp_internal.h b/dither_pie_amd/csrc/dp_internal.h
--- a/dither_pie_amd/csrc/dp_internal.h
+++ b/dither_pie_amd/csrc/dp_internal.h
@@ -29,6 +29,11 @@
     return nullptr;
 #endif
 }
+#ifdef DP_EXPERIMENTS
+constexpr bool kExperiments = true;
+#else
+constexpr bool kExperiments = false;
+#endif
 int hip_fail(hipError_t e, const char *what);
 
 inline void trace_diffusion(const char *kernel, const char *schedule, int G, long long grid, int waves, size_t lds, int K, int n_inner,
@@ -87,6 +92,8 @@
     const uint32_t *fine_tab;
     int fine_words;
     int fine_win, fine_wide;
+    const uint32_t *fsub_tab;
+    int fsub_win, fsub_wide;
     int n_split;
     int n_slow_blocks;
     int n_split_cells;
@@ -177,6 +184,8 @@
     std::vector<uint32_t> fine_masks;
     uint32_t *fine_dev;
     std::atomic<bool> fine_pending;
+    std::atomic<bool> fine_plain_pending;
+    std::atomic<int> fine_sub_room;
     int metric;
     dp::MetDev met;
     void *met_blob;
@@ -203,7 +212,7 @@
 namespace dp {
 int build_accel(PalDev &dev, const std::vector<uint32_t> &p4_host, void **blob_out, size_t *blob_bytes, std::vector<uint32_t> *fine_masks,
                 uint32_t **fine_dev);
-int build_fine(PalDev &dev, const std::vector<uint32_t> &p4_host, const std::vector<uint32_t> &fine_masks, uint32_t *fine_dev);
+int build_fine(PalDev &dev, const std::vector<uint32_t> &p4_host, const std::vector<uint32_t> &fine_masks, uint32_t *fine_dev, bool sub);
 int build_accel_float(PalDev &dev, const float *pal_f32, const uint8_t *lut_host, void **blob_out, size_t *blob_bytes);
 int build_ed_cells(PalDev &dev, const double *pts_host, void **blob_out);
 int build_ed_ext(PalDev &dev, const double *pts_host, void **blob_out);
diff --git a/dither_pie_amd/csrc/host.cpp b/dither_pie_amd/csrc/host.cpp
--- a/dither_pie_amd/csrc/host.cpp
+++ b/dither_pie_amd/csrc/host.cpp
@@ -5,6 +5,7 @@
 #include <numeric>
 
 #include "dp_internal.h"
+#include "ordered_fine.h"
 #include "../../include/ditherpie_hip_dotdiff.h"
 #include "../../include/ditherpie_hip_cells.h"
 #include "../../include/ditherpie_hip_voidcluster.h"
@@ -263,6 +264,8 @@
     p->pat_blob = nullptr;
     p->fine_dev = nullptr;
     p->fine_pending = false;
+    p->fine_plain_pending = false;
+    p->fine_sub_room = 0;
     p->metric = metric;
     p->met = dp::MetDev{nullptr, nullptr, nullptr, nullptr, 0};
     p->met_blob = nullptr;
@@ -315,18 +318,35 @@
     return DP_OK;
 }
 
-static int ensure_fine_table(const dp_palette *pal_c, hipStream_t s)
+static int ensure_fine_table(const dp_palette *pal_c, hipStream_t s, const int thr_bytes)
 {
     dp_palette *p = const_cast<dp_palette *>(pal_c);
     std::lock_guard<std::mutex> lock(p->build_mu);
-    if (!p->fine_pending.load()) return DP_OK;
+    const bool first = p->fine_pending.load();
+    if (!first && !(p->fine_plain_pending.load() && thr_bytes > p->fine_sub_room.load())) return DP_OK;
     hipStreamCaptureStatus capturing = hipStreamCaptureStatusNone;
     if (hipStreamIsCapturing(s, &capturing) != hipSuccess || capturing != hipStreamCaptureStatusNone) return DP_OK;
-    p->fine_pending = false;
     dp::PalDev d = snapshot(p);
-    const int rc = build_fine(d, p->p4_host, p->fine_masks, p->fine_dev);
-    std::vector<uint32_t>().swap(p->fine_masks);
-    if (rc != DP_OK) return rc;
+    bool plain = !first;
+    if (first) {
+        p->fine_pending = false;
+        if (dp::kFineSubShipped > 0 || dp::kExperiments) {
+            const int rc = build_fine(d, p->p4_host, p->fine_masks, p->fine_dev, true);
+            if (rc != DP_OK) return rc;
+        }
+        const int room = d.fsub_tab ? dp::kLeanTabBytes - (int)dp::fine_sub_bytes(d.fsub_win, d.fsub_wide) : -1;
+        plain = dp::kExperiments || thr_bytes > room;
+        if (!plain) {
+            p->fine_sub_room = room;
+            p->fine_plain_pending = true;
+        }
+    }
+    if (plain) {
+        p->fine_plain_pending = false;
+        const int rc = build_fine(d, p->p4_host, p->fine_masks, p->fine_dev, false);
+        std::vector<uint32_t>().swap(p->fine_masks);
+        if (rc != DP_OK) return rc;
+    }
     publish(p, d);
     return DP_OK;
 }
@@ -607,8 +627,11 @@
                   dp_ordered_workspace_bytes(n_frames, h, w));
         return DP_EWORKSPACE;
     }
-    if (mode == DP_MODE_MATRIX && thr->dev.mpad && pal->fine_pending.load(std::memory_order_relaxed)) {
-        const int rc = ensure_fine_table(pal, (hipStream_t)stream);
+    const int fine_thr_bytes = mode == DP_MODE_MATRIX && thr->dev.mpad ? thr->dev.th_h * thr->dev.tw_pad * 4 : 0;
+    if (mode == DP_MODE_MATRIX && thr->dev.mpad &&
+        (pal->fine_pending.load(std::memory_order_relaxed) ||
+         (pal->fine_plain_pending.load(std::memory_order_relaxed) && fine_thr_bytes > pal->fine_sub_room.load(std::memory_order_relaxed)))) {
+        const int rc = ensure_fine_table(pal, (hipStream_t)stream, fine_thr_bytes);
         if (rc != DP_OK) return rc;
     }
     return launch_ordered(in_dev, out_dev, n_frames, h, w, y0, x0, snapshot(pal), mode, thr ? &thr->dev : nullptr,
diff --git a/dither_pie_amd/csrc/host_logic.h b/dither_pie_amd/csrc/host_logic.h
--- a/dither_pie_amd/csrc/host_logic.h
+++ b/dither_pie_amd/csrc/host_logic.h
@@ -436,6 +436,8 @@
 constexpr int kFineIds = kWideCap;
 
 inline int fine_cell(const int r, const int g, const int b) { return (r >> 3) | ((g >> 3) << 5) | ((b >> 3) << 10); }
+constexpr uint16_t kFineSubTag = 0x8000u;
+inline int fine_sub_cell(const int r, const int g, const int b) { return ((r >> 2) & 1) | (((g >> 2) & 1) << 1) | (((b >> 2) & 1) << 2); }
 
 struct FineTable {
     bool ok = false;
@@ -447,6 +449,9 @@
     std::vector<uint16_t> wide_cell;
     std::vector<uint32_t> wide;
     std::vector<uint16_t> wide_idx;
+    bool sub = false;
+    std::vector<uint16_t> rows;
+    std::vector<uint16_t> sub_wide;
     std::vector<uint32_t> lds_image() const
     {
         std::vector<uint32_t> im;
@@ -461,11 +466,22 @@
         }
         return im;
     }
+    std::vector<uint32_t> sub_image() const
+    {
+        std::vector<uint32_t> im;
+        im.reserve(quad.size() + wide.size() + pair.size() + kFineCells / 2 + rows.size() / 2);
+        im.insert(im.end(), quad.begin(), quad.end());
+        im.insert(im.end(), wide.begin(), wide.end());
+        im.insert(im.end(), pair.begin(), pair.end());
+        for (int c = 0; c < kFineCells; c += 2) im.push_back((uint32_t)off[c] | ((uint32_t)off[c + 1] << 16));
+        for (size_t i = 0; i < rows.size(); i += 2) im.push_back((uint32_t)rows[i] | ((uint32_t)rows[i + 1] << 16));
+        return im;
+    }
 };
 
 template <class Fits>
-void fine_pack(const uint32_t *tmask, const uint32_t *nmask, const int mw, const int K, const std::vector<uint32_t> &coord4, Fits fits,
-               FineTable &ft)
+void fine_pack_units(const uint32_t *tmask, const uint32_t *nmask, const int mw, const int K, const std::vector<uint32_t> &coord4, Fits fits,
+                     FineTable &ft, const bool sub)
 {
     ft = FineTable{};
     if (K < kWideList || K > 256 || K > 32 * mw) return;
@@ -522,10 +538,51 @@
         cls[cell] = (uint8_t)((kFineWindow - nt) * (kFineQuad + 1) + (kFineQuad - nn));
         ++class_count[cls[cell] + 1];
     }
+    const int n_units = kFineCells + (sub ? 8 * ft.n_wide : 0);
+    if (sub) {
+        tms.resize(n_units), nms.resize(n_units), cls.resize(n_units, 0xff);
+        for (int k = 0; k < ft.n_wide; ++k) {
+            const int cell = ft.wide_cell[k];
+            const int r0 = (cell & 31) * 8, g0 = ((cell >> 5) & 31) * 8, b0 = (cell >> 10) * 8;
+            const uint16_t *list = &ft.wide_idx[(size_t)k * kWideList];
+            int pr[kWideList], pg[kWideList], pb[kWideList];
+            for (int i = 0; i < kWideList; ++i) {
+                const uint32_t c = coord4[list[i]];
+                pr[i] = (int)(c & 255u), pg[i] = (int)((c >> 8) & 255u), pb[i] = (int)((c >> 16) & 255u);
+            }
+            for (int s = 0; s < 8; ++s) {
+                Mask tm{{0, 0, 0, 0}}, nm{{0, 0, 0, 0}};
+                for (int i = 0; i < 64; ++i) {
+                    const int r = r0 + (s & 1) * 4 + (i & 3), g = g0 + ((s >> 1) & 1) * 4 + ((i >> 2) & 3), b = b0 + (s >> 2) * 4 + (i >> 4);
+                    int d[kWideList], d0 = 1 << 30, d1 = 1 << 30;
+                    for (int q = 0; q < kWideList; ++q) {
+                        d[q] = (r - pr[q]) * (r - pr[q]) + (g - pg[q]) * (g - pg[q]) + (b - pb[q]) * (b - pb[q]);
+                        if (d[q] < d0) d1 = d0, d0 = d[q];
+                        else if (d[q] < d1) d1 = d[q];
+                    }
+                    for (int q = 0; q < kWideList; ++q) {
+                        if (d[q] <= d1) tm.set(list[q]);
+                        if (d[q] == d0) nm.set(list[q]);
+                    }
+                }
+                const int u = kFineCells + 8 * k + s;
+                tms[u] = tm, nms[u] = nm;
+                const int nt = tm.count(), nn = nm.count();
+                if (nn > kFineQuad || nt > kFineWindow) {
+                    ft.sub_wide.push_back((uint16_t)(8 * k + s));
+                    continue;
+                }
+                cls[u] = (uint8_t)((kFineWindow - nt) * (kFineQuad + 1) + (kFineQuad - nn));
+                ++class_count[cls[u] + 1];
+            }
+        }
+    }
     for (int c = 0; c < kClasses; ++c) class_count[c + 1] += class_count[c];
     std::vector<int> order(class_count[kClasses]);
-    for (int cell = 0; cell < kFineCells; ++cell)
+    for (int cell = 0; cell < n_units; ++cell)
         if (cls[cell] != 0xff) order[class_count[cls[cell]]++] = cell;
+    std::vector<uint16_t> unit_win(sub ? n_units : 0, 0);
+    auto win_of = [&](const int u) -> uint16_t & { return u < kFineCells ? ft.off[u] : unit_win[u]; };
     struct Win {
         Mask a, ab;
         int na, nb;
@@ -542,7 +599,7 @@
         bool met = false;
         for (; seen[slot] != 0; slot = (slot + 1) & (kSlots - 1))
             if (nms[seen[slot] - 1] == nm && tms[seen[slot] - 1] == tm) {
-                ft.off[cell] = ft.off[seen[slot] - 1];
+                win_of(cell) = win_of(seen[slot] - 1);
                 met = true;
                 break;
             }
@@ -597,7 +654,12 @@
                 holds[j].push_back(best);
             }
         });
-        ft.off[cell] = (uint16_t)best;
+        win_of(cell) = (uint16_t)best;
+    }
+    if (sub) {
+        ft.sub = true;
+        ft.rows.assign(unit_win.begin() + kFineCells, unit_win.end());
+        for (int k = 0; k < ft.n_wide; ++k) ft.off[ft.wide_cell[k]] = (uint16_t)(kFineSubTag | k);
     }
     ft.n_win = (int)wins.size();
     ft.win_idx.assign((size_t)ft.n_win * kFineWindow, 0);
@@ -623,6 +685,19 @@
             else ft.pair[(size_t)wi * (kFineWindow - kFineQuad) + p - kFineQuad] = c;
         }
     ft.ok = true;
+}
+
+template <class Fits>
+void fine_pack(const uint32_t *tmask, const uint32_t *nmask, const int mw, const int K, const std::vector<uint32_t> &coord4, Fits fits,
+               FineTable &ft)
+{
+    fine_pack_units(tmask, nmask, mw, K, coord4, fits, ft, false);
+}
+template <class Fits>
+void fine_pack_sub(const uint32_t *tmask, const uint32_t *nmask, const int mw, const int K, const std::vector<uint32_t> &coord4, Fits fits,
+                   FineTable &ft)
+{
+    fine_pack_units(tmask, nmask, mw, K, coord4, fits, ft, true);
 }
 
 
diff --git a/dither_pie_amd/csrc/host_sanitize.cpp b/dither_pie_amd/csrc/host_sanitize.cpp
--- a/dither_pie_amd/csrc/host_sanitize.cpp
+++ b/dither_pie_amd/csrc/host_sanitize.cpp
@@ -676,6 +676,118 @@
     return bad ? 1 : 0;
 }
 
+static int run_finesub(const char *path, const int K, const char *out_path)
+{
+    if (K < 2 || K > 256) {
+        fprintf(stderr, "finesub: 2 <= K <= 256\n");
+        return 2;
+    }
+    std::vector<uint8_t> pal((size_t)K * 3);
+    FILE *f = fopen(path, "rb");
+    if (!f || fread(pal.data(), 1, pal.size(), f) != pal.size()) {
+        fprintf(stderr, "cannot read %d colours from %s\n", K, path);
+        return 2;
+    }
+    fclose(f);
+    const int mw = 8;
+    std::vector<uint32_t> coord4(K), tm, nm;
+    for (int j = 0; j < K; ++j) coord4[j] = (uint32_t)pal[3 * j] | ((uint32_t)pal[3 * j + 1] << 8) | ((uint32_t)pal[3 * j + 2] << 16);
+    fine_masks(pal, K, mw, tm, nm);
+    FineTable ft, again;
+    fine_pack_sub(tm.data(), nm.data(), mw, K, coord4, fine_sub_fits, ft);
+    fine_pack_sub(tm.data(), nm.data(), mw, K, coord4, fine_sub_fits, again);
+    const std::vector<uint32_t> im = ft.ok ? ft.sub_image() : std::vector<uint32_t>();
+    int bad = ft.ok != again.ok || ft.off != again.off || ft.rows != again.rows || ft.win_idx != again.win_idx || ft.wide_idx != again.wide_idx ||
+              ft.sub_wide != again.sub_wide;
+    if (ft.ok) {
+        bad += (int64_t)im.size() * 4 != fine_sub_image_bytes(ft.n_win, ft.n_wide) || !fine_sub_fits(ft.n_win, ft.n_wide) || !ft.sub;
+        size_t still = 0;
+        for (int k = 0; k < ft.n_wide; ++k) {
+            const int cell = ft.wide_cell[(size_t)k];
+            bad += ft.off[(size_t)cell] != (uint16_t)(kFineSubTag | k);
+            for (int sc = 0; sc < 8; ++sc) {
+                std::vector<uint8_t> in_t((size_t)K, 0), in_n((size_t)K, 0);
+                std::vector<int> d((size_t)K);
+                for (int i = 0; i < 64; ++i) {
+                    const int r = (cell & 31) * 8 + (sc & 1) * 4 + (i & 3), g = ((cell >> 5) & 31) * 8 + ((sc >> 1) & 1) * 4 + ((i >> 2) & 3),
+                              b = (cell >> 10) * 8 + (sc >> 2) * 4 + (i >> 4);
+                    bad += fine_cell(r, g, b) != cell || fine_sub_cell(r, g, b) != sc;
+                    int d0 = 1 << 30, d1 = 1 << 30;
+                    for (int j = 0; j < K; ++j) {
+                        const uint8_t *q = &pal[3 * (size_t)j];
+                        d[(size_t)j] = (r - q[0]) * (r - q[0]) + (g - q[1]) * (g - q[1]) + (b - q[2]) * (b - q[2]);
+                        if (d[(size_t)j] < d0) d1 = d0, d0 = d[(size_t)j];
+                        else if (d[(size_t)j] < d1) d1 = d[(size_t)j];
+                    }
+                    for (int j = 0; j < K; ++j) {
+                        if (d[(size_t)j] <= d1) in_t[(size_t)j] = 1;
+                        if (d[(size_t)j] == d0) in_n[(size_t)j] = 1;
+                    }
+                }
+                int nt = 0, nn = 0;
+                for (int j = 0; j < K; ++j) nt += in_t[(size_t)j], nn += in_n[(size_t)j];
+                const uint16_t wi = ft.rows[(size_t)k * 8 + sc];
+                const bool wide = nn > kFineQuad || nt > kFineWindow;
+                if (wide) {
+                    bad += wi != 0 || still >= ft.sub_wide.size() || ft.sub_wide[still] != (uint16_t)(8 * k + sc);
+                    ++still;
+                    continue;
+                }
+                bad += wi == 0 || wi >= ft.n_win;
+                if (wi == 0 || wi >= ft.n_win) continue;
+                const uint16_t *e = &ft.win_idx[(size_t)wi * kFineWindow];
+                for (int j = 0; j < K; ++j) {
+                    bool in_quad = false, in_win = false;
+                    for (int q = 0; q < kFineWindow; ++q)
+                        if (e[q] == j) in_win = true, in_quad = in_quad || q < kFineQuad;
+                    bad += (in_n[(size_t)j] && !in_quad) || (in_t[(size_t)j] && !in_win);
+                }
+            }
+        }
+        bad += still != ft.sub_wide.size();
+    }
+    f = fopen(out_path, "wb");
+    if (!f) return 2;
+    const int32_t head[5] = {ft.ok ? 1 : 0, ft.n_win, ft.n_wide, (int32_t)ft.sub_wide.size(), (int32_t)im.size()};
+    fwrite(head, sizeof(int32_t), 5, f);
+    if (ft.ok) {
+        fwrite(ft.off.data(), 2, ft.off.size(), f);
+        fwrite(ft.rows.data(), 2, ft.rows.size(), f);
+        fwrite(ft.win_idx.data(), 2, ft.win_idx.size(), f);
+        fwrite(ft.wide_cell.data(), 2, ft.wide_cell.size(), f);
+        fwrite(ft.sub_wide.data(), 2, ft.sub_wide.size(), f);
+        fwrite(ft.wide_idx.data(), 2, ft.wide_idx.size(), f);
+        fwrite(ft.quad.data(), 4, ft.quad.size(), f);
+        fwrite(ft.pair.data(), 4, ft.pair.size(), f);
+        fwrite(ft.wide.data(), 4, ft.wide.size(), f);
+        fwrite(im.data(), 4, im.size(), f);
+    }
+    fclose(f);
+    printf("finesub K=%d ok=%d windows=%d wide=%d still_wide=%zu bytes=%lld bad=%d\n", K, (int)ft.ok, ft.n_win, ft.n_wide, ft.sub_wide.size(),
+           (long long)(ft.ok ? fine_sub_bytes(ft.n_win, ft.n_wide) : 0), bad);
+    return bad ? 1 : 0;
+}
+
+static int run_finesublevel(const char *path, const int n_cases)
+{
+    FILE *f = fopen(path, "rb");
+    if (!f) {
+        fprintf(stderr, "cannot open %s\n", path);
+        return 2;
+    }
+    for (int c = 0; c < n_cases; ++c) {
+        FineSubFacts ff;
+        if (fread(&ff, sizeof(ff), 1, f) != 1 || ff.n_win < 0 || ff.n_wide < 0 || ff.thr_bytes < 0) {
+            fprintf(stderr, "bad record %d in %s\n", c, path);
+            fclose(f);
+            return 2;
+        }
+        printf("sub %d %d\n", c, fine_sub_level(ff));
+    }
+    fclose(f);
+    return 0;
+}
+
 static int run_fineplan(const char *path, const int n_cases)
 {
     FILE *f = fopen(path, "rb");
@@ -918,7 +1030,7 @@
 int main(int argc, char **argv)
 {
     if (argc < 4) {
-        fprintf(stderr, "usage: %s kdtree|edtables|accel <pts.f64> <K> [bw]  |  mediancut <rgb.u8> <n> <depth>  |  indexmap <lists.bin> <n>  |  giflzw <cases.bin> <n>  |  pngdeflate|pngdyn|pngfile <cases.bin> <n>  |  orderedplan <cases.bin> <n>  |  voidcluster <cases.bin> <n>  |  metric <cases.bin> <n>  |  finepack <pal.u8> <K> <out.bin>  |  fineplan <cases.bin> <n>  |  finekeys <cases.bin> <n>  |  idiffplan <cases.bin> <n>  |  okfit <cases.bin> <n>  |  resamplecoeffs <cases.bin> <n>  |  resample <cases.bin> <n> <out.bin>\n", argv[0]);
+        fprintf(stderr, "usage: %s kdtree|edtables|accel <pts.f64> <K> [bw]  |  mediancut <rgb.u8> <n> <depth>  |  indexmap <lists.bin> <n>  |  giflzw <cases.bin> <n>  |  pngdeflate|pngdyn|pngfile <cases.bin> <n>  |  orderedplan <cases.bin> <n>  |  voidcluster <cases.bin> <n>  |  metric <cases.bin> <n>  |  finepack <pal.u8> <K> <out.bin>  |  fineplan <cases.bin> <n>  |  finekeys <cases.bin> <n>  |  finesub <pal.u8> <K> <out.bin>  |  finesublevel <cases.bin> <n>  |  idiffplan <cases.bin> <n>  |  okfit <cases.bin> <n>  |  resamplecoeffs <cases.bin> <n>  |  resample <cases.bin> <n> <out.bin>\n", argv[0]);
         return 2;
     }
     if (std::string(argv[1]) == "mediancut") return run_mediancut(argv[2], atol(argv[3]), argc > 4 ? atoi(argv[4]) : 4);
@@ -933,6 +1045,8 @@
     if (std::string(argv[1]) == "finepack") return argc > 4 ? run_finepack(argv[2], atoi(argv[3]), argv[4]) : 2;
     if (std::string(argv[1]) == "fineplan") return run_fineplan(argv[2], atoi(argv[3]));
     if (std::string(argv[1]) == "finekeys") return run_finekeys(argv[2], atoi(argv[3]));
+    if (std::string(argv[1]) == "finesub") return argc > 4 ? run_finesub(argv[2], atoi(argv[3]), argv[4]) : 2;
+    if (std::string(argv[1]) == "finesublevel") return run_finesublevel(argv[2], atoi(argv[3]));
     if (std::string(argv[1]) == "idiffplan") return run_idiffplan(argv[2], atoi(argv[3]));
     if (std::string(argv[1]) == "okfit") return run_okfit(argv[2], atoi(argv[3]));
     if (std::string(argv[1]) == "resamplecoeffs") return run_resamplecoeffs(argv[2], atoi(argv[3]));
diff --git a/dither_pie_amd/csrc/ordered.hip b/dither_pie_amd/csrc/ordered.hip
--- a/dither_pie_amd/csrc/ordered.hip
+++ b/dither_pie_amd/csrc/ordered.hip
@@ -1945,7 +1945,35 @@
     uint32_t wide_at, norm_at, pair_at, off_at, ids_at, thr_at;
 };
 
-template <int MODE, int KEYS>
+__device__ __forceinline__ uint32_t fine_row_address(const uint32_t tag, const uint32_t x, const uint32_t rows_at)
+{
+    const uint32_t sub2 = __builtin_amdgcn_udot4((x >> 2) & 0x010101u, 0x00080402u, rows_at, false);
+    return ((tag & (uint32_t)(kFineIds - 1)) << 4) + sub2;
+}
+
+template <int MODE>
+__device__ __forceinline__ bool resolve_window(const uint32_t x, const LeanThr &th, const int sh, const uint8_t *s_bytes, const uint32_t win,
+                                               const uint32_t pair_at, const int neg2, uint32_t &c)
+{
+    const uint4 ca = *reinterpret_cast<const uint4 *>(s_bytes + (win << 4));
+    const uint32_t pb = pair_at + (win << 3);
+    const uint2 cb = *reinterpret_cast<const uint2 *>(s_bytes + pb);
+    int m0, m1, m2;
+    cand6(x, ca, cb.x, cb.y, neg2, m0, m1, m2);
+    const int a0 = m0 >> kLocalBits, a1 = m1 >> kLocalBits, a2 = m2 >> kLocalBits;
+    if (a0 == a1 || a1 == a2) return false;
+    const int xx = (int)__builtin_amdgcn_udot4(x, x, 0u, false);
+    const uint32_t d0 = (uint32_t)(a0 + xx);
+    const uint32_t S = d0 + (uint32_t)a1 + (uint32_t)xx;
+    bool eq;
+    const bool nearest = lean_decide<MODE>(d0, S, th, sh, eq);
+    if (eq) return false;
+    const uint32_t pos = (uint32_t)(nearest ? m0 : m1) & 0xfcu;
+    c = *reinterpret_cast<const uint32_t *>(s_bytes + (pos < 16u ? (win << 4) + pos : pb + pos - 16u));
+    return true;
+}
+
+template <int MODE, int KEYS, int SUB>
 __device__ __forceinline__ uint32_t fine_pixel_full(const uint32_t entry, const uint8_t *__restrict__ in, uint8_t *__restrict__ out,
                                                     unsigned long long *__restrict__ flags, const Geo &g, const PalDev &pal,
                                                     const ThrDev &thr, const uint32_t *s_words, const FineLds &at)
@@ -1960,7 +1988,21 @@
     const uint32_t cell2 = fine_cell_offset(x);
     uint32_t c = 0;
     bool done = false, slow = false;
-    if (*reinterpret_cast<const uint16_t *>(s_bytes + at.off_at + cell2) == 0) {
+    if constexpr (SUB != 0) {
+        uint32_t tag = *reinterpret_cast<const uint16_t *>(s_bytes + at.off_at + cell2);
+        if constexpr (SUB == 1) {
+            const uint32_t off_src = (uint32_t)pal.fsub_win * kFineWindow + (uint32_t)pal.fsub_wide * kWideList;
+            tag = tag == 0u ? (uint32_t) reinterpret_cast<const uint16_t *>(pal.fsub_tab + off_src)[cell2 >> 1] : 0u;
+        }
+        if ((tag & kFineSubTag) != 0u) {
+            const uint32_t win = *reinterpret_cast<const uint16_t *>(s_bytes + fine_row_address(tag, x, at.ids_at));
+            if (win == 0u)
+                done = resolve_wide<MODE>(x, th, thr.sh, pal.fsub_tab + (uint32_t)pal.fsub_win * kFineQuad + (tag & (uint32_t)(kFineIds - 1)) * kWideList,
+                                          kWideList, c);
+            else if constexpr (SUB == 1)
+                done = resolve_window<MODE>(x, th, thr.sh, s_bytes, win, at.pair_at, g.neg2, c);
+        }
+    } else if (*reinterpret_cast<const uint16_t *>(s_bytes + at.off_at + cell2) == 0) {
         const uint16_t *ids = reinterpret_cast<const uint16_t *>(s_bytes + at.ids_at);
         const uint32_t cell = cell2 >> 1;
         uint32_t lo = 0;
@@ -1985,7 +2027,7 @@
     return rest ? ((entry & ~15u) | rest) : 0u;
 }
 
-template <int MODE, int KEYS>
+template <int MODE, int KEYS, int SUB = 0>
 __global__ __launch_bounds__(kCellBlock, 4) void ordered_fine_kernel(const uint8_t *__restrict__ in, uint8_t *__restrict__ out,
                                                                     unsigned long long *__restrict__ flags, const Geo g,
                                                                     const PalDev pal, const ThrDev thr, const float sx, const float sy,
@@ -1994,6 +2036,7 @@
     static_assert(MODE == 1, "integer thresholds in LDS only");
     (void)sx, (void)sy, (void)sc;
     static_assert(KEYS >= 0 && KEYS <= 2, "key levels: ordered_fine.h");
+    static_assert(SUB == 0 || ((SUB == 1 || SUB == 2) && KEYS == 1), "SUB levels: ordered_fine.h");
     __shared__ __align__(16) uint32_t smem[kLeanLdsWords];
     FineLds at;
     if constexpr (KEYS == 0) {
@@ -2005,20 +2048,21 @@
         at.off_at = at.pair_at + (uint32_t)pal.fine_win * ((kFineWindow - kFineQuad) * 4);
     } else {
         constexpr int kPairRec = KEYS == 2 ? 4 : 2;
-        const int n_win = pal.fine_win;
-        const int pair_src = n_win * kFineQuad + pal.fine_wide * kWideList;
+        const uint32_t *tab = SUB == 0 ? pal.fine_tab : pal.fsub_tab;
+        const int n_win = SUB == 0 ? pal.fine_win : pal.fsub_win, n_wide = SUB == 0 ? pal.fine_wide : pal.fsub_wide;
+        const int pair_src = n_win * kFineQuad + n_wide * kWideList;
         const int tail_src = pair_src + n_win * (kFineWindow - kFineQuad);
         at.wide_at = 0;
         at.norm_at = (uint32_t)n_win * (kFineQuad * 4);
         at.pair_at = 2 * at.norm_at;
         at.off_at = at.pair_at + (uint32_t)n_win * (kPairRec * 4);
         for (int wi = threadIdx.x; wi < n_win; wi += kCellBlock) {
-            const uint4 c = *reinterpret_cast<const uint4 *>(&pal.fine_tab[wi * kFineQuad]);
+            const uint4 c = *reinterpret_cast<const uint4 *>(&tab[wi * kFineQuad]);
             *reinterpret_cast<uint4 *>(&smem[wi * 4]) = c;
             *reinterpret_cast<uint4 *>(&smem[n_win * 4 + wi * 4]) =
                 make_uint4((__builtin_amdgcn_udot4(c.x, c.x, 0u, false) << kLocalBits), (__builtin_amdgcn_udot4(c.y, c.y, 0u, false) << kLocalBits) + 4u,
                            (__builtin_amdgcn_udot4(c.z, c.z, 0u, false) << kLocalBits) + 8u, (__builtin_amdgcn_udot4(c.w, c.w, 0u, false) << kLocalBits) + 12u);
-            const uint2 b = *reinterpret_cast<const uint2 *>(&pal.fine_tab[pair_src + wi * 2]);
+            const uint2 b = *reinterpret_cast<const uint2 *>(&tab[pair_src + wi * 2]);
             if constexpr (KEYS == 2)
                 *reinterpret_cast<uint4 *>(&smem[n_win * 8 + wi * 4]) =
                     make_uint4(b.x, b.y, (__builtin_amdgcn_udot4(b.x, b.x, 0u, false) << kLocalBits) + 16u,
@@ -2027,11 +2071,18 @@
                 *reinterpret_cast<uint2 *>(&smem[n_win * 8 + wi * 2]) = b;
         }
         uint32_t *s_tail = smem + at.off_at / 4;
-        for (int i = threadIdx.x * 2; i < (kFineCells + kFineIds) / 2; i += kCellBlock * 2)
-            *reinterpret_cast<uint2 *>(&s_tail[i]) = *reinterpret_cast<const uint2 *>(&pal.fine_tab[tail_src + i]);
+        const int tail_words = SUB == 0 ? (kFineCells + kFineIds) / 2 : kFineCells / 2 + n_wide * 4;
+        for (int i = threadIdx.x * 2; i < tail_words; i += kCellBlock * 2) {
+            uint2 v = *reinterpret_cast<const uint2 *>(&tab[tail_src + i]);
+            if (SUB == 1 && i < kFineCells / 2) {
+                v.x &= ~(((v.x & 0x80008000u) >> 15) * 0xffffu);
+                v.y &= ~(((v.y & 0x80008000u) >> 15) * 0xffffu);
+            }
+            *reinterpret_cast<uint2 *>(&s_tail[i]) = v;
+        }
     }
     at.ids_at = at.off_at + kFineCells * 2;
-    at.thr_at = at.ids_at + kFineIds * 2;
+    at.thr_at = at.ids_at + (SUB == 0 ? (uint32_t)kFineIds * 2 : (uint32_t)pal.fsub_wide * 16);
     {
         const int n = thr.th_h * thr.tw_pad;
         const int thr_word = KEYS == 0 ? pal.fine_words : (int)(at.thr_at / 4);
@@ -2054,7 +2105,7 @@
         qcount -= n;
         __threadfence_block();
         uint32_t rest = 0u;
-        if (lane < n) rest = fine_pixel_full<MODE, KEYS>(s_queue[qcount + lane], in, out, flags, g, pal, thr, smem, at);
+        if (lane < n) rest = fine_pixel_full<MODE, KEYS, SUB>(s_queue[qcount + lane], in, out, flags, g, pal, thr, smem, at);
         queue_push(s_queue, qcount, rest != 0u, rest);
     };
 
@@ -2069,8 +2120,16 @@
         const uint32_t gidx1 = gidx0 + gridDim.x * kCellBlock;
         if (tile + gridDim.x < n_tiles && gidx1 < n_full) wnn = in3[gidx1];
     }
+    auto sub_windows = [&](const uint32_t xq[4], uint32_t win[4]) {
+        if constexpr (SUB == 2) {
+#pragma unroll
+            for (int q = 0; q < 4; ++q)
+                if ((win[q] & kFineSubTag) != 0u) win[q] = *reinterpret_cast<const uint16_t *>(s_bytes + fine_row_address(win[q], xq[q], at.ids_at));
+        }
+    };
     unpack4(wn, xn);
     windows(xn, winn);
+    sub_windows(xn, winn);
     const bool use_cls = thr.has_cls != 0;
     uint32_t cls_word = 0, cls_shift = 0;
     auto tile_class = [&](const uint32_t ty, const uint32_t tx, const uint32_t gi) {
@@ -2187,6 +2246,7 @@
 #pragma unroll
             for (int q = 0; q < 4; ++q) rare[q] = gidx * 4u + (uint32_t)q < g.n_px;
         }
+        sub_windows(xn, winn);
         const uint32_t rmask = (rare[0] ? 1u : 0u) | (rare[1] ? 2u : 0u) | (rare[2] ? 4u : 0u) | (rare[3] ? 8u : 0u);
         const unsigned long long rb = __ballot(rmask != 0u);
         if (rb != 0ull) {
@@ -2850,13 +2910,13 @@
     return cached;
 }
 
-static inline void trace_plan(const OrderedPlan &p, bool aligned, bool fine, int keys)
+static inline void trace_plan(const OrderedPlan &p, bool aligned, bool fine, int keys, int sub)
 {
 #ifdef DP_EXPERIMENTS
     if (std::getenv("DP_ORDERED_TRACE")) {
         constexpr const char *tables[] = {"plain8", "plain4", "warped"};
-        char keys_s[16] = "";
-        if (fine) snprintf(keys_s, sizeof(keys_s), " keys=%d", keys);
+        char keys_s[32] = "";
+        if (fine) snprintf(keys_s, sizeof(keys_s), " keys=%d sub=%d", keys, sub);
         fprintf(stderr, "dp_ordered_u8: pass 1 = %s (4-byte aligned frames: %d) mode=%d bw=%d adapt=%d warp=%d half=%d table=%s fix_big_queue=%d kernel=%s%s\n",
                 family_name(p.family), aligned ? 1 : 0, p.mode, p.bw, p.adapt ? 1 : 0, p.warp ? 1 : 0, p.half ? 1 : 0, tables[p.table],
                 p.fix_big_queue ? 1 : 0, fine ? "fine" : family_name(p.family), keys_s);
@@ -2866,6 +2926,7 @@
     (void)aligned;
     (void)fine;
     (void)keys;
+    (void)sub;
 #endif
 }
 
@@ -2918,8 +2979,14 @@
     return nullptr;
 }
 
-TileKernel fine_kernel(const int keys)
-{
+TileKernel fine_kernel(const int keys, const int sub)
+{
+    if (sub == 2) return keys == 1 ? ordered_fine_kernel<1, 1, 2> : nullptr;
+#ifdef DP_EXPERIMENTS
+    if (sub == 1) return keys == 1 ? ordered_fine_kernel<1, 1, 1> : nullptr;
+#else
+    if (sub == 1) return nullptr;
+#endif
     switch (keys) {
     case 0: return ordered_fine_kernel<1, 0>;
     case 1: return ordered_fine_kernel<1, 1>;
@@ -3011,12 +3078,19 @@
         g.adv_x = plan.adv_x;
         const bool brute = plan.family == kFamBrute;
         const FineFacts fine_facts{pal.fine_tab != nullptr, pal.fine_win, pal.fine_wide, thr.th_h * thr.tw_pad * 4};
-        const bool fine = fine_replaces(plan, fine_facts) && !exp_env("DP_NO_FINE_KERNEL");
+        const bool fine_plain = fine_replaces(plan, fine_facts) && !exp_env("DP_NO_FINE_KERNEL");
         int keys_cap = kFineKeysShipped;
         if (const char *cap = exp_env("DP_FINE_KEYS_MAX")) keys_cap = std::min(2, std::max(0, std::atoi(cap)));
-        const int fine_keys = fine ? std::min(fine_keys_level(fine_facts), keys_cap) : 0;
+        int sub_cap = kFineSubShipped;
+        if (const char *cap = exp_env("DP_FINE_SUB_MAX")) sub_cap = std::min(2, std::max(0, std::atoi(cap)));
+        const bool sub_only = pal.fine_tab == nullptr && pal.fsub_tab != nullptr && fine_plan_ok(plan) && !exp_env("DP_NO_FINE_KERNEL");
+        const int keys_plain = fine_plain ? std::min(fine_keys_level(fine_facts), keys_cap) : (sub_only ? std::min(1, keys_cap) : 0);
+        const FineSubFacts sub_facts{pal.fsub_tab != nullptr && (fine_plain || sub_only), pal.fsub_win, pal.fsub_wide, fine_facts.thr_bytes, keys_plain, sub_cap};
+        const int fine_sub = fine_sub_level(sub_facts);
+        const bool fine = fine_plain || fine_sub != 0;
+        const int fine_keys = fine ? keys_plain : 0;
         const BruteKernel brute_k = brute ? brute_kernel(plan, pal.is_integer != 0) : nullptr;
-        const TileKernel tile_k = brute ? nullptr : (fine ? fine_kernel(fine_keys) : tile_kernel(plan));
+        const TileKernel tile_k = brute ? nullptr : (fine ? fine_kernel(fine_keys, fine_sub) : tile_kernel(plan));
         const FixKernel fix_k = fix_kernel(plan);
         if ((brute ? brute_k == nullptr : tile_k == nullptr) || fix_k == nullptr) {
             set_error("dp_ordered_u8: no %s kernel for mode %d", family_name(plan.family), plan.mode);
@@ -3043,7 +3117,7 @@
                                plan.n_tiles);
         }
         DP_HIP(hipGetLastError());
-        trace_plan(plan, g.aligned, fine, fine_keys);
+        trace_plan(plan, g.aligned, fine, fine_keys, fine_sub);
         prof_mid(pm, s);
         hipLaunchKernelGGL(fix_k, dim3(plan.fix_grid), dim3(kBlock), 0, s, in_c, out_c, fl, plan.n_words, g, pal, thr, sx, sy, ign_scale);
         prof_end(pm, s);
diff --git a/dither_pie_amd/csrc/ordered_fine.h b/dither_pie_amd/csrc/ordered_fine.h
--- a/dither_pie_amd/csrc/ordered_fine.h
+++ b/dither_pie_amd/csrc/ordered_fine.h
@@ -40,4 +40,36 @@
 
 constexpr int kFineKeysShipped = 1;
 
+constexpr int64_t fine_sub_bytes(const int n_win, const int n_wide)
+{
+    return (int64_t)n_win * 40 + kFineCells * 2 + (int64_t)n_wide * 16;
 }
+constexpr int64_t fine_sub_image_bytes(const int n_win, const int n_wide)
+{
+    return (int64_t)n_win * (kFineWindow * 4) + (int64_t)n_wide * (kWideList * 4 + 16) + kFineCells * 2;
+}
+constexpr bool fine_sub_fits(const int n_win, const int n_wide)
+{
+    return n_wide <= kFineIds && fine_sub_bytes(n_win, n_wide) + 16 * 19 * 4 <= kLeanTabBytes && fine_sub_image_bytes(n_win, n_wide) <= kLeanTabBytes;
+}
+
+struct FineSubFacts {
+    int32_t present;
+    int32_t n_win, n_wide;
+    int32_t thr_bytes;
+    int32_t keys;
+    int32_t cap;
+};
+inline int fine_sub_level(const FineSubFacts &f)
+{
+    if (f.present == 0 || f.keys != 1 || f.cap < 1 || f.n_wide > kFineIds) return 0;
+    return fine_sub_bytes(f.n_win, f.n_wide) + (int64_t)f.thr_bytes <= kLeanTabBytes ? (f.cap < 2 ? 1 : 2) : 0;
+}
+inline bool fine_plan_ok(const OrderedPlan &p)
+{
+    return p.family == kFamLean && p.mode == 1 && p.bw == 8 && p.table == kTabPlain8 && !p.adapt && !p.warp && !p.half;
+}
+
+constexpr int kFineSubShipped = 2;
+
+}
```

After: 448,500 Mpixel/s, median of 6. 1.08x the previous value.
